# alexoz12v2/cuda-optix-pathtracing

Hardware: AMD Instinct MI355X
Metric: Msamples/s (paths x spp / s) (higher is better)
Workload: dtype f32

## Files before the change

### cuda-optix-pathtracing_amd/binding.py

```python
import ctypes as C
import subprocess
from pathlib import Path

import numpy as np

_HERE = Path(__file__).resolve().parent
_CSRC = _HERE / "csrc"
_LIB = None

DMT_ACCEL_BRUTE_FORCE = 0
DMT_ACCEL_BVH = 1
BVH_BUILD_HOST = 0
BVH_BUILD_DEVICE = 1
BVH_BUILT_BY_HOST = 0
BVH_BUILT_BY_DEVICE = 1
BVH_BUILT_BY_HOST_AFTER_DEVICE = 2
BVH_UPDATE_REBUILD = 0
BVH_UPDATE_REFIT = 1
BVH_UPDATE_AUTO = 2
BVH_UPDATED_NONE = 0
BVH_UPDATED_REFIT = 1
BVH_UPDATED_REBUILD = 2
BVH_UPDATED_REBUILD_AFTER_REFIT = 3


class DmtError(RuntimeError):
    pass


def library_path():
    import os
    alt = os.environ.get("DMT_HIP_LIB")
    return Path(alt) if alt else _CSRC / "libdmt_hip.so"


def build_library(force=False):
    args = ["make", "-C", str(_CSRC)]
    if force:
        args.append("-B")
    subprocess.check_call(args)
    return library_path()


def load_library():
    global _LIB
    if _LIB is None:
        so = library_path()
        if not so.exists():
            raise DmtError(f"{so} is missing: run `python -c 'import __graft_entry__ as g; g.build()'` "
                           "(the HIP path has no fallback)")
        lib = C.CDLL(str(so))
        lib.dmt_last_error.restype = C.c_char_p
        lib.dmt_last_error.argtypes = [C.c_void_p]
        _LIB = lib
    return _LIB


EXPORTED_SYMBOLS = [
    "dmt_ctx_create", "dmt_ctx_destroy", "dmt_last_error", "dmt_upload_triangles", "dmt_upload_bsdfs",
    "dmt_upload_lights", "dmt_set_camera", "dmt_set_limits", "dmt_set_accel", "dmt_set_light_sampling", "dmt_light_tree_pmfs", "dmt_light_tree_ref_select", "dmt_set_bvh_strategy", "dmt_set_partition", "dmt_set_chunk", "dmt_render_profile",
    "dmt_upload_area_lights", "dmt_upload_textures", "dmt_upload_envmap", "dmt_clear_envmap", "dmt_envmap_tables", "dmt_test_envmap",
    "dmt_set_stream", "dmt_film_clear", "dmt_film_bind", "dmt_film_device_ptrs", "dmt_download_film",
    "dmt_render", "dmt_render_adaptive", "dmt_render_stats", "dmt_sync", "dmt_sched_diag", "dmt_kernel_time", "dmt_kernel_info", "dmt_bvh_validate", "dmt_brute_cull_plan", "dmt_brute_cull_box_plan", "dmt_test_triangle_intersect",
    "dmt_test_sampler", "dmt_test_camera_rays", "dmt_test_bsdf", "dmt_test_bsdf_ng", "dmt_test_material", "dmt_test_light", "dmt_test_half",
    "dmt_test_trace_samples", "dmt_test_trace_log", "dmt_test_closest_hit",
    "dmt_set_texture_filter", "dmt_texture_mip_chain", "dmt_texture_footprint", "dmt_test_texture_filter",
    "dmt_render_aovs", "dmt_upload_aovs", "dmt_download_aovs", "dmt_denoise_defaults", "dmt_denoise",
    "dmt_set_accel_build", "dmt_accel_build_info", "dmt_accel_download", "dmt_lbvh_reference", "dmt_bvh_check",
    "dmt_update_vertices", "dmt_update_vertices_device", "dmt_set_accel_update", "dmt_accel_update_info", "dmt_bvh_refit_reference",
    "dmt_download_aov_surface", "dmt_upload_aov_surface", "dmt_camera_project", "dmt_test_camera_project", "dmt_temporal_defaults",
    "dmt_denoise_temporal", "dmt_temporal_reset", "dmt_temporal_info", "dmt_temporal_download",
    "dmt_set_sampler_table", "dmt_sampler_table_plan", "dmt_test_sampler_table",
    "dmt_set_lens", "dmt_lens_info", "dmt_lens_rays", "dmt_focus_distance_at", "dmt_test_lens_values",
    "dmt_set_motion", "dmt_clear_motion", "dmt_set_shutter", "dmt_motion_info", "dmt_shutter_times", "dmt_motion_positions",
    "dmt_motion_bvh_validate", "dmt_test_shutter_times", "dmt_test_closest_hit_at",
]

SAMPLER_TABLE_OFF = 0
SAMPLER_TABLE_AUTO = 1
SAMPLER_TABLE_FORCE = 2


class SamplerTablePlanRecord(C.Structure):
    _fields_ = [("use", C.c_uint32), ("period_width", C.c_uint32), ("period_height", C.c_uint32), ("entry_bytes", C.c_uint32),
                ("slices", C.c_uint32), ("reserved", C.c_uint32), ("slice_bytes", C.c_uint64)]


def sampler_table_plan(width, height, owned_pixels, spp, chunk_spp, budget_bytes=0, mode=SAMPLER_TABLE_AUTO):
    lib = load_library()
    rec = SamplerTablePlanRecord()
    args = [int(width), int(height), C.c_uint64(int(owned_pixels)), C.c_uint32(int(spp)), C.c_uint32(int(chunk_spp)),
            C.c_uint64(int(budget_bytes)), int(mode)]
    rc = lib.dmt_sampler_table_plan(*args, C.byref(rec), None, C.c_uint32(0))
    if rc != 0:
        raise DmtError(f"dmt_sampler_table_plan failed ({rc})")
    lens = (C.c_uint32 * max(int(rec.slices), 1))()
    rc = lib.dmt_sampler_table_plan(*args, C.byref(rec), lens, C.c_uint32(int(rec.slices)))
    if rc != 0:
        raise DmtError(f"dmt_sampler_table_plan failed ({rc})")
    out = {name: int(getattr(rec, name)) for name, _ in SamplerTablePlanRecord._fields_ if name != "reserved"}
    out["use"] = bool(rec.use)
    out["slice_spp"] = [int(x) for x in lens[:int(rec.slices)]]
    return out


class DenoiseParams(C.Structure):
    _fields_ = [("iterations", C.c_int32), ("sigma_normal", C.c_float), ("sigma_position", C.c_float),
                ("sigma_albedo", C.c_float), ("sigma_luminance", C.c_float)]


def denoise_defaults():
    lib = load_library()
    lib.dmt_denoise_defaults.restype = DenoiseParams
    p = lib.dmt_denoise_defaults()
    return {name: getattr(p, name) for name, _ in DenoiseParams._fields_}



class TemporalParams(C.Structure):
    _fields_ = [("alpha", C.c_float), ("normal_threshold", C.c_float), ("plane_threshold", C.c_float)]


class TemporalRecord(C.Structure):
    _fields_ = [("frames", C.c_uint32), ("reprojected", C.c_uint32), ("reset", C.c_uint32), ("temporal_ms", C.c_float),
                ("history_bytes", C.c_uint64)]


def temporal_defaults():
    lib = load_library()
    lib.dmt_temporal_defaults.restype = TemporalParams
    p = lib.dmt_temporal_defaults()
    return {name: getattr(p, name) for name, _ in TemporalParams._fields_}


def camera_project(camera44, points):
    lib = load_library()
    cam = np.ascontiguousarray(camera44, np.uint8).reshape(44)
    p = np.ascontiguousarray(points, np.float32).reshape(-1, 3)
    xy, depth = np.zeros((p.shape[0], 2), np.float32), np.zeros(p.shape[0], np.float32)
    rc = lib.dmt_camera_project(cam.ctypes.data_as(C.c_void_p), int(p.shape[0]), p.ctypes.data_as(C.c_void_p),
                                xy.ctypes.data_as(C.c_void_p), depth.ctypes.data_as(C.c_void_p))
    if rc != 0:
        raise DmtError(f"dmt_camera_project failed ({rc})")
    return xy, depth


def lens_rays(camera44, lens_radius, focus_distance, pxs, pys, ss):
    lib = load_library()
    cam = np.ascontiguousarray(camera44, np.uint8).reshape(44)
    pxs, pys, ss = (np.ascontiguousarray(a, np.int32).reshape(-1) for a in (pxs, pys, ss))
    n = pxs.shape[0]
    assert pys.shape[0] == n and ss.shape[0] == n
    o, d, u = np.zeros((n, 3), np.float32), np.zeros((n, 3), np.float32), np.zeros((n, 2), np.float32)
    as_p = lambda a: a.ctypes.data_as(C.c_void_p)
    rc = lib.dmt_lens_rays(as_p(cam), C.c_float(lens_radius), C.c_float(focus_distance), int(n), as_p(pxs), as_p(pys), as_p(ss),
                           as_p(o), as_p(d), as_p(u))
    if rc != 0:
        raise DmtError(f"dmt_lens_rays failed ({rc})")
# ... 340 lines not shown
        else:
            self.upload_textures(None, None, None, None)

    def upload_textures(self, tex_rgba, tex_desc, mat_tex, tri_uv):
        if tex_desc is None or len(tex_desc) == 0:
            self._check(self._lib.dmt_upload_textures(self._ctx, None, C.c_uint64(0), None, C.c_uint32(0), None, C.c_uint32(0), None,
                                                      C.c_uint64(0)), "dmt_upload_textures")
            return
        rgba = np.ascontiguousarray(tex_rgba, np.uint8).reshape(-1, 4)
        desc = np.ascontiguousarray(tex_desc, np.int32).reshape(-1, 3)
        mt = np.ascontiguousarray(mat_tex, np.uint32).reshape(-1, 4)
        uv = np.ascontiguousarray(tri_uv, np.float32).reshape(-1, 6)
        self._check(self._lib.dmt_upload_textures(self._ctx, _p(rgba), C.c_uint64(rgba.shape[0]), _p(desc), C.c_uint32(desc.shape[0]), _p(mt),
                                                  C.c_uint32(mt.shape[0]), _p(uv), C.c_uint64(uv.shape[0])), "dmt_upload_textures")

    def upload_area_lights(self, tri, le):
        tri = np.ascontiguousarray(tri, np.uint32).reshape(-1)
        le = np.ascontiguousarray(le, np.float32).reshape(-1, 3)
        assert tri.shape[0] == le.shape[0]
        self._check(self._lib.dmt_upload_area_lights(self._ctx, _p(tri), _p(le), C.c_uint32(tri.shape[0])),
                    "dmt_upload_area_lights")

    def upload_envmap(self, rgb, quat=(0, 0, 0, 1), scale=1.0):
        rgb = np.ascontiguousarray(rgb, np.float32)
        h, w = rgb.shape[:2]
        q = np.ascontiguousarray(quat, np.float32)
        self._check(self._lib.dmt_upload_envmap(self._ctx, _p(rgb), int(w), int(h), _p(q), C.c_float(scale)),
                    "dmt_upload_envmap")

    def clear_envmap(self):
        self._check(self._lib.dmt_clear_envmap(self._ctx), "dmt_clear_envmap")

    def test_envmap(self, u2, wi):
        u2, wi = _f32(u2).reshape(-1, 2), _f32(wi).reshape(-1, 3)
        n = u2.shape[0]
        assert wi.shape[0] == n
        out = dict(wi=np.zeros((n, 3), np.float32), pdf=np.zeros(n, np.float32), uv=np.zeros((n, 2), np.float32),
                   Le=np.zeros((n, 3), np.float32), ok=np.zeros(n, np.int32), Le_dir=np.zeros((n, 3), np.float32),
                   pdf_dir=np.zeros(n, np.float32))
        self._check(self._lib.dmt_test_envmap(self._ctx, n, _p(u2), _p(wi), _p(out["wi"]), _p(out["pdf"]), _p(out["uv"]),
                                              _p(out["Le"]), _p(out["ok"]), _p(out["Le_dir"]), _p(out["pdf_dir"])),
                    "dmt_test_envmap")
        return out

    def set_limits(self, max_depth):
        self._check(self._lib.dmt_set_limits(self._ctx, int(max_depth)), "dmt_set_limits")

    def set_accel(self, mode):
        self._check(self._lib.dmt_set_accel(self._ctx, int(mode)), "dmt_set_accel")

    def set_accel_build(self, mode):
        self._check(self._lib.dmt_set_accel_build(self._ctx, int(mode)), "dmt_set_accel_build")

    def accel_build_info(self):
        rec = AccelBuildRecord()
        self._check(self._lib.dmt_accel_build_info(self._ctx, C.byref(rec)), "dmt_accel_build_info")
        return {name: getattr(rec, name) for name, _ in AccelBuildRecord._fields_ if name != "reserved"}

    def download_accel(self):
        info = self.accel_build_info()
        nodes = np.zeros((max(info["nodes"], 1), 64), np.uint8)
        pairs = np.zeros((max(info["pairs"], 1), 2), np.uint32)
        self._check(self._lib.dmt_accel_download(self._ctx, _p(nodes), C.c_size_t(nodes.shape[0]), _p(pairs), C.c_size_t(pairs.shape[0])),
                    "dmt_accel_download")
        return nodes[:info["nodes"]].copy(), pairs[:info["pairs"]].copy()

    def set_light_sampling(self, mode):
        self._check(self._lib.dmt_set_light_sampling(self._ctx, int(mode)), "dmt_set_light_sampling")

    def set_texture_filter(self, mode):
        self._check(self._lib.dmt_set_texture_filter(self._ctx, int(mode)), "dmt_set_texture_filter")

    def set_bvh_strategy(self, strategy, paths_per_pass=0):
        self._check(self._lib.dmt_set_bvh_strategy(self._ctx, int(strategy), C.c_uint64(int(paths_per_pass))), "dmt_set_bvh_strategy")

    def set_partition(self, rank, world):
        self._check(self._lib.dmt_set_partition(self._ctx, int(rank), int(world)), "dmt_set_partition")

    def set_chunk(self, samples_per_item):
        self._check(self._lib.dmt_set_chunk(self._ctx, C.c_uint32(samples_per_item)), "dmt_set_chunk")

    def set_sampler_table(self, mode, budget_bytes=0):
        self._check(self._lib.dmt_set_sampler_table(self._ctx, int(mode), C.c_uint64(int(budget_bytes))), "dmt_set_sampler_table")

    def set_stream(self, stream_ptr):
        self._check(self._lib.dmt_set_stream(self._ctx, C.c_void_p(stream_ptr)), "dmt_set_stream")

    def film_clear(self):
        self._check(self._lib.dmt_film_clear(self._ctx), "dmt_film_clear")

    def film_bind(self, mean_ptr, m2_ptr):
        self._check(self._lib.dmt_film_bind(self._ctx, C.c_void_p(mean_ptr), C.c_void_p(m2_ptr)), "dmt_film_bind")

    def film_device_ptrs(self):
        a, b = C.c_void_p(), C.c_void_p()
        self._check(self._lib.dmt_film_device_ptrs(self._ctx, C.byref(a), C.byref(b)), "dmt_film_device_ptrs")
        return a.value, b.value

    def download_film(self):
        mean = np.zeros((self.height, self.width, 4), np.float32)
        m2 = np.zeros((self.height, self.width, 4), np.float32)
        self._check(self._lib.dmt_download_film(self._ctx, _p(mean), _p(m2)), "dmt_download_film")
        return mean, m2

    def render(self, spp, sample_offset=0, region=None):
        x0, y0, x1, y1 = region if region is not None else (0, 0, self.width, self.height)
        self._check(self._lib.dmt_render(self._ctx, C.c_uint32(sample_offset), C.c_uint32(spp), int(x0), int(y0),
                                         int(x1), int(y1)), "dmt_render")

    def render_adaptive(self, threshold, max_spp, step_spp, min_spp=0, region=None):
        x0, y0, x1, y1 = region if region is not None else (0, 0, self.width, self.height)
        rounds, samples = C.c_uint32(0), C.c_uint64(0)
        self._check(self._lib.dmt_render_adaptive(self._ctx, C.c_uint32(min_spp), C.c_uint32(max_spp), C.c_uint32(step_spp),
                                                  C.c_float(threshold), int(x0), int(y0), int(x1), int(y1), C.byref(rounds),
                                                  C.byref(samples)), "dmt_render_adaptive")
        return int(rounds.value), int(samples.value)

    def render_stats(self, spp, sample_offset=0, region=None):
        x0, y0, x1, y1 = region if region is not None else (0, 0, self.width, self.height)
        out = np.zeros(6, np.uint64)
        self._check(self._lib.dmt_render_stats(self._ctx, C.c_uint32(sample_offset), C.c_uint32(spp), int(x0), int(y0),
                                               int(x1), int(y1), _p(out)), "dmt_render_stats")
        keys = ["samples", "closest_rays", "shadow_rays", "node_visits", "tri_tests", "bounces"]
        return dict(zip(keys, (int(v) for v in out)))

    def render_profile(self, spp, sample_offset=0, region=None):
        x0, y0, x1, y1 = region if region is not None else (0, 0, self.width, self.height)
        out = np.zeros(16, np.uint64)
        self._check(self._lib.dmt_render_profile(self._ctx, C.c_uint32(sample_offset), C.c_uint32(spp), int(x0), int(y0),
                                                 int(x1), int(y1), _p(out)), "dmt_render_profile")
        keys = ["samples", "closest_rays", "shadow_rays", "node_visits", "tri_tests", "bounces", "it_node", "it_leaf",
                "it_shade", "it_outer", "it_prep", "lanes_leaf", "lanes_shade", "lanes_prep", "dead_nodes", "overflow_pushes"]
        return dict(zip(keys, (int(v) for v in out)))

    def render_aovs(self, aov_spp=4):
        self._check(self._lib.dmt_render_aovs(self._ctx, C.c_uint32(aov_spp)), "dmt_render_aovs")
        self._aov_shape = (self.height, self.width)

    def upload_aovs(self, albedo, normal, position):
        a, n, p = _f32(albedo), _f32(normal), _f32(position)
        assert a.ndim == 3 and a.shape[2] == 4 and a.shape == n.shape == p.shape
        h, w = a.shape[:2]
        self._check(self._lib.dmt_upload_aovs(self._ctx, _p(a), _p(n), _p(p), int(w), int(h)), "dmt_upload_aovs")
        self._aov_shape = (h, w)

    def download_aovs(self):
        h, w = self._aov_shape or (self.height, self.width)
        out = [np.zeros((h, w, 4), np.float32) for _ in range(3)]
        self._check(self._lib.dmt_download_aovs(self._ctx, *[_p(x) for x in out]), "dmt_download_aovs")
        return tuple(out)

    def denoise(self, params=None, film=None):
        p = denoise_defaults()
        unknown = set(params or {}) - set(p)
        if unknown:
            raise ValueError(f"unknown denoise parameters {sorted(unknown)}")
        p.update(params or {})
        cp = DenoiseParams(int(p["iterations"]), float(p["sigma_normal"]), float(p["sigma_position"]), float(p["sigma_albedo"]),
                           float(p["sigma_luminance"]))
        mean = m2 = None
        if film is not None:
            mean, m2 = _f32(film[0]), _f32(film[1])
            assert mean.shape == m2.shape == (self.height, self.width, 4)
        out = np.zeros((self.height, self.width, 4), np.float32)
        ms = C.c_float()
        self._check(self._lib.dmt_denoise(self._ctx, C.byref(cp), _p(mean), _p(m2), _p(out), C.byref(ms)), "dmt_denoise")
# ... 67 lines not shown

    def kernel_time(self, reset=True):
        ms, n = C.c_double(), C.c_uint64()
        self._check(self._lib.dmt_kernel_time(self._ctx, C.byref(ms), C.byref(n), int(bool(reset))), "dmt_kernel_time")
        return ms.value, n.value

    def kernel_info(self):
        v = [C.c_int() for _ in range(5)]
        self._check(self._lib.dmt_kernel_info(self._ctx, *[C.byref(x) for x in v]), "dmt_kernel_info")
        keys = ["vgprs", "sgprs", "lds_bytes", "blocks_per_cu", "cu_count"]
        return dict(zip(keys, (x.value for x in v)))

    def test_triangle_intersect(self, xs, ys, zs, o, d):
        xs, ys, zs = _f32(xs), _f32(ys), _f32(zs)
        n = xs.size // 4
        o, d = _f32(o), _f32(d)
        hit = np.zeros(n, np.int32)
        t = np.zeros(n, np.float32)
        pos, nrm, err = (np.zeros((n, 3), np.float32) for _ in range(3))
        self._check(self._lib.dmt_test_triangle_intersect(self._ctx, _p(xs), _p(ys), _p(zs), C.c_size_t(n), _p(o),
                                                          _p(d), _p(hit), _p(t), _p(pos), _p(nrm), _p(err)),
                    "dmt_test_triangle_intersect")
        return hit, t, pos, nrm, err

    def test_sampler(self, w, h, pxs, pys, ss, ndims):
        pxs, pys, ss = _i32(pxs), _i32(pys), _i32(ss)
        n = pxs.shape[0]
        hi = np.zeros(n, np.int32)
        p2 = np.zeros((n, 2), np.float32)
        d = np.zeros((n, ndims), np.float32)
        self._check(self._lib.dmt_test_sampler(self._ctx, int(w), int(h), n, _p(pxs), _p(pys), _p(ss), int(ndims),
                                               _p(hi), _p(p2), _p(d)), "dmt_test_sampler")
        return hi, p2, d

    def test_sampler_table(self, w, h, s0, n):
        pw, ph = min(int(w), 128), min(int(h), 128)
        vals = np.zeros((n, ph, pw, 8), np.float32)
        jit = np.zeros((n, ph, pw, 2), np.float32)
        self._check(self._lib.dmt_test_sampler_table(self._ctx, int(w), int(h), C.c_uint32(int(s0)), C.c_uint32(int(n)), _p(vals), _p(jit)),
                    "dmt_test_sampler_table")
        return vals, jit

    def test_camera_rays(self, pxs, pys, ss):
        pxs, pys, ss = _i32(pxs), _i32(pys), _i32(ss)
        n = pxs.shape[0]
        o = np.zeros((n, 3), np.float32)
        d = np.zeros((n, 3), np.float32)
        self._check(self._lib.dmt_test_camera_rays(self._ctx, n, _p(pxs), _p(pys), _p(ss), _p(o), _p(d)),
                    "dmt_test_camera_rays")
        return o, d

    def test_lens_values(self, pxs, pys, ss):
        pxs, pys, ss = _i32(pxs), _i32(pys), _i32(ss)
        n = pxs.shape[0]
        u = np.zeros((n, 2), np.float32)
        self._check(self._lib.dmt_test_lens_values(self._ctx, n, _p(pxs), _p(pys), _p(ss), _p(u)), "dmt_test_lens_values")
        return u

    def test_bsdf(self, bsdf32, ns, wo, u2, uc, wi_eval):
        b = np.ascontiguousarray(bsdf32, np.uint8).reshape(32)
        ns, wo, wi_eval = _f32(ns, (-1, 3)), _f32(wo, (-1, 3)), _f32(wi_eval, (-1, 3))
        u2, uc = _f32(u2, (-1, 2)), _f32(uc, (-1,))
        n = ns.shape[0]
        prep = np.zeros((n, 12), np.float32)
        samp = np.zeros((n, 10), np.float32)
        ev = np.zeros((n, 4), np.float32)
        self._check(self._lib.dmt_test_bsdf(self._ctx, _p(b), n, _p(ns), _p(wo), _p(u2), _p(uc), _p(wi_eval),
                                            _p(prep), _p(samp), _p(ev)), "dmt_test_bsdf")
        return prep, samp, ev

    def test_bsdf_ng(self, bsdf32, ns, ng, wo, u2, uc, wi_eval):
        b = np.ascontiguousarray(bsdf32, np.uint8).reshape(32)
        ns, ng, wo, wi_eval = _f32(ns, (-1, 3)), _f32(ng, (-1, 3)), _f32(wo, (-1, 3)), _f32(wi_eval, (-1, 3))
        u2, uc = _f32(u2, (-1, 2)), _f32(uc, (-1,))
        n = ns.shape[0]
        assert ng.shape[0] == n and wo.shape[0] == n and wi_eval.shape[0] == n and u2.shape[0] == n and uc.shape[0] == n
        prep = np.zeros((n, 12), np.float32)
        samp = np.zeros((n, 10), np.float32)
        ev = np.zeros((n, 4), np.float32)
        self._check(self._lib.dmt_test_bsdf_ng(self._ctx, _p(b), n, _p(ns), _p(ng), _p(wo), _p(u2), _p(uc), _p(wi_eval),
                                               _p(prep), _p(samp), _p(ev)), "dmt_test_bsdf_ng")
        return prep, samp, ev

    def test_material(self, tri, bu, bv, ng):
        tri, bu, bv, ng = _i32(tri), _f32(bu, (-1,)), _f32(bv, (-1,)), _f32(ng, (-1, 3))
        n = tri.shape[0]
        assert bu.shape[0] == n and bv.shape[0] == n and ng.shape[0] == n
        rec, rec2 = np.zeros((n, 32), np.uint8), np.zeros((n, 32), np.uint8)
        ns = np.zeros((n, 3), np.float32)
        mix = np.zeros(n, np.float32)
        self._check(self._lib.dmt_test_material(self._ctx, n, _p(tri), _p(bu), _p(bv), _p(ng), _p(rec), _p(ns), _p(rec2),
                                                _p(mix)), "dmt_test_material")
        return rec, ns, rec2, mix

    def test_light(self, light32, pos, nrm, u2, had_t):
        l = np.ascontiguousarray(light32, np.uint8).reshape(32)
        pos, nrm, u2 = _f32(pos, (-1, 3)), _f32(nrm, (-1, 3)), _f32(u2, (-1, 2))
        ht = _i32(had_t)
        n = pos.shape[0]
        out = np.zeros((n, 14), np.float32)
        self._check(self._lib.dmt_test_light(self._ctx, _p(l), n, _p(pos), _p(nrm), _p(u2), _p(ht), _p(out)),
                    "dmt_test_light")
        return out

    def test_half(self, floats=None, halves=None):
        h_out = f_out = None
        n = 0
        if floats is not None:
            floats = _f32(floats, (-1,))
            n = floats.shape[0]
            h_out = np.zeros(n, np.uint16)
        if halves is not None:
            halves = np.ascontiguousarray(halves, np.uint16).reshape(-1)
            n = halves.shape[0]
            f_out = np.zeros(n, np.float32)
        if floats is not None and halves is not None:
            assert floats.shape[0] == halves.shape[0]
        self._check(self._lib.dmt_test_half(self._ctx, n, _p(floats), _p(h_out), _p(halves), _p(f_out)),
                    "dmt_test_half")
        return h_out, f_out

    def test_trace_samples(self, pxs, pys, ss):
        pxs, pys, ss = _i32(pxs), _i32(pys), _i32(ss)
        n = pxs.shape[0]
        out = np.zeros((n, 3), np.float32)
        self._check(self._lib.dmt_test_trace_samples(self._ctx, n, _p(pxs), _p(pys), _p(ss), _p(out)),
                    "dmt_test_trace_samples")
        return out

    def test_texture_filter(self, tri, bu, bv, tex, depth=0):
        tri, tex = _i32(tri), _i32(tex)
        bu, bv = _f32(bu), _f32(bv)
        n = tri.shape[0]
        tex = np.ascontiguousarray(np.broadcast_to(tex, (n,)), np.int32)
        depth = np.ascontiguousarray(np.broadcast_to(_i32(depth), (n,)), np.int32)
        assert bu.shape[0] == n and bv.shape[0] == n
        rgb = np.zeros((n, 3), np.float32)
        branch = np.zeros(n, np.int32)
        lod = np.zeros(n, np.float32)
        self._check(self._lib.dmt_test_texture_filter(self._ctx, n, _p(tri), _p(bu), _p(bv), _p(tex), _p(depth), _p(rgb),
                                                      _p(branch), _p(lod)), "dmt_test_texture_filter")
        return rgb, branch, lod

    def test_trace_log(self, px, py, s, cap=64):
        rec = np.zeros((cap, 12), np.float32)
        n = C.c_int()
        L = np.zeros(3, np.float32)
        self._check(self._lib.dmt_test_trace_log(self._ctx, int(px), int(py), int(s), _p(rec), int(cap), C.byref(n),
                                                 _p(L)), "dmt_test_trace_log")
        return rec[:n.value], L

    def test_shutter_times(self, pxs, pys, ss):
        pxs, pys, ss = _i32(pxs), _i32(pys), _i32(ss)
        n = pxs.shape[0]
        t = np.zeros(n, np.float32)
        self._check(self._lib.dmt_test_shutter_times(self._ctx, n, _p(pxs), _p(pys), _p(ss), _p(t)), "dmt_test_shutter_times")
        return t

    def test_closest_hit_at(self, o, d, time):
        o, d = _f32(o, (-1, 3)), _f32(d, (-1, 3))
        n = o.shape[0]
        time = np.ascontiguousarray(np.broadcast_to(np.asarray(time, np.float32), (n,)))
        idx, t, uv = np.zeros(n, np.int32), np.zeros(n, np.float32), np.zeros((n, 2), np.float32)
        self._check(self._lib.dmt_test_closest_hit_at(self._ctx, n, _p(o), _p(d), _p(time), _p(idx), _p(t), _p(uv)),
                    "dmt_test_closest_hit_at")
        return idx, t, uv

    def test_closest_hit(self, o, d):
        o, d = _f32(o, (-1, 3)), _f32(d, (-1, 3))
        n = o.shape[0]
        idx = np.zeros(n, np.int32)
        t = np.zeros(n, np.float32)
        self._check(self._lib.dmt_test_closest_hit(self._ctx, n, _p(o), _p(d), _p(idx), _p(t)),
                    "dmt_test_closest_hit")
        return idx, t
```

### cuda-optix-pathtracing_amd/csrc/dmt_hip.hip

```cpp
#include <hip/hip_runtime.h>

#include <algorithm>
#include <chrono>
#include <cmath>
#include <cstddef>
#include <cstdio>
#include <cstdlib>
#include <cstring>
#include <limits>
#include <memory>
#include <new>
#include <string>
#include <vector>

#include "../../include/dmt_hip.h"
#include "pt_device.hpp"
#include "bvh_device.hpp"
#include "bvh_gpu_build.hpp"
#include "devbuf.hpp"
#include "envmap.hpp"
#include "light_tree.hpp"
#include "light_tree_ref.hpp"

using namespace dmt;

namespace {

constexpr uint32_t kCullMaxClusters = 12;
constexpr uint32_t kCullGroup = 4;
constexpr uint32_t kCullMaxTris = 44;
constexpr uint32_t kCullSlotBits = 6;
constexpr uint32_t kCullMaxIndex = 1u << (32 - kCullSlotBits);
struct CullCluster {
  float b[6];
  uint32_t box;
  uint32_t first, count;
  uint32_t slot, magic;
  uint32_t pad;
};
struct CullRec {
  uint32_t first, countSlot, magic;
};
struct CullView {
  TriIsect const* always;
  uint32_t const* alwaysIdx;
  CullCluster const* clusters;
  float const* tri9;
  uint32_t alwaysCount, clusterCount;
};

struct RenderParams {
  SceneView scene;
  CullView cull;
  BvhView bvh;
  CameraXf cam;
  SamplerParams sp;
  float4* __restrict__ mean;
  float4* __restrict__ m2;
  uint32_t* __restrict__ counter;
  int width, height;
  int x0, y0, x1, y1;
  int tx0, ty0, rtx;
  uint32_t numItems;
  uint32_t subShift;
  int rank, world;
  uint32_t sampleOffset, spp;
  uint32_t chunkSpp;
  uint32_t numChunks;
  float* stage;
  uint32_t* link;
  uint32_t* slabBusy;
  uint32_t const* tileList;
  unsigned long long const* tileMask;
  unsigned long long* schedDiag;
  float4 const* samTab;
  float2 const* samTabJit;
  float2 const* samTabLens;
  uint32_t samTabS0, samTabPw, samTabPh;
  float lensR, lensD;
  int maxDepth;
  int shadeThreshold;
  EnvView env;
  uint32_t const* areaOf;
  uint32_t const* areaTri;
  float const* areaLe;
  uint32_t areaCount;
  uint32_t const* texRgba;
  int32_t const* texDesc;
  uint32_t const* matTex;
  float const* triUv;
  LightTreeNode const* lightTree;
  LightTreeRefNode const* lightTreeRef;
  unsigned long long* stats;
  float texCfr[12];
  float texMinDx[3], texMinDy[3];
  float texSppScale;
  uint32_t const* texMip;
  int32_t const* texMipDesc;
  MotionView motion;
};

typedef RenderParams const DMT_CONST_AS* KArgs;
DMT_DEV KArgs kargs_base() { return (KArgs)__builtin_amdgcn_kernarg_segment_ptr(); }
DMT_DEV KArgs kargs(KArgs p) {
  asm volatile("" : "+s"(p));
  return p;
}
DMT_DEV SceneView load_scene(KArgs k) {
  k = kargs(k);
  SceneView s;
  s.tris = k->scene.tris, s.post = k->scene.post, s.bsdfs = k->scene.bsdfs, s.lights = k->scene.lights;
  s.infLights = k->scene.infLights, s.triCount = k->scene.triCount, s.bsdfCount = k->scene.bsdfCount;
  s.lightCount = k->scene.lightCount, s.infLightCount = k->scene.infLightCount;
  return s;
}
DMT_DEV BvhView load_bvh(KArgs k) {
  k = kargs(k);
  BvhView b;
  b.nodes = k->bvh.nodes, b.pairs = k->bvh.pairs, b.overflow = k->bvh.overflow, b.overflowStride = k->bvh.overflowStride;
  return b;
}

DMT_DEV EnvView load_env(KArgs k) {
  k = kargs(k);
  EnvView e;
  e.func = k->env.func, e.cdf = k->env.cdf, e.rowInt = k->env.rowInt, e.mFunc = k->env.mFunc, e.mCdf = k->env.mCdf;
  e.rgb = k->env.rgb, e.mInt = k->env.mInt, e.w = k->env.w, e.h = k->env.h;
  e.qx = k->env.qx, e.qy = k->env.qy, e.qz = k->env.qz, e.qw = k->env.qw;
  return e;
}

#ifndef DMT_SECTION_TIMING
#define DMT_SECTION_TIMING 0
#endif
#if DMT_SECTION_TIMING
__device__ unsigned long long g_sect[16];
__shared__ unsigned long long s_sectLast[kLdsThreads / 64];
__shared__ unsigned long long s_sectAcc[kLdsThreads / 64][16];
#endif
DMT_DEV void sect_mark(int i) {
#if DMT_SECTION_TIMING
  unsigned long long const now = __builtin_readcyclecounter();
  unsigned long long const m = __ballot(1);
  if (int(__ffsll((long long)m)) - 1 == int(threadIdx.x & 63u)) {
    uint32_t const w = threadIdx.x >> 6;
    s_sectAcc[w][i] += now - s_sectLast[w];
    s_sectLast[w] = now;
  }
#endif
}
struct PathState {
  RayPair rp;
  f3 beta, L;
  int depth;
  bool lastT;
  bool active;
  bool hasShadow;
  bool finPending;
  float smax;
  Sampler rng;
  uint32_t sidx;
  float lastPdf;
  bool lastSpecular;
};
__shared__ float s_cold[7 * kLdsThreads];
DMT_DEV void put_C(f3 v) {
  float* const c = s_cold + threadIdx.x;
  c[0 * kLdsThreads] = v.x, c[1 * kLdsThreads] = v.y, c[2 * kLdsThreads] = v.z;
}
DMT_DEV f3 get_C() {
  float const* const c = s_cold + threadIdx.x;
  return mk3(c[0 * kLdsThreads], c[1 * kLdsThreads], c[2 * kLdsThreads]);
}
DMT_DEV void put_Lfin(f3 v) {
  float* const c = s_cold + threadIdx.x;
  c[3 * kLdsThreads] = v.x, c[4 * kLdsThreads] = v.y, c[5 * kLdsThreads] = v.z;
}
DMT_DEV f3 get_Lfin() {
  float const* const c = s_cold + threadIdx.x;
  return mk3(c[3 * kLdsThreads], c[4 * kLdsThreads], c[5 * kLdsThreads]);
}
DMT_DEV void put_finIdx(uint32_t i) { s_cold[6 * kLdsThreads + threadIdx.x] = __uint_as_float(i); }
// ... 431 lines not shown
  gram_schmidt(ng, tx, ty);
  f3 const ns = tx * n.x + ty * n.y + ng * n.z;
  float const l2 = dot(ns, ns);
  return (l2 > 0.f && l2 < kInf) ? ns / sqrtf(l2) : ng;
}

template <bool CULL = true>
DMT_DEV void trace_pair_brute(KArgs k, PathState const& st, bool doC, bool doS, int& bestTri, float& bu, float& bv, bool& occluded);

#include "motion.hpp"

constexpr uint32_t kFeatBvh = 1u << 0;
constexpr uint32_t kFeatStats = 1u << 1;
constexpr uint32_t kFeatEnv = 1u << 2;
constexpr uint32_t kFeatArea = 1u << 3;
constexpr uint32_t kFeatTex = 1u << 4;
constexpr uint32_t kFeatBlend = 1u << 5;
constexpr uint32_t kFeatLightTree = 1u << 6;
constexpr uint32_t kFeatLightTreeRef = 1u << 7;
constexpr uint32_t kFeatTexFilter = 1u << 8;
constexpr uint32_t kFeatMotion = 1u << 9;

template <uint32_t F>
DMT_DEV Hit shade_hit(KArgs k, SceneView const& sc, int tri, float bu, float bv, f3 rd) {
  if constexpr (F & kFeatMotion) return hit_finish(motion_post(k, sc.post[tri], tri, motion_time()), bu, bv, rd);
  else return hit_finish(sc.post[tri], bu, bv, rd);
}

template <uint32_t F>
DMT_DEV bool path_shade(KArgs k, PathState& st, int bestTri, float bu, float bv) {
  static_assert(!((F & kFeatLightTree) && (F & kFeatLightTreeRef)), "one light tree at a time");
  static_assert(!((F & kFeatTex) && (F & kFeatBlend)), "kFeatBlend carries the texture code itself");
  static_assert(!(F & kFeatTexFilter) || (F & (kFeatTex | kFeatBlend)), "the texture filter needs the texture code");
  static_assert(!(F & kFeatMotion) || !(F & ~(kFeatMotion | kFeatBvh | kFeatEnv)), "motion: the plain and env-map rows only");
  SceneView const sc = load_scene(k);
  int const maxDepth = kargs(k)->maxDepth;
  if constexpr (F & kFeatEnv) {
    if (bestTri < 0) {
      EnvView const env = load_env(k);
      float pdfLight = 0.f;
      f3 const Le = env_eval_dir(env, ray_dir(st), pdfLight);
      if (st.depth == 0 || st.lastSpecular)
        st.L = st.L + st.beta * Le;
      else
        st.L = st.L + st.beta * (st.lastPdf / (st.lastPdf + pdfLight)) * Le;
      return true;
    }
  }
  if (bestTri < 0) {
    if (sc.infLightCount > 0) {
      uint32_t const li = pick_index(st.rng.get1D(), sc.infLightCount);
      Rec32 const light = sc.infLights[li];
      float const pmf = 1.f / float(sc.infLightCount);
      if (light_type(light) == LT_ENV) st.L = st.L + st.beta * light_intensity(light) / pmf;
    }
    sect_mark(4);
    return true;
  }
  f3 const rd = ray_dir(st);
  Hit const hit = shade_hit<F>(k, sc, bestTri, bu, bv, rd);
  uint32_t nAll = sc.lightCount;
  if constexpr (F & kFeatArea) {
    KArgs const ka = kargs(k);
    nAll += ka->areaCount;
    uint32_t const ai = ka->areaOf[bestTri];
    if (ai != 0xFFFFFFFFu) {
      f3 const o = mk3(st.rp.ox.x, st.rp.oy.x, st.rp.oz.x);
      float const pl = area_pdf(sc.post[bestTri], rd, dot(hit.pos - o, rd));
      if (pl > 0.f) {
        f3 const Le = mk3(ka->areaLe[3 * ai], ka->areaLe[3 * ai + 1], ka->areaLe[3 * ai + 2]);
        if (st.depth == 0 || st.lastSpecular) {
          st.L = st.L + st.beta * Le;
        } else {
          float const a = st.lastPdf, b = pl * ((F & kFeatEnv) ? 0.5f : 1.f) / float(nAll);
          st.L = st.L + st.beta * Le * ((a * a) / (a * a + b * b));
        }
      }
    }
  }
  sect_mark(4);
  if (st.depth >= maxDepth) return true;

  f3 const wo = -rd;
  Rec32 rec = sc.bsdfs[hit.matId];
  f3 ns = hit.normal;
  Rec32 rec2{};
  float mix = 0.f;
  bool blend = false;
  constexpr bool FILT = (F & kFeatTexFilter) != 0;
  TexDiff td{0.f, 0.f, 0.f, 0.f};
  if constexpr (FILT) {
    if (st.depth == 0) td = tex_footprint(k, bestTri, hit.pos, hit.normal);
  }
  if constexpr (F & kFeatBlend) {
    if (hi16(rec.w[1]) == BS_GGX_BLEND) {
      mix = blend_metallic<FILT>(k, rec, hit.matId, bestTri, bu, bv, td);
      rec.w[1] = (rec.w[1] & 0x0000FFFFu) | (uint32_t(BS_GGX_DIEL) << 16);
      rec2 = sc.bsdfs[hit.matId + 1u];
      if (mix >= 1.f) rec = rec2;
      else blend = mix > 0.f;
    }
  }
  if constexpr (F & (kFeatTex | kFeatBlend)) {
    if (!(F & kFeatBlend) || kargs(k)->matTex != nullptr) {
      ns = apply_material_textures<FILT>(k, rec, hit.matId, bestTri, bu, bv, hit.normal, td);
      if (blend) (void)apply_material_textures<FILT>(k, rec2, hit.matId + 1u, bestTri, bu, bv, hit.normal, td);
    }
  }
#if DMT_SECTION_TIMING
  {
    bool const ggx = hi16(rec.w[1]) != BS_OREN;
    unsigned long long const all = __ballot(1), mg = __ballot(ggx);
    if (int(__ffsll((long long)all)) - 1 == int(threadIdx.x & 63u)) {
      unsigned long long* const acc = s_sectAcc[threadIdx.x >> 6];
      acc[11] += mg ? 1u : 0u, acc[12] += uint32_t(__popcll(mg)), acc[13] += 1u, acc[14] += uint32_t(__popcll(all));
    }
  }
#endif
  Bsdf const b = bsdf_prepare(rec, ns, wo);
  Bsdf b2{};
  if constexpr (F & kFeatBlend) {
    if (blend) b2 = bsdf_prepare(rec2, ns, wo);
  }
  auto blend_pdf = [&](float pdfD, float pdfC) { return (1.f - pdfD) * pdfC + pdfD * mix; };
  auto eval_material = [&](f3 wi, float& pdf) {
    f3 f = eval_bsdf(b, wo, wi, ns, hit.normal, pdf) * b.weight;
    if constexpr (F & kFeatBlend) {
      if (blend) {
        float pdfC = 0.f;
        f3 const fC = eval_bsdf(b2, wo, wi, ns, hit.normal, pdfC) * b2.weight;
        f = f * (1.f - mix) + fC * mix;
        pdf = blend_pdf(pdf, pdfC);
      }
    }
    return f;
  };
  sect_mark(5);

  float uLight = st.rng.get1D();
  f2 const uLight2 = st.rng.get2D();
  bool envNee = false;
  if constexpr (F & kFeatEnv) {
    envNee = uLight < 0.5f;
    uLight = envNee ? uLight : (uLight - 0.5f) * 2.f;
    if (envNee) {
      EnvView const env = load_env(k);
      EnvSampleDev const es = env_sample(env, uLight2);
      if (es.ok) {
        float bsdfPdf = 0.f;
        f3 const f = eval_material(es.wi, bsdfPdf);
        f3 const Le = env_eval_uv(env, es.uv);
        if (!is_zero(f) && max3(Le) > 0.f) {
          put_C(st.beta * (Le * f / (es.pdf * 0.5f + bsdfPdf)));
          set_shadow_ray(st, offset_ray_origin(hit.pos, hit.error, hit.normal, es.wi), es.wi);
          st.smax = kInf;
          st.hasShadow = true;
        }
      }
    }
  }
  bool areaNee = false;
  if constexpr (F & kFeatArea) {
    uint32_t const li = pick_index(uLight, nAll);
    areaNee = !envNee && li >= sc.lightCount;
    if (areaNee) {
      KArgs const ka = kargs(k);
      uint32_t const ai = li - sc.lightCount;
      AreaSampleDev const as = area_sample(sc.post[ka->areaTri[ai]], hit.pos, uLight2);
      if (as.ok) {
        float bsdfPdf = 0.f;
        f3 const f = eval_material(as.wi, bsdfPdf);
        if (!is_zero(f)) {
          f3 const Le = mk3(ka->areaLe[3 * ai], ka->areaLe[3 * ai + 1], ka->areaLe[3 * ai + 2]);
          float const a = as.pdf * ((F & kFeatEnv) ? 0.5f : 1.f) / float(nAll), bb = bsdfPdf;
          put_C(st.beta * (Le * f * (((a * a) / (a * a + bb * bb)) / a)));
          set_shadow_ray(st, offset_ray_origin(hit.pos, hit.error, hit.normal, as.wi), as.wi);
          st.smax = as.dist * 0.999f;
          st.hasShadow = true;
        }
      }
    }
  }
  bool treeNee = false;
  if constexpr (F & kFeatLightTreeRef) {
    treeNee = !envNee && sc.lightCount > 1;
    if (treeNee) {
      LightTreeRefSelection const sel = ltr_select(kargs(k)->lightTreeRef, hit.pos.x, hit.pos.y, hit.pos.z, hit.normal.x, hit.normal.y,
                                                   hit.normal.z, uLight, (F & kFeatEnv) ? 0.5f : 1.f);
      bool pending = false;
      f3 pendC = mk3(0, 0, 0), pendO = mk3(0, 0, 0), pendD = mk3(0, 0, 0);
      float pendMax = 0.f;
      for (uint32_t i = 0; i < sel.count; ++i) {
        Rec32 const light = sc.lights[sel.indices[i]];
        float const pmf = sel.pmfs[i];
        LightSample const ls = sample_light(light, hit.pos, uLight2, st.lastT, hit.normal);
        if (!ls.valid()) continue;
        float bsdfPdf = 0.f;
        f3 const f = eval_material(ls.direction, bsdfPdf);
        if (is_zero(f)) continue;
        f3 const Le = eval_light(light, ls);
        f3 C;
        if (ls.delta) {
          C = st.beta * Le * f / pmf;
        } else {
          float const w = sqr(pmf * ls.pdf) / sqr(pmf * ls.pdf + bsdfPdf);
          C = Le * f * st.beta * w;
        }
        if (pending) {
          bool occ;
          if constexpr (F & kFeatBvh) {
            occ = bvh_any(load_bvh(k), true, pendO, pendD, pendMax, blockIdx.x * blockDim.x + threadIdx.x);
          } else {
            PathState tmp = st;
            set_shadow_ray(tmp, pendO, pendD);
            tmp.smax = pendMax;
            int bt;
            float tu, tvv;
            trace_pair_brute<false>(k, tmp, false, true, bt, tu, tvv, occ);
          }
          if (!occ) st.L = st.L + pendC;
        }
        pending = true, pendC = C, pendMax = ls.distance;
        pendO = offset_ray_origin(hit.pos, hit.error, hit.normal, ls.direction), pendD = ls.direction;
      }
      if (pending) {
        put_C(pendC);
        set_shadow_ray(st, pendO, pendD);
        st.smax = pendMax;
        st.hasShadow = true;
      }
    }
  }
  if (!envNee && !areaNee && !treeNee && sc.lightCount > 0) {
    uint32_t li = 0;
    float pmf = 0.f;
    bool picked = true;
    if constexpr (F & kFeatLightTree) {
      float treePmf = 0.f;
      int const sel = lt_select(kargs(k)->lightTree, hit.pos.x, hit.pos.y, hit.pos.z, hit.normal.x, hit.normal.y, hit.normal.z, uLight, treePmf);
      picked = sel >= 0;
      li = picked ? uint32_t(sel) : 0u;
      pmf = ((F & kFeatEnv) ? 0.5f : 1.f) * treePmf;
    } else {
      li = pick_index(uLight, (F & kFeatArea) ? nAll : sc.lightCount);
      pmf = ((F & kFeatEnv) ? 0.5f : 1.f) / float((F & kFeatArea) ? nAll : sc.lightCount);
    }
    Rec32 const light = sc.lights[li];
    LightSample const ls = sample_light(light, hit.pos, uLight2, st.lastT, hit.normal);
    sect_mark(6);
    if (picked && ls.valid()) {
      float bsdfPdf = 0.f;
      f3 const f = eval_material(ls.direction, bsdfPdf);
      if (!is_zero(f)) {
        f3 const Le = eval_light(light, ls);
        if (ls.delta) {
          put_C(st.beta * Le * f / pmf);
        } else {
          float const w = sqr(pmf * ls.pdf) / sqr(pmf * ls.pdf + bsdfPdf);
          put_C(Le * f * st.beta * w);
        }
        set_shadow_ray(st, offset_ray_origin(hit.pos, hit.error, hit.normal, ls.direction), ls.direction);
        st.smax = ls.distance;
        st.hasShadow = true;
      }
    }
  }

  sect_mark(7);
  f2 const u2 = st.rng.get2D();
  float const uc = st.rng.get1D();
  BsdfSample bs = sample_bsdf(b, wo, ns, hit.normal, u2, uc);
  if constexpr (F & kFeatBlend) {
    if (blend) {
      BsdfSample sC = sample_bsdf(b2, wo, ns, hit.normal, u2, uc);
      sC.f = bs.f * (1.f - mix) + sC.f * mix;
      sC.pdf = blend_pdf(bs.pdf, sC.pdf);
      sC.eta = 1.f;
      bs = sC;
    }
  }
  sect_mark(8);
  if (!bs.valid()) return true;
  st.lastT = bs.refract;
  if constexpr (F & (kFeatEnv | kFeatArea)) st.lastPdf = bs.pdf, st.lastSpecular = bs.delta;
  set_ray(st, offset_ray_origin(hit.pos, hit.error, hit.normal, bs.wi), bs.wi);
  st.beta = st.beta * (bs.f * fabsf(dot(bs.wi, hit.normal)) / bs.pdf);
  float const rrBeta = max3(st.beta * bs.eta);
  if (rrBeta < 1 && st.depth > 1) {
    float const q = fmaxf(0.f, 1.f - rrBeta);
    if (st.rng.get1D() < q) return true;
    st.beta = st.beta / (1 - q);
  }
  ++st.depth;
  sect_mark(9);
  return false;
}

DMT_DEV TriS load_tri(TriIsect const DMT_CONST_AS* tris, uint32_t i) {
  TriS T;
  T.p0x = tris[i].p0x, T.p0y = tris[i].p0y, T.p0z = tris[i].p0z;
  T.e0x = tris[i].e0x, T.e0y = tris[i].e0y, T.e0z = tris[i].e0z;
  T.e1x = tris[i].e1x, T.e1y = tris[i].e1y, T.e1z = tris[i].e1z;
  return T;
}

struct BruteHit {
  float bt, bu, bv;
  int tri;
  bool occluded;
};
#define DMT_TRI_DECL(P) float P##0, P##1, P##2, P##3, P##4, P##5, P##6, P##7, P##8
#define DMT_TRI_LOAD(P, idx)                                                                          \
  P##0 = tris[idx].p0x, P##1 = tris[idx].p0y, P##2 = tris[idx].p0z, P##3 = tris[idx].e0x, P##4 = tris[idx].e0y, \
  P##5 = tris[idx].e0z, P##6 = tris[idx].e1x, P##7 = tris[idx].e1y, P##8 = tris[idx].e1z
#define DMT_TRI_TEST(P, idx)                                                                                   \
  do {                                                                                                         \
    MTPair m;                                                                                                  \
    mt_core9<v2f>(P##0, P##1, P##2, P##3, P##4, P##5, P##6, P##7, P##8, st.rp.ox, st.rp.oy, st.rp.oz, st.rp.dx, \
                  st.rp.dy, st.rp.dz, m.det, m.t, m.u, m.v);                                                   \
    bool const v1 = mt_valid(m.det.x, m.t.x, m.u.x, m.v.x);                                                    \
    bool const v2 = mt_valid(m.det.y, m.t.y, m.u.y, m.v.y);                                                    \
    if (doC && v1 && m.t.x < h.bt) {                  \
      h.bt = m.t.x;                                                                                            \
      h.tri = int(idx);                                                                                        \
      h.bu = m.u.x;                                                                                            \
      h.bv = m.v.x;                                                                                            \
    }                                                                                                          \
    if (doS && v2 && m.t.y < st.smax) h.occluded = true;                                         \
  } while (0)

__shared__ float s_cullTri[9 * kCullMaxTris];
__shared__ CullRec s_cullRec[kCullMaxClusters];
__shared__ unsigned long long s_cullKey[kLdsThreads];
__shared__ unsigned long long s_cullOcc[kLdsThreads / 64];
__shared__ uint8_t s_cullOwner[kLdsThreads / 64][kCullGroup][128];
constexpr float kCullTSlack = 1.0f + 1.0f / 256;
constexpr float kCullRel = 1.0f / 16384;
constexpr float kCullTLo = 1e-4f * (1.0f - 1.0f / 256);

#ifndef DMT_CULL_COUNTS
#define DMT_CULL_COUNTS 0
#endif
#if DMT_CULL_COUNTS
__device__ unsigned long long g_cullCount[16];
#endif

DMT_DEV void cull_stage(KArgs k) {
  k = kargs(k);
  if (k->cull.clusterCount == 0) return;
  float const* const t9 = k->cull.tri9;
  for (uint32_t i = threadIdx.x; i < 9 * kCullMaxTris; i += blockDim.x) s_cullTri[i] = t9[i];
  CullCluster const* const cl = k->cull.clusters;
  for (uint32_t i = threadIdx.x; i < kCullMaxClusters; i += blockDim.x)
    s_cullRec[i] = CullRec{cl[i].first, cl[i].count | cl[i].slot << 16, cl[i].magic};
// ... 820 lines not shown
        }
        bool const onNode = traversing && !(tv.cur & kBvhLeafFlag);
        bool const onLeaf = traversing && (tv.cur & kBvhLeafFlag) != 0u;
        int const nNode = __popcll(__ballot(onNode)), nLeaf = __popcll(__ballot(onLeaf));
        if (nNode + nLeaf == 0) break;
        if (__popcll(__ballot(tv.phase == TR_DONE)) >= shadeThreshold) break;
#ifdef DMT_BVH_BOTH_STEPS
        if constexpr (STATS) ++ls.itNode, ++ls.itLeaf, ls.lanesLeaf += onLeaf ? 1u : 0u;
        if (onNode) trav_node<STATS>(bvh, tv, STATS ? &ls.tc : nullptr);
        if (onLeaf) trav_leaf<STATS>(bvh, tv, ray_org(st), ray_dir(st), STATS ? &ls.tc : nullptr, leafMotion());
#else
        if (nNode * DMT_BVH_NODE_WEIGHT >= nLeaf * DMT_BVH_LEAF_WEIGHT) {
          if constexpr (STATS) ++ls.itNode;
          if (onNode) {
            trav_node<STATS>(bvh, tv, nd, STATS ? &ls.tc : nullptr);
            if (!(tv.cur & kBvhLeafFlag)) nd = node_fetch(bvh, tv.cur);
          }
        } else {
          if constexpr (STATS) ++ls.itLeaf, ls.lanesLeaf += onLeaf ? 1u : 0u;
          if (onLeaf) {
            trav_leaf<STATS>(bvh, tv, ray_org(st), ray_dir(st), STATS ? &ls.tc : nullptr, leafMotion());
            if (!(tv.cur & kBvhLeafFlag)) nd = node_fetch(bvh, tv.cur);
          }
        }
#endif
      }
      if constexpr (STATS) ++ls.itShade, ls.lanesShade += tv.phase == TR_DONE ? 1u : 0u;
      if (tv.phase == TR_DONE) {
        if constexpr (STATS) ls.bounces += (st.active && tv.bestTri >= 0 && st.depth < kargs(Pk)->maxDepth) ? 1u : 0u;
        lane_finish<F & ~kFeatStats>(Pk, st, st.active, st.hasShadow, tv.bestTri, tv.bu, tv.bv, st.smax < 0.f, sink);
        tv.phase = TR_IDLE;
      }
    }
  }
  flush_stats<STATS>(Pk, ls);
}

#define DMT_MEGAKERNELS(X)                                                          \
  X(, 0, DMT_MIN_WAVES_PER_SIMD, megakernel_body)                                   \
  X(_bvh, kFeatBvh, DMT_MIN_WAVES_PER_SIMD_BVH, megakernel_body_bvh)                \
  X(_env, kFeatEnv, 4, megakernel_body)                                             \
  X(_bvh_env, kFeatBvh | kFeatEnv, 3, megakernel_body_bvh)                          \
  X(_area, kFeatArea, 4, megakernel_body)                                           \
  X(_bvh_area, kFeatBvh | kFeatArea, 3, megakernel_body_bvh)                        \
  X(_env_area, kFeatEnv | kFeatArea, 4, megakernel_body)                            \
  X(_bvh_env_area, kFeatBvh | kFeatEnv | kFeatArea, 3, megakernel_body_bvh)         \
  X(_tex, kFeatTex, 4, megakernel_body)                                             \
  X(_bvh_tex, kFeatBvh | kFeatTex, 3, megakernel_body_bvh)                          \
  X(_env_tex, kFeatEnv | kFeatTex, 4, megakernel_body)                              \
  X(_bvh_env_tex, kFeatBvh | kFeatEnv | kFeatTex, 3, megakernel_body_bvh)           \
  X(_blend, kFeatBlend, 3, megakernel_body)                                         \
  X(_bvh_blend, kFeatBvh | kFeatBlend, 2, megakernel_body_bvh)                      \
  X(_env_blend, kFeatEnv | kFeatBlend, 3, megakernel_body)                          \
  X(_bvh_env_blend, kFeatBvh | kFeatEnv | kFeatBlend, 2, megakernel_body_bvh)       \
  X(_ltree, kFeatLightTree, 4, megakernel_body)                                     \
  X(_bvh_ltree, kFeatBvh | kFeatLightTree, 3, megakernel_body_bvh)                  \
  X(_env_ltree, kFeatEnv | kFeatLightTree, 4, megakernel_body)                      \
  X(_bvh_env_ltree, kFeatBvh | kFeatEnv | kFeatLightTree, 3, megakernel_body_bvh)   \
  X(_ltree2, kFeatLightTreeRef, 3, megakernel_body)                                 \
  X(_bvh_ltree2, kFeatBvh | kFeatLightTreeRef, 2, megakernel_body_bvh)              \
  X(_env_ltree2, kFeatEnv | kFeatLightTreeRef, 3, megakernel_body)                  \
  X(_bvh_env_ltree2, kFeatBvh | kFeatEnv | kFeatLightTreeRef, 2, megakernel_body_bvh)   \
  X(_texf, kFeatTex | kFeatTexFilter, 2, megakernel_body)                           \
  X(_bvh_texf, kFeatBvh | kFeatTex | kFeatTexFilter, 2, megakernel_body_bvh)        \
  X(_env_texf, kFeatEnv | kFeatTex | kFeatTexFilter, 2, megakernel_body)            \
  X(_bvh_env_texf, kFeatBvh | kFeatEnv | kFeatTex | kFeatTexFilter, 2, megakernel_body_bvh) \
  X(_blendf, kFeatBlend | kFeatTexFilter, 2, megakernel_body)                       \
  X(_bvh_blendf, kFeatBvh | kFeatBlend | kFeatTexFilter, 2, megakernel_body_bvh)    \
  X(_env_blendf, kFeatEnv | kFeatBlend | kFeatTexFilter, 2, megakernel_body)        \
  X(_bvh_env_blendf, kFeatBvh | kFeatEnv | kFeatBlend | kFeatTexFilter, 2, megakernel_body_bvh) \
  X(_motion, kFeatMotion, 4, megakernel_body)                                       \
  X(_bvh_motion, kFeatBvh | kFeatMotion, 3, megakernel_body_bvh)                    \
  X(_env_motion, kFeatEnv | kFeatMotion, 4, megakernel_body)                        \
  X(_bvh_env_motion, kFeatBvh | kFeatEnv | kFeatMotion, 3, megakernel_body_bvh)
#define DMT_STATS_MEGAKERNELS(X)                                                    \
  X(_bvh_stats, kFeatBvh | kFeatStats, 2, megakernel_body_bvh)                      \
  X(_bvh_stats_env, kFeatBvh | kFeatStats | kFeatEnv, 2, megakernel_body_bvh)

#define DMT_DEFINE_MEGAKERNEL(suffix, mask, waves, body) \
  __global__ void __launch_bounds__(256, waves) k_megakernel##suffix(RenderParams P) { body<mask>(); }
DMT_MEGAKERNELS(DMT_DEFINE_MEGAKERNEL)
DMT_STATS_MEGAKERNELS(DMT_DEFINE_MEGAKERNEL)

__global__ void __launch_bounds__(256) k_sampler_table(SamplerParams sp, uint32_t s0, uint32_t n, uint32_t pw, uint32_t ph,
                                                       float4* vals, float2* jit, float2* lens) {
  uint32_t const e = blockIdx.x * 256u + threadIdx.x;
  if (e >= n * pw * ph) return;
  uint32_t const x = e % pw, row = e / pw, y = row % ph, k = row / ph;
  int32_t const hidx = halton_pixel_base(sp, int(x), int(y)) + int32_t(s0 + k) * (sp.scale0 * sp.scale1);
  float* const u = s_sampler_u + threadIdx.x;
  sampler_values(uint32_t(hidx), u);
  vals[2 * size_t(e)] = make_float4(u[0 * kLdsThreads], u[1 * kLdsThreads], u[2 * kLdsThreads], u[3 * kLdsThreads]);
  vals[2 * size_t(e) + 1] = make_float4(u[4 * kLdsThreads], u[5 * kLdsThreads], u[6 * kLdsThreads], u[7 * kLdsThreads]);
  f2 const p = pixel2d(sp, hidx);
  jit[e] = make_float2(p.x, p.y);
  if (lens) {
    LensU const u = lens_values(uint32_t(hidx));
    lens[e] = make_float2(u.x, u.y);
  }
}

DMT_DEV bool adaptive_active(float4 m, float4 v, uint32_t offset, uint32_t minSpp, uint32_t maxSpp, float threshold) {
  float const N = v.w;
  if (N != float(offset) || !(N < float(maxSpp))) return false;
  if (N < float(minSpp) || N < 2.f) return true;
  float const err = sqrtf((v.x + v.y + v.z) / (N * (N - 1.f))) / fmaxf(m.x + m.y + m.z, 1e-3f);
  return err > threshold;
}
struct AdaptiveArgs {
  float4 const* mean;
  float4 const* m2;
  unsigned long long* mask;
  uint32_t* list;
  uint32_t* counters;
  int width, x0, y0, x1, y1, tx0, ty0, rtx;
  uint32_t owned;
  int rank, world;
  uint32_t offset, minSpp, maxSpp;
  float threshold;
};
__global__ void __launch_bounds__(256) k_adaptive_mask(AdaptiveArgs A) {
  uint32_t const w = blockIdx.x * 4u + (threadIdx.x >> 6);
  if (w >= A.owned) return;
  int const lane = int(threadIdx.x) & 63;
  uint32_t const j = uint32_t(A.rank) + w * uint32_t(A.world);
  int const px = (A.tx0 + int(j % uint32_t(A.rtx))) * 8 + (lane & 7), py = (A.ty0 + int(j / uint32_t(A.rtx))) * 8 + (lane >> 3);
  bool active = false;
  if (px >= A.x0 && px < A.x1 && py >= A.y0 && py < A.y1) {
    size_t const pidx = size_t(px) + size_t(py) * size_t(A.width);
    active = adaptive_active(film_load(A.mean + pidx), film_load(A.m2 + pidx), A.offset, A.minSpp, A.maxSpp, A.threshold);
  }
  unsigned long long const word = __ballot(active);
  if (lane == 0) {
    A.mask[j] = word;
    if (word != 0ull) {
      A.list[atomicAdd(&A.counters[0], 1u)] = j;
      atomicAdd(&A.counters[1], uint32_t(__popcll(word)));
    }
  }
}

#include "wavefront.hpp"
#include "denoise.hpp"

}

constexpr uint32_t kSamTabEntryBytes = 40;
constexpr uint32_t kSamTabLensEntryBytes = 48;
constexpr uint64_t kSamTabDefaultBudget = 512ull << 20;
constexpr uint64_t kSamTabMinRatio = 4;
struct SamplerTablePlan {
  bool use = false;
  uint32_t pw = 0, ph = 0;
  uint32_t slices = 0;
  uint32_t sliceChunks = 0;
};
static SamplerTablePlan samplerTablePlan(int width, int height, uint64_t ownedPixels, uint32_t spp, uint32_t chunkSpp, uint64_t budget, int mode,
                                         uint32_t entryBytes = kSamTabEntryBytes) {
  SamplerTablePlan p;
  if (width <= 0 || height <= 0) return p;
  p.pw = uint32_t(width < 128 ? width : 128), p.ph = uint32_t(height < 128 ? height : 128);
  if (mode == DMT_SAMPLER_TABLE_OFF || spp == 0 || chunkSpp == 0) return p;
  if (chunkSpp > spp) chunkSpp = spp;
  uint64_t const period = uint64_t(p.pw) * p.ph;
  if (mode != DMT_SAMPLER_TABLE_FORCE && ownedPixels < kSamTabMinRatio * period) return p;
  uint64_t const chunkEntries = uint64_t(chunkSpp) * period;
  uint64_t maxChunks = budget / (chunkEntries * entryBytes);
  uint64_t const maxChunksByIndex = 0x7FFFFFFFull / chunkEntries;
  if (maxChunks > maxChunksByIndex) maxChunks = maxChunksByIndex;
  if (maxChunks == 0) return p;
  uint64_t const numChunks = (uint64_t(spp) + chunkSpp - 1) / chunkSpp;
  uint64_t const k = (numChunks + maxChunks - 1) / maxChunks;
  p.sliceChunks = uint32_t((numChunks + k - 1) / k);
  p.slices = uint32_t((numChunks + p.sliceChunks - 1) / p.sliceChunks);
  p.use = true;
  return p;
}

struct dmt_ctx {
  int device = 0;
  hipStream_t ownStream = nullptr;
  hipStream_t stream = nullptr;
  std::string err;
  DevBuf<TriIsect> d_tris;
  DevBuf<TriPost> d_post;
  DevBuf<Rec32> d_bsdfs, d_lights, d_inf;
  uint32_t triCount = 0, bsdfCount = 0, lightCount = 0, infCount = 0;
  uint32_t maxMatId = 0;
  int bruteCull = 2;
  DevBuf<TriIsect> d_cullAlways;
  DevBuf<uint32_t> d_cullIdx;
  DevBuf<CullCluster> d_cullClusters;
  DevBuf<float> d_cullTri9;
  uint32_t cullAlwaysCount = 0, cullClusterCount = 0;
  std::vector<float> h_xs, h_ys, h_zs;
  std::vector<uint32_t> h_mat;
  DevBuf<Bvh4Node> d_bvhNodes;
  int shadeThresholdEnv = 0;
  DevBuf<TriPair> d_trisBvh;
  DevBuf<uint32_t> d_overflow;
  bool haveBvh = false;
  int bvhDepth = 0;
  uint32_t bvhNodeCount = 0, bvhPairCount = 0;
  int blocksPerCUBvh = 0;
  int accelBuild = DMT_BVH_BUILD_HOST;
  dmt_accel_build_record buildRecord{};
  lbvh_gpu::Scratch lbvhScratch;
  std::vector<uint32_t> bvhLevels;
  int accelUpdate = DMT_BVH_UPDATE_REBUILD;
  double maxCostRatio = 0.0;
  dmt_accel_update_record updateRecord{};
  bool costAtBuildKnown = false;
  lbvh_gpu::RefitScratch refitScratch;
  int lightSampling = DMT_LIGHTS_UNIFORM;
  std::vector<uint8_t> h_lights;
  DevBuf<LightTreeNode> d_lightTree;
  DevBuf<LightTreeRefNode> d_lightTreeRef;
  uint32_t lightTreeNodes = 0;
  int lightTreeDepth = 0;
  bool lightTreeValid = false;
  bool lightTreeTooDeep = false;
  bool lightsTreeable = false;
  std::vector<std::pair<void const*, int>> occupancy;
  DevBuf<uint32_t> d_texRgba;
  DevBuf<int32_t> d_texDesc;
  DevBuf<uint32_t> d_matTex;
  DevBuf<float> d_triUv;
  uint32_t texCount = 0, matTexCount = 0;
  DevBuf<uint32_t> d_texMip;
  DevBuf<int32_t> d_texMipDesc;
  int texFilter = DMT_TEXFILTER_LEVEL0;
  float texFoot[19] = {};
  bool hasBlend = false;
  size_t triUvCount = 0;
  int bvhStrategy = 0;
  size_t wfTargetPaths = size_t(1) << 22;
  DevBuf<float> d_wfState;
  DevBuf<uint32_t> d_wfQueue;
  DevBuf<uint32_t> d_wfCounts;
  int wfBlocksTrace = 0, wfBlocksShade = 0;
  DevBuf<float> d_env;
  EnvView env{};
  DevBuf<uint32_t> d_areaOf;
  DevBuf<uint32_t> d_areaTri;
  DevBuf<float> d_areaLe;
  uint32_t areaCount = 0;
  std::vector<uint32_t> h_areaTri;
  std::vector<float> h_areaLe;
  bool haveTris = false, haveBsdfs = false, haveLights = false, haveCamera = false;
  dmt_camera cam{};
  CameraXf xf{};
  SamplerParams sp{};
  float lensR = 0.f, lensD = 1.f;
  bool haveMotion = false;
  float shutterOpen = 0.f, shutterClose = 1.f;
  std::vector<float> h_xs1, h_ys1, h_zs1;
  DevBuf<TriIsect> d_dtris;
  DevBuf<TriKey1> d_post1;
  DevBuf<Bvh4Node> d_mNodes;
  DevBuf<TriPair> d_mPairs;
  DevBuf<TriPairDelta> d_mDelta;
  bool haveMotionTree = false;
  uint32_t mNodeCount = 0, mPairCount = 0;
  int mDepth = 0;
  double mBuildMs = 0.0;
  DevBuf<float4> ownMean, ownM2;
  float4* d_mean = nullptr;
  float4* d_m2 = nullptr;
  int filmW = 0, filmH = 0;
// ... 302 lines not shown
  if (c->env.w > 0) F |= kFeatEnv;
  if (c->areaCount > 0) F |= kFeatArea;
  if (c->hasBlend) F |= kFeatBlend;
  else if (c->texCount > 0) F |= kFeatTex;
  if (treeable && c->lightSampling == DMT_LIGHTS_TREE) F |= kFeatLightTree;
  if (treeable && c->lightSampling == DMT_LIGHTS_TREE_REFERENCE) F |= kFeatLightTreeRef;
  if (c->texFilter == DMT_TEXFILTER_REFERENCE && (F & (kFeatTex | kFeatBlend))) F |= kFeatTexFilter;
  if (c->haveMotion) F |= kFeatMotion;
  return F;
}
int ensureLightTree(dmt_ctx* ctx);
int resolveFeatures(dmt_ctx* ctx, uint32_t* mask) {
  if ((featuresOf(ctx) & (kFeatLightTree | kFeatLightTreeRef)) && !ctx->lightTreeValid) {
    if (int const rc = ensureLightTree(ctx)) return rc;
  }
  *mask = featuresOf(ctx);
  return DMT_OK;
}
int checkFeatures(dmt_ctx* ctx, uint32_t F) {
  if (F & kFeatMotion) {
    if (F & kFeatStats) return fail(ctx, DMT_ERR_STATE, "dmt_render_stats / dmt_render_profile: motion blur (dmt_set_motion) has no counting kernels");
    if (F & kFeatTexFilter) return fail(ctx, DMT_ERR_STATE, "dmt_render: motion blur (dmt_set_motion) together with the first-hit texture filter is not supported");
    if (F & (kFeatTex | kFeatBlend)) return fail(ctx, DMT_ERR_STATE, "dmt_render: motion blur (dmt_set_motion) together with image textures or blend materials is not supported");
    if (F & kFeatArea) return fail(ctx, DMT_ERR_STATE, "dmt_render: motion blur (dmt_set_motion) together with emissive triangles is not supported");
    if (F & (kFeatLightTree | kFeatLightTreeRef)) return fail(ctx, DMT_ERR_STATE, "dmt_render: motion blur (dmt_set_motion) together with a light tree is not supported");
    if ((F & kFeatBvh) && ctx->bvhStrategy == 2) return fail(ctx, DMT_ERR_STATE, "dmt_render: motion blur (dmt_set_motion) together with the wavefront BVH strategy is not supported");
  }
  if ((F & kFeatStats) && (F & (kFeatTex | kFeatBlend | kFeatArea | kFeatLightTree | kFeatLightTreeRef)))
    return fail(ctx, DMT_ERR_STATE, "dmt_render_stats / dmt_render_profile: the counting kernels exist for the plain and env-map BVH kernels only; "
                                    "with textures, blended materials, emissive triangles or a light tree they would describe a different kernel");
  if ((F & kFeatBlend) && (F & kFeatArea)) return fail(ctx, DMT_ERR_STATE, "dmt_render: fractional-metallic materials together with emissive triangles are not supported");
  if ((F & kFeatTex) && (F & kFeatArea)) return fail(ctx, DMT_ERR_STATE, "dmt_render: image textures together with emissive triangles are not supported");
  if (ctx->texCount > 0 && (ctx->matTexCount != ctx->bsdfCount || ctx->triUvCount != ctx->triCount))
    return fail(ctx, DMT_ERR_STATE, "dmt_render: texture tables do not match the uploaded BSDFs / triangles (upload textures last)");
  return DMT_OK;
}

SceneView sceneView(dmt_ctx const* c) {
  SceneView s;
  s.tris = c->d_tris.get(), s.post = c->d_post.get(), s.bsdfs = c->d_bsdfs.get(), s.lights = c->d_lights.get();
  s.infLights = c->d_inf.get();
  s.triCount = c->triCount, s.bsdfCount = c->bsdfCount, s.lightCount = c->lightCount;
  s.infLightCount = c->infCount;
  return s;
}

BvhView bvhView(dmt_ctx const* c, size_t threads) {
  BvhView b;
  b.nodes = c->d_bvhNodes.get(), b.pairs = c->d_trisBvh.get(), b.overflow = c->d_overflow.get();
  b.overflowStride = uint32_t(threads);
  return b;
}

int bvhShadeThreshold(dmt_ctx const* c) {
  if (c->shadeThresholdEnv > 0) return c->shadeThresholdEnv;
  uint32_t const n = c->bvhNodeCount;
  return n <= 1024u ? 56 : n <= 16384u ? 52 : n <= 131072u ? 40 : DMT_BVH_SHADE_THRESHOLD;
}
RenderParams baseParams(dmt_ctx const* c, size_t threads) {
  RenderParams P{};
  P.scene = sceneView(c);
  if (c->cullClusterCount > 0) {
    P.cull.always = c->d_cullAlways.get(), P.cull.alwaysIdx = c->d_cullIdx.get(), P.cull.clusters = c->d_cullClusters.get();
    P.cull.tri9 = c->d_cullTri9.get(), P.cull.alwaysCount = c->cullAlwaysCount, P.cull.clusterCount = c->cullClusterCount;
  } else {
    P.cull.always = c->d_tris.get(), P.cull.alwaysCount = c->triCount;
  }
  P.bvh = bvhView(c, threads);
  P.cam = c->xf;
  P.sp = c->sp;
  P.lensR = c->lensR, P.lensD = c->lensD;
  P.maxDepth = c->maxDepth;
  P.shadeThreshold = bvhShadeThreshold(c);
  P.env = c->env;
  P.areaOf = c->d_areaOf.get(), P.areaTri = c->d_areaTri.get(), P.areaLe = c->d_areaLe.get(), P.areaCount = c->areaCount;
  if (c->texCount > 0) {
    P.texRgba = c->d_texRgba.get(), P.texDesc = c->d_texDesc.get(), P.matTex = c->d_matTex.get(), P.triUv = c->d_triUv.get();
    P.texMip = c->d_texMip.get(), P.texMipDesc = c->d_texMipDesc.get();
    memcpy(P.texCfr, c->texFoot, 12 * sizeof(float));
    memcpy(P.texMinDx, c->texFoot + 12, 3 * sizeof(float));
    memcpy(P.texMinDy, c->texFoot + 15, 3 * sizeof(float));
    P.texSppScale = c->texFoot[18];
  }
  uint32_t const F = featuresOf(c);
  if ((F & kFeatLightTree) && c->lightTreeValid) P.lightTree = c->d_lightTree.get();
  if ((F & kFeatLightTreeRef) && c->lightTreeValid) P.lightTreeRef = c->d_lightTreeRef.get();
  return P;
}

template <class Fn>
struct KernelRow { uint32_t mask; Fn fn; };
template <class Fn, size_t N>
Fn kernelOf(KernelRow<Fn> const (&rows)[N], uint32_t mask) {
  for (KernelRow<Fn> const& r : rows) if (r.mask == mask) return r.fn;
  return nullptr;
}
int noKernel(dmt_ctx* ctx, char const* what, uint32_t mask) {
  ctx->err = std::string(what) + ": no kernel is compiled for this combination of scene features (mask " + std::to_string(mask) + ")";
  return DMT_ERR_STATE;
}
typedef void (*MegakernelFn)(RenderParams);
typedef void (*WfKernelFn)(RenderParams, WfParams);
#define DMT_MEGAKERNEL_ROW(suffix, mask, waves, body) {mask, k_megakernel##suffix},
#define DMT_WF_SHADE_ROW(suffix, mask, waves) {mask, k_wf_shade##suffix},
KernelRow<MegakernelFn> const kMegakernels[] = {DMT_MEGAKERNELS(DMT_MEGAKERNEL_ROW) DMT_STATS_MEGAKERNELS(DMT_MEGAKERNEL_ROW)};
KernelRow<WfKernelFn> const kWfShadeKernels[] = {DMT_WF_SHADE_KERNELS(DMT_WF_SHADE_ROW)};

MegakernelFn megakernelOf(uint32_t mask) { return kernelOf(kMegakernels, mask); }
int blocksPerCuOf(dmt_ctx* c, MegakernelFn kernel) {
  void const* const fn = reinterpret_cast<void const*>(kernel);
  for (auto const& e : c->occupancy)
    if (e.first == fn) return e.second;
  int n = 0;
  if (hipOccupancyMaxActiveBlocksPerMultiprocessor(&n, fn, 256, 0) != hipSuccess || n <= 0) n = 1;
  c->occupancy.emplace_back(fn, n);
  return n;
}

hipError_t reserveOverflow(dmt_ctx* ctx, size_t threads) { return ctx->d_overflow.reserve(threads * size_t(kBvhOverflowStack)); }

void treeBuilt(dmt_ctx* ctx) {
  ctx->updateRecord.updates_since_build = 0;
  ctx->updateRecord.sah_cost = ctx->updateRecord.sah_cost_at_build = 0.0;
  ctx->costAtBuildKnown = false;
}

int buildBvhHost(dmt_ctx* ctx, int builder) {
  uint32_t const n = ctx->triCount;
  auto const t0 = std::chrono::steady_clock::now();
  bvh_build::Result r = bvh_build::build(ctx->h_xs.data(), ctx->h_ys.data(), ctx->h_zs.data(), n);
  size_t const npairs = r.pairTris.size() / 2;
  if (npairs > 0x7FFFFFFFull || r.nodes.size() > 0x7FFFFFFFull) return fail(ctx, DMT_ERR_INVALID, "BVH: too many nodes / triangle pairs");
  std::vector<TriPair> pairs(npairs ? npairs + 3 : 0);
  for (size_t p = 0; p < npairs; ++p)
    for (int half = 0; half < 2; ++half) {
      uint32_t const i = r.pairTris[2 * p + size_t(half)];
      float const* xs = &ctx->h_xs[4 * size_t(i)];
      float const* ys = &ctx->h_ys[4 * size_t(i)];
      float const* zs = &ctx->h_zs[4 * size_t(i)];
      TriPair& P = pairs[p];
      P.p0x[half] = xs[0], P.p0y[half] = ys[0], P.p0z[half] = zs[0];
      P.e0x[half] = xs[1] - xs[0], P.e0y[half] = ys[1] - ys[0], P.e0z[half] = zs[1] - zs[0];
      P.e1x[half] = xs[2] - xs[0], P.e1y[half] = ys[2] - ys[0], P.e1z[half] = zs[2] - zs[0];
      P.orig[half] = i;
    }
  for (size_t p = npairs; p < pairs.size(); ++p) pairs[p] = pairs[npairs - 1];
  DevBuf<Bvh4Node> nodes;
  DevBuf<TriPair> leaves;
  HIP_TRY(ctx, nodes.assign(r.nodes.data(), r.nodes.size()));
  HIP_TRY(ctx, leaves.assign(pairs.data(), pairs.size()));
  ctx->d_bvhNodes = std::move(nodes), ctx->d_trisBvh = std::move(leaves);
  ctx->bvhDepth = r.depth;
  ctx->bvhNodeCount = uint32_t(r.nodes.size());
  ctx->bvhPairCount = uint32_t(npairs);
  ctx->haveBvh = true;
  ctx->bvhLevels = refit::levelBounds(r.nodes.data(), r.nodes.size());
  treeBuilt(ctx);
  dmt_accel_build_record& R = ctx->buildRecord;
  R = dmt_accel_build_record{};
  R.builder = builder;
  R.triangles = n, R.nodes = ctx->bvhNodeCount, R.pairs = ctx->bvhPairCount, R.depth = r.depth;
  R.build_ms = std::chrono::duration<double, std::milli>(std::chrono::steady_clock::now() - t0).count();
  return DMT_OK;
}

int buildBvh(dmt_ctx* ctx) {
// ... 266 lines not shown
  HIP_TRY(ctx, hipMemcpy(&folds, ctx->d_schedDiag.get(), sizeof(folds), hipMemcpyDeviceToHost));
  if (folds != ctx->expectedFolds) {
    char msg[200];
    snprintf(msg, sizeof(msg), "in-launch ordering: %llu sample chunks were folded into the film, %llu were launched: the film is invalid",
             folds, ctx->expectedFolds);
    ctx->expectedFolds = folds;
    return fail(ctx, DMT_ERR_HIP, msg);
  }
  return DMT_OK;
}

int finishTest(dmt_ctx* ctx) {
  HIP_TRY(ctx, hipGetLastError());
  HIP_TRY(ctx, hipStreamSynchronize(ctx->stream));
  return DMT_OK;
}

}

#include "denoise_host.hpp"

static int rebuildAreaLights(dmt_ctx* ctx);

extern "C" {

int dmt_ctx_create(int device_ordinal, dmt_ctx** out) {
  if (!out) return DMT_ERR_INVALID;
  *out = nullptr;
  int count = 0;
  if (hipGetDeviceCount(&count) != hipSuccess || count <= 0) {
    g_createError = "no HIP device available (the HIP path has no CPU fallback)";
    return DMT_ERR_NO_DEVICE;
  }
  if (device_ordinal < 0 || device_ordinal >= count) {
    g_createError = "device ordinal out of range";
    return DMT_ERR_INVALID;
  }
  std::unique_ptr<dmt_ctx> ctx(new (std::nothrow) dmt_ctx());
  if (!ctx) return DMT_ERR_INVALID;
  ctx->device = device_ordinal;
  hipError_t e = hipSetDevice(device_ordinal);
  if (e == hipSuccess) e = hipStreamCreateWithFlags(&ctx->ownStream, hipStreamNonBlocking);
  hipDeviceProp_t prop{};
  if (e == hipSuccess) e = hipGetDeviceProperties(&prop, device_ordinal);
  if (e == hipSuccess) e = ctx->d_counter.reserve(2);
  if (e == hipSuccess) e = hipMemset(ctx->d_counter.get(), 0, 2 * sizeof(uint32_t));
  if (e == hipSuccess) e = ctx->d_schedDiag.reserve(kSchedDiagWords);
  if (e == hipSuccess) e = hipMemset(ctx->d_schedDiag.get(), 0, kSchedDiagWords * sizeof(unsigned long long));
  int bpc = 0;
  if (e == hipSuccess)
    e = hipOccupancyMaxActiveBlocksPerMultiprocessor(&bpc, reinterpret_cast<void const*>(k_megakernel), 256, 0);
  int bpcBvh = 0;
  if (e == hipSuccess)
    e = hipOccupancyMaxActiveBlocksPerMultiprocessor(&bpcBvh, reinterpret_cast<void const*>(k_megakernel_bvh), 256, 0);
  if (e != hipSuccess) {
    g_createError = std::string("dmt_ctx_create: ") + hipGetErrorString(e);
    if (ctx->ownStream) (void)hipStreamDestroy(ctx->ownStream);
    return DMT_ERR_HIP;
  }
  ctx->stream = ctx->ownStream;
  ctx->cuCount = prop.multiProcessorCount;
  ctx->blocksPerCU = bpc > 0 ? bpc : 1;
  ctx->blocksPerCUBvh = bpcBvh > 0 ? bpcBvh : 1;
  if (char const* e3 = std::getenv("DMT_BVH_STRATEGY")) {
    int const v = std::atoi(e3);
    ctx->bvhStrategy = v < 0 || v > 2 ? 0 : v;
  }
  if (char const* e5 = std::getenv("DMT_BVH_SHADE_THRESHOLD")) {
    int const v = std::atoi(e5);
    ctx->shadeThresholdEnv = v < 1 ? 0 : (v > 64 ? 64 : v);
  }
  if (char const* e4 = std::getenv("DMT_WF_PATHS")) {
    long long const v = std::atoll(e4);
    if (v >= 4096) ctx->wfTargetPaths = size_t(v);
  }
  if (char const* e6 = std::getenv("DMT_BRUTE_CULL")) {
    int const v = std::atoi(e6);
    ctx->bruteCull = v == 0 ? 0 : v == 1 ? 1 : 2;
  }
  if (char const* e7 = std::getenv("DMT_SAMPLER_TABLE")) {
    int const v = std::atoi(e7);
    ctx->samTabMode = v == 0 ? DMT_SAMPLER_TABLE_OFF : v == 2 ? DMT_SAMPLER_TABLE_FORCE : DMT_SAMPLER_TABLE_AUTO;
  }
  if (char const* e2 = std::getenv("DMT_SUB_SHIFT")) {
    int const v = std::atoi(e2);
    ctx->subShift = v < 0 ? -1 : (v > 2 ? 2 : v);
  }
  *out = ctx.release();
  return DMT_OK;
}

int dmt_ctx_destroy(dmt_ctx* ctx) {
  if (!ctx) return DMT_ERR_INVALID;
  (void)hipSetDevice(ctx->device);
  (void)hipStreamSynchronize(ctx->stream);
  for (auto& ev : ctx->events) {
    (void)hipEventDestroy(ev.first);
    (void)hipEventDestroy(ev.second);
  }
  if (ctx->ownStream) (void)hipStreamDestroy(ctx->ownStream);
  delete ctx;
  return DMT_OK;
}

const char* dmt_last_error(const dmt_ctx* ctx) { return ctx ? ctx->err.c_str() : g_createError.c_str(); }

int dmt_upload_triangles(dmt_ctx* ctx, const float* xs, const float* ys, const float* zs,
                         const uint32_t* mat_id, size_t count) {
  if (!ctx) return DMT_ERR_INVALID;
  if ((count && (!xs || !ys || !zs || !mat_id)) || count > 0x7FFFFFFFu)
    return fail(ctx, DMT_ERR_INVALID, "dmt_upload_triangles: null array or count out of range");
  HIP_TRY(ctx, hipSetDevice(ctx->device));
  std::vector<TriIsect> a;
  std::vector<TriPost> b;
  packSoup(xs, ys, zs, mat_id, count, a, b);
  uint32_t maxMat = 0;
  for (size_t i = 0; i < count; ++i)
    if (mat_id[i] > maxMat) maxMat = mat_id[i];
  DevBuf<TriIsect> tris;
  DevBuf<TriPost> post;
  HIP_TRY(ctx, tris.assign(a.data(), count));
  HIP_TRY(ctx, post.assign(b.data(), count));
  CullTables cull;
  if (int const rcC = uploadCullTables(ctx, planCullClusters(ctx, xs, ys, zs, mat_id, count), a.data(), count, cull)) return rcC;
  ctx->d_tris = std::move(tris), ctx->d_post = std::move(post);
  adoptCullTables(ctx, cull);
  ctx->triCount = uint32_t(count);
  ctx->maxMatId = maxMat;
  ctx->haveTris = true;
  ctx->h_xs.assign(xs, xs + 4 * count), ctx->h_ys.assign(ys, ys + 4 * count), ctx->h_zs.assign(zs, zs + 4 * count);
  ctx->h_mat.assign(mat_id, mat_id + count);
  ctx->haveBvh = false;
  dropMotion(ctx);
  ctx->dn.dropVertexMirror();
  ctx->h_areaTri.clear(), ctx->h_areaLe.clear();
  if (int const rcA = rebuildAreaLights(ctx)) return rcA;
  if (ctx->accel == DMT_ACCEL_BVH) return buildBvh(ctx);
  return DMT_OK;
}

namespace {
int beginUpdate(dmt_ctx* ctx, char const* name, bool nullArray, size_t count, EventPair& T, bool* done) {
  *done = false;
  if (!ctx) return DMT_ERR_INVALID;
  if (!ctx->haveTris) return fail(ctx, DMT_ERR_STATE, "update of vertices before any dmt_upload_triangles");
  if (count != ctx->triCount) return fail(ctx, DMT_ERR_INVALID, "update of vertices: count differs from the uploaded triangle count");
  if (count && nullArray) {
    ctx->err = std::string(name) + ": null array";
    return DMT_ERR_INVALID;
  }
  if (count == 0) {
    *done = true;
    return DMT_OK;
  }
  HIP_TRY(ctx, hipSetDevice(ctx->device));
  HIP_TRY(ctx, hipStreamSynchronize(ctx->stream));
  HIP_TRY(ctx, hipEventCreate(&T.a));
  HIP_TRY(ctx, hipEventCreate(&T.b));
  HIP_TRY(ctx, hipEventRecord(T.a, ctx->stream));
  return DMT_OK;
}
}

int dmt_update_vertices(dmt_ctx* ctx, const float* xs, const float* ys, const float* zs, size_t count) {
  EventPair T;
  bool done = false;
  if (int const rc = beginUpdate(ctx, "dmt_update_vertices", !xs || !ys || !zs, count, T, &done)) return rc;
  if (done) return DMT_OK;
  dropMotion(ctx);
  std::vector<TriIsect> a;
  std::vector<TriPost> b;
  packSoup(xs, ys, zs, ctx->h_mat.data(), count, a, b);
  CullTables cull;
  if (int const rcC = uploadCullTables(ctx, planCullClusters(ctx, xs, ys, zs, ctx->h_mat.data(), count), a.data(), count, cull)) return rcC;
  HIP_TRY(ctx, hipMemcpy(ctx->d_tris.get(), a.data(), count * sizeof(TriIsect), hipMemcpyHostToDevice));
  HIP_TRY(ctx, hipMemcpy(ctx->d_post.get(), b.data(), count * sizeof(TriPost), hipMemcpyHostToDevice));
  adoptCullTables(ctx, cull);
  ctx->h_xs.assign(xs, xs + 4 * count), ctx->h_ys.assign(ys, ys + 4 * count), ctx->h_zs.assign(zs, zs + 4 * count);
  if (int const rcT = mirrorHostUpdate(ctx)) return rcT;
  return finishUpdate(ctx, T);
}

int dmt_update_vertices_device(dmt_ctx* ctx, const void* d_verts9, size_t count) {
  EventPair T;
  bool done = false;
  if (int const rc = beginUpdate(ctx, "dmt_update_vertices_device", !d_verts9, count, T, &done)) return rc;
  if (done) return DMT_OK;
  dropMotion(ctx);
  HIP_TRY(ctx, lbvh_gpu::packRecords(static_cast<float const*>(d_verts9), uint32_t(count), ctx->d_tris.get(), ctx->d_post.get(), ctx->stream));
  if (int const rcT = mirrorDeviceUpdate(ctx, d_verts9, count)) return rcT;
  std::vector<TriPost> b(count);
  HIP_TRY(ctx, hipMemcpyAsync(b.data(), ctx->d_post.get(), count * sizeof(TriPost), hipMemcpyDeviceToHost, ctx->stream));
  HIP_TRY(ctx, hipStreamSynchronize(ctx->stream));
  for (size_t i = 0; i < count; ++i) {
    TriPost const& q = b[i];
    ctx->h_xs[4 * i] = q.p0x, ctx->h_xs[4 * i + 1] = q.p1x, ctx->h_xs[4 * i + 2] = q.p2x;
    ctx->h_ys[4 * i] = q.p0y, ctx->h_ys[4 * i + 1] = q.p1y, ctx->h_ys[4 * i + 2] = q.p2y;
    ctx->h_zs[4 * i] = q.p0z, ctx->h_zs[4 * i + 1] = q.p1z, ctx->h_zs[4 * i + 2] = q.p2z;
  }
  std::vector<CullCluster> const clusters = planCullClusters(ctx, ctx->h_xs.data(), ctx->h_ys.data(), ctx->h_zs.data(), ctx->h_mat.data(), count);
  std::vector<TriIsect> a;
  if (!clusters.empty()) {
    a.resize(count);
    HIP_TRY(ctx, hipMemcpy(a.data(), ctx->d_tris.get(), count * sizeof(TriIsect), hipMemcpyDeviceToHost));
  }
  CullTables cull;
  if (int const rcC = uploadCullTables(ctx, clusters, a.data(), count, cull)) return rcC;
  adoptCullTables(ctx, cull);
  return finishUpdate(ctx, T);
}

int dmt_set_accel_update(dmt_ctx* ctx, int mode, double max_cost_ratio) {
  if (!ctx) return DMT_ERR_INVALID;
  if (mode != DMT_BVH_UPDATE_REBUILD && mode != DMT_BVH_UPDATE_REFIT && mode != DMT_BVH_UPDATE_AUTO)
    return fail(ctx, DMT_ERR_INVALID, "dmt_set_accel_update: unknown mode");
  if (mode == DMT_BVH_UPDATE_AUTO && !(std::isfinite(max_cost_ratio) && max_cost_ratio > 1.0))
    return fail(ctx, DMT_ERR_INVALID, "dmt_set_accel_update: DMT_BVH_UPDATE_AUTO needs a finite max_cost_ratio > 1");
  ctx->accelUpdate = mode;
  if (mode == DMT_BVH_UPDATE_AUTO) ctx->maxCostRatio = max_cost_ratio;
  return DMT_OK;
}

int dmt_accel_update_info(dmt_ctx* ctx, dmt_accel_update_record* out) {
  if (!ctx || !out) return DMT_ERR_INVALID;
  *out = ctx->updateRecord;
  return DMT_OK;
}

int dmt_upload_bsdfs(dmt_ctx* ctx, const void* bsdf32, uint32_t count) {
  if (!ctx) return DMT_ERR_INVALID;
  if (count && !bsdf32) return fail(ctx, DMT_ERR_INVALID, "dmt_upload_bsdfs: null array");
  HIP_TRY(ctx, hipSetDevice(ctx->device));
  DevBuf<Rec32> bsdfs;
  HIP_TRY(ctx, bsdfs.assign(bsdf32, count));
  bool blend = false;
  for (uint32_t i = 0; i < count; ++i) {
    uint32_t w1;
    memcpy(&w1, static_cast<unsigned char const*>(bsdf32) + 32 * size_t(i) + 4, 4);
    if ((w1 >> 16) == BS_GGX_BLEND) {
      uint32_t w1next = 0;
      if (i + 1 < count) memcpy(&w1next, static_cast<unsigned char const*>(bsdf32) + 32 * size_t(i + 1) + 4, 4);
      if (i + 1 >= count || (w1next >> 16) != BS_GGX_COND)
        return fail(ctx, DMT_ERR_INVALID, "dmt_upload_bsdfs: a blend record (type 4) must be followed by its GGX conductor record");
      blend = true;
    }
  }
  ctx->d_bsdfs = std::move(bsdfs);
  ctx->hasBlend = blend;
  ctx->bsdfCount = count;
  ctx->haveBsdfs = true;
  return DMT_OK;
}

int dmt_upload_lights(dmt_ctx* ctx, const void* lights32, uint32_t count, const void* infinite32,
                      uint32_t infinite_count) {
  if (!ctx) return DMT_ERR_INVALID;
  if ((count && !lights32) || (infinite_count && !infinite32))
    return fail(ctx, DMT_ERR_INVALID, "dmt_upload_lights: null array");
  HIP_TRY(ctx, hipSetDevice(ctx->device));
  DevBuf<Rec32> lights, inf;
  HIP_TRY(ctx, lights.assign(lights32, count));
  HIP_TRY(ctx, inf.assign(infinite32, infinite_count));
  ctx->d_lights = std::move(lights), ctx->d_inf = std::move(inf);
  ctx->lightCount = count;
  ctx->infCount = infinite_count;
  ctx->haveLights = true;
  ctx->h_lights.assign(static_cast<uint8_t const*>(lights32), static_cast<uint8_t const*>(lights32) + size_t(count) * 32);
  ctx->lightTreeValid = false;
  ctx->lightTreeTooDeep = false;
  ctx->lightsTreeable = count > 0;
  for (uint32_t i = 0; i < count; ++i) {
    uint16_t type;
    memcpy(&type, ctx->h_lights.data() + 32 * size_t(i) + 6, 2);
    if (type != 0 && type != 1) ctx->lightsTreeable = false;
  }
  return DMT_OK;
}

int dmt_set_camera(dmt_ctx* ctx, const dmt_camera* cam) {
  if (!ctx) return DMT_ERR_INVALID;
  if (!cam || cam->width <= 0 || cam->height <= 0 || cam->width > 65536 || cam->height > 65536)
    return fail(ctx, DMT_ERR_INVALID, "dmt_set_camera: bad camera / resolution");
  HIP_TRY(ctx, hipSetDevice(ctx->device));
  if (cam->width != ctx->filmW || cam->height != ctx->filmH) {
    size_t const pixels = size_t(cam->width) * size_t(cam->height);
    DevBuf<float4> mean, m2;
    HIP_TRY(ctx, mean.reserve(pixels));
    HIP_TRY(ctx, m2.reserve(pixels));
    HIP_TRY(ctx, hipMemsetAsync(mean.get(), 0, pixels * sizeof(float4), ctx->stream));
    HIP_TRY(ctx, hipMemsetAsync(m2.get(), 0, pixels * sizeof(float4), ctx->stream));
    ctx->ownMean = std::move(mean), ctx->ownM2 = std::move(m2);
    ctx->d_mean = ctx->ownMean.get(), ctx->d_m2 = ctx->ownM2.get();
    ctx->filmW = cam->width, ctx->filmH = cam->height;
    ctx->dn.dropHistory();
  }
  ctx->cam = *cam;
  float m[16];
  cameraFromRaster(cam->focal_length, cam->sensor_size, uint32_t(cam->width), uint32_t(cam->height), m);
  memcpy(ctx->xf.cfr, m, sizeof(m));
  worldFromCamera(cam->dir, cam->pos, m);
  memcpy(ctx->xf.rfc, m, sizeof(m));
  ctx->sp = computeSamplerParams(cam->width, cam->height);
  textureFootprint(*cam, ctx->texFoot);
  ctx->haveCamera = true;
  return DMT_OK;
}

int dmt_set_limits(dmt_ctx* ctx, int max_depth) {
  if (!ctx) return DMT_ERR_INVALID;
  if (max_depth < 0) return fail(ctx, DMT_ERR_INVALID, "dmt_set_limits: max_depth < 0");
  ctx->maxDepth = max_depth;
  return DMT_OK;
}

int dmt_set_accel(dmt_ctx* ctx, int mode) {
  if (!ctx) return DMT_ERR_INVALID;
  if (mode != DMT_ACCEL_BRUTE_FORCE && mode != DMT_ACCEL_BVH) return fail(ctx, DMT_ERR_INVALID, "dmt_set_accel: unknown mode");
  ctx->accel = mode;
  if (mode == DMT_ACCEL_BVH && ctx->haveTris && !ctx->haveBvh) {
    HIP_TRY(ctx, hipSetDevice(ctx->device));
    if (int const rc = buildBvh(ctx)) return rc;
  }
  if (mode == DMT_ACCEL_BVH && ctx->haveMotion) {
    HIP_TRY(ctx, hipSetDevice(ctx->device));
    return ensureMotionTree(ctx);
  }
  return DMT_OK;
}

int dmt_set_accel_build(dmt_ctx* ctx, int mode) {
  if (!ctx) return DMT_ERR_INVALID;
  if (mode != DMT_BVH_BUILD_HOST && mode != DMT_BVH_BUILD_DEVICE) return fail(ctx, DMT_ERR_INVALID, "dmt_set_accel_build: unknown mode");
  if (mode == ctx->accelBuild) return DMT_OK;
  ctx->accelBuild = mode;
  ctx->haveBvh = false;
  if (ctx->accel == DMT_ACCEL_BVH && ctx->haveTris) {
    HIP_TRY(ctx, hipSetDevice(ctx->device));
    HIP_TRY(ctx, hipStreamSynchronize(ctx->stream));
    return buildBvh(ctx);
  }
  return DMT_OK;
}

int dmt_accel_build_info(dmt_ctx* ctx, dmt_accel_build_record* out) {
  if (!ctx || !out) return DMT_ERR_INVALID;
  if (!ctx->haveBvh) {
// ... 930 lines not shown
```

### cuda-optix-pathtracing_amd/csrc/probes.hpp

```cpp
#pragma once

#include "probe_stage.hpp"

namespace {

template <uint32_t F>
__global__ void k_test_trace(RenderParams P, int n, int32_t const* pxs, int32_t const* pys, int32_t const* ss, float* L3) {
  KArgs const k = kargs_base();
  if constexpr (!(F & (kFeatBvh | kFeatMotion))) cull_stage(k);
  int const i = int(blockIdx.x * blockDim.x + threadIdx.x);
  PathState st{};
  if (i < n) {
    ColdArgs const c = load_cold_args(k);
    path_begin(st, c.cam, c.sp, pxs[i], pys[i], halton_pixel_base(c.sp, pxs[i], pys[i]), uint32_t(ss[i]), kargs(k)->lensR, kargs(k)->lensD);
    if constexpr (F & kFeatMotion) motion_set_time(motion_sample_time(k, halton_pixel_base(c.sp, pxs[i], pys[i]), uint32_t(ss[i])));
  }
  auto store = [&](f3 L, uint32_t) { L3[3 * i] = L.x, L3[3 * i + 1] = L.y, L3[3 * i + 2] = L.z; };
  uint32_t const gtid = blockIdx.x * blockDim.x + threadIdx.x;
  while (__any(st.active || st.hasShadow)) lane_step<F>(k, gtid, st, store);
}

__global__ void k_test_texfilter(RenderParams P, int n, int32_t const* tri, float const* bu, float const* bv, int32_t const* tex,
                                 int32_t const* depth, float* rgb3, int32_t* branch, float* lod) {
#pragma clang fp contract(off)
// ... 60 lines not shown
        float* r = rec12 + 12 * n++;
        f3 pos = mk3(0, 0, 0);
        if (bestTri >= 0) pos = shade_hit<MOTION ? kFeatMotion : 0u>(k, sc, bestTri, bu, bv, ray_dir(st)).pos;
        r[0] = float(bestTri), r[1] = pos.x, r[2] = pos.y, r[3] = pos.z;
        r[4] = st.beta.x, r[5] = st.beta.y, r[6] = st.beta.z, r[7] = st.L.x, r[8] = st.L.y, r[9] = st.L.z;
        r[10] = float(st.depth), r[11] = float(st.rng.dim);
      }
      ended = path_shade<MOTION ? kFeatMotion : 0u>(k, st, bestTri, bu, bv);
      if (ended) st.active = false;
    }
    if (ended && !st.hasShadow) break;
  }
  *nOut = n;
  L3[0] = st.L.x, L3[1] = st.L.y, L3[2] = st.L.z;
}
__global__ void k_test_trace_log(RenderParams P, int px, int py, int smp, float* rec12, int cap, int* nOut,
                                 float* L3) {
  test_trace_log_body<false>(px, py, smp, rec12, cap, nOut, L3);
}
__global__ void k_test_trace_log_motion(RenderParams P, int px, int py, int smp, float* rec12, int cap, int* nOut, float* L3) {
  test_trace_log_body<true>(px, py, smp, rec12, cap, nOut, L3);
}

__global__ void k_test_tri(float const* xs, float const* ys, float const* zs, uint32_t n, f3 o, f3 d,
                           int32_t* hit, float* t, float* pos3, float* nrm3, float* err3) {
  uint32_t const i = blockIdx.x * blockDim.x + threadIdx.x;
  if (i >= n) return;
  f3 const p0 = mk3(xs[4 * i], ys[4 * i], zs[4 * i]);
  f3 const p1 = mk3(xs[4 * i + 1], ys[4 * i + 1], zs[4 * i + 1]);
  f3 const p2 = mk3(xs[4 * i + 2], ys[4 * i + 2], zs[4 * i + 2]);
  f3 const e0 = mk3(p1.x - p0.x, p1.y - p0.y, p1.z - p0.z);
  f3 const e1 = mk3(p2.x - p0.x, p2.y - p0.y, p2.z - p0.z);
  Ray const ray{o, d};
  MTResult const r = mt_test(p0, e0, e1, ray);
  hit[i] = r.valid ? 1 : 0;
  float const inf = kInf;
  t[i] = r.valid ? r.t : inf;
  f3 pos = mk3(0, 0, 0), nrm = mk3(0, 0, 0), err = mk3(0, 0, 0);
  if (r.valid) {
    TriPost P;
    P.p0x = p0.x, P.p0y = p0.y, P.p0z = p0.z, P.p1x = p1.x, P.p1y = p1.y, P.p1z = p1.z;
    P.p2x = p2.x, P.p2y = p2.y, P.p2z = p2.z;
    f3 const nn = normalize(cross(e1, e0));
    P.nx = nn.x, P.ny = nn.y, P.nz = nn.z;
    P.matId = 0;
    Hit const h = hit_finish(P, r.u, r.v, mk3(0, 0, 0));
    pos = h.pos, nrm = h.normal, err = h.error;
  }
  pos3[3 * i] = pos.x, pos3[3 * i + 1] = pos.y, pos3[3 * i + 2] = pos.z;
  nrm3[3 * i] = nrm.x, nrm3[3 * i + 1] = nrm.y, nrm3[3 * i + 2] = nrm.z;
  err3[3 * i] = err.x, err3[3 * i + 1] = err.y, err3[3 * i + 2] = err.z;
}

__global__ void k_test_sampler(SamplerParams sp, int n, int32_t const* pxs, int32_t const* pys,
                               int32_t const* ss, int ndims, int32_t* hidx, float* pix2, float* dims) {
  int const i = int(blockIdx.x * blockDim.x + threadIdx.x);
  if (i >= n) return;
  int32_t const h = halton_pixel_base(sp, pxs[i], pys[i]) + ss[i] * (sp.scale0 * sp.scale1);
  hidx[i] = h;
  f2 const p = pixel2d(sp, h);
  pix2[2 * i] = p.x, pix2[2 * i + 1] = p.y;
  Sampler r;
  r.start(uint32_t(h));
  for (int d = 0; d < ndims; ++d) dims[size_t(i) * ndims + d] = r.get1D();
}

__global__ void k_test_camera(CameraXf cam, SamplerParams sp, float lensR, float lensD, int n, int32_t const* pxs,
                              int32_t const* pys, int32_t const* ss, float* o3, float* d3, float* lens2) {
  int const i = int(blockIdx.x * blockDim.x + threadIdx.x);
  if (i >= n) return;
  int32_t const h = halton_pixel_base(sp, pxs[i], pys[i]) + ss[i] * (sp.scale0 * sp.scale1);
  if (lens2) {
    LensU const u = lens_values(uint32_t(h));
    lens2[2 * i] = u.x, lens2[2 * i + 1] = u.y;
    return;
  }
  Ray const r = camera_ray_any(cam, sp, pxs[i], pys[i], h, lensR, lensD);
  o3[3 * i] = r.o.x, o3[3 * i + 1] = r.o.y, o3[3 * i + 2] = r.o.z;
  d3[3 * i] = r.d.x, d3[3 * i + 1] = r.d.y, d3[3 * i + 2] = r.d.z;
}

template <bool kOwnNg>
DMT_DEV void test_bsdf_body(Rec32 rec, int n, float const* ns3, float const* ng3, float const* wo3, float const* u2,
                            float const* uc, float const* wi3, float* prep12, float* samp10, float* eval4) {
  int const i = int(blockIdx.x * blockDim.x + threadIdx.x);
  if (i >= n) return;
  f3 const ns = mk3(ns3[3 * i], ns3[3 * i + 1], ns3[3 * i + 2]);
  f3 const ng = kOwnNg ? mk3(ng3[3 * i], ng3[3 * i + 1], ng3[3 * i + 2]) : ns;
  f3 const wo = mk3(wo3[3 * i], wo3[3 * i + 1], wo3[3 * i + 2]);
  Bsdf const b = bsdf_prepare(rec, ns, wo);
  float* p = prep12 + 12 * size_t(i);
  p[0] = b.weight.x, p[1] = b.weight.y, p[2] = b.weight.z;
  bool const oren = b.type == BS_OREN, ggx = b.type == BS_GGX_DIEL || b.type == BS_GGX_COND;
  p[3] = oren ? b.ms.x : 0.f, p[4] = oren ? b.ms.y : 0.f, p[5] = oren ? b.ms.z : 0.f;
  p[6] = ggx ? b.escale : 0.f, p[7] = float(b.type), p[8] = ggx ? b.ax : 0.f, p[9] = ggx ? b.ay : 0.f, p[10] = ggx ? b.phi0 : 0.f;
  p[11] = b.type == BS_GGX_DIEL ? b.eta : 0.f;
  BsdfSample const s = sample_bsdf(b, wo, ns, ng, mk2(u2[2 * i], u2[2 * i + 1]), uc[i]);
  float* o = samp10 + 10 * size_t(i);
  o[0] = s.wi.x, o[1] = s.wi.y, o[2] = s.wi.z, o[3] = s.f.x, o[4] = s.f.y, o[5] = s.f.z;
  o[6] = s.pdf, o[7] = s.eta, o[8] = s.delta ? 1.f : 0.f, o[9] = s.refract ? 1.f : 0.f;
  float pdf = 0.f;
  f3 const f = eval_bsdf(b, wo, mk3(wi3[3 * i], wi3[3 * i + 1], wi3[3 * i + 2]), ns, ng, pdf) * b.weight;
  float* e = eval4 + 4 * size_t(i);
  e[0] = f.x, e[1] = f.y, e[2] = f.z, e[3] = pdf;
}

__global__ void k_test_bsdf(Rec32 rec, int n, float const* ns3, float const* wo3, float const* u2, float const* uc, float const* wi3,
                            float* prep12, float* samp10, float* eval4) {
  test_bsdf_body<false>(rec, n, ns3, nullptr, wo3, u2, uc, wi3, prep12, samp10, eval4);
}

__global__ void k_test_bsdf_ng(Rec32 rec, int n, float const* ns3, float const* ng3, float const* wo3, float const* u2,
                               float const* uc, float const* wi3, float* prep12, float* samp10, float* eval4) {
  test_bsdf_body<true>(rec, n, ns3, ng3, wo3, u2, uc, wi3, prep12, samp10, eval4);
}

__global__ void k_test_material(RenderParams P, int n, int32_t const* tri, float const* bu, float const* bv, float const* ng3,
                                uint32_t* rec8, float* ns3, uint32_t* rec2_8, float* mixOut) {
  KArgs const k = kargs_base();
  int const i = int(blockIdx.x * blockDim.x + threadIdx.x);
  if (i >= n) return;
  SceneView const sc = load_scene(k);
  uint32_t const matId = sc.post[tri[i]].matId;
  f3 const ng = mk3(ng3[3 * i], ng3[3 * i + 1], ng3[3 * i + 2]);
  Rec32 rec = sc.bsdfs[matId], rec2{};
  float mix = 0.f;
  bool const blend = hi16(rec.w[1]) == BS_GGX_BLEND && matId + 1u < sc.bsdfCount;
  if (blend) {
    mix = blend_metallic<false>(k, rec, matId, tri[i], bu[i], bv[i]);
    rec.w[1] = (rec.w[1] & 0x0000FFFFu) | (uint32_t(BS_GGX_DIEL) << 16);
    rec2 = sc.bsdfs[matId + 1u];
  }
  f3 ns = ng;
  if (kargs(k)->matTex != nullptr) {
    ns = apply_material_textures<false>(k, rec, matId, tri[i], bu[i], bv[i], ng);
    if (blend) (void)apply_material_textures<false>(k, rec2, matId + 1u, tri[i], bu[i], bv[i], ng);
  }
  if (blend) rec.w[1] = (rec.w[1] & 0x0000FFFFu) | (uint32_t(BS_GGX_BLEND) << 16);
  for (int w = 0; w < 8; ++w) rec8[8 * size_t(i) + w] = rec.w[w], rec2_8[8 * size_t(i) + w] = rec2.w[w];
  ns3[3 * i] = ns.x, ns3[3 * i + 1] = ns.y, ns3[3 * i + 2] = ns.z;
  mixOut[i] = mix;
}

__global__ void k_test_light(Rec32 rec, int n, float const* pos3, float const* nrm3, float const* u2,
                             int32_t const* hadT, float* out14) {
  int const i = int(blockIdx.x * blockDim.x + threadIdx.x);
  if (i >= n) return;
  LightSample const s = sample_light(rec, mk3(pos3[3 * i], pos3[3 * i + 1], pos3[3 * i + 2]),
                                     mk2(u2[2 * i], u2[2 * i + 1]), hadT[i] != 0,
                                     mk3(nrm3[3 * i], nrm3[3 * i + 1], nrm3[3 * i + 2]));
  f3 const Le = eval_light(rec, s);
  float* o = out14 + 14 * size_t(i);
  o[0] = s.pLight.x, o[1] = s.pLight.y, o[2] = s.pLight.z;
  o[3] = s.direction.x, o[4] = s.direction.y, o[5] = s.direction.z;
  o[6] = s.pdf, o[7] = float(s.delta), o[8] = s.distance, o[9] = s.factor;
  o[10] = Le.x, o[11] = Le.y, o[12] = Le.z, o[13] = s.valid() ? 1.f : 0.f;
}

__global__ void k_test_half(int n, float const* fin, uint16_t* hout, uint16_t const* hin, float* fout) {
  int const i = int(blockIdx.x * blockDim.x + threadIdx.x);
  if (i >= n) return;
  if (fin && hout) hout[i] = uint16_t(f2h(fin[i]));
  if (hin && fout) fout[i] = h2f(hin[i]);
}

__global__ void k_test_closest(RenderParams P, bool useBvh, int n, float const* o3, float const* d3, int32_t* tri,
                               float* tOut) {
  KArgs const k = kargs_base();
  if (!useBvh) cull_stage(k);
  int const i = int(blockIdx.x * blockDim.x + threadIdx.x);
  bool const alive = i < n;
  PathState st{};
  if (alive)
    set_ray(st, mk3(o3[3 * i], o3[3 * i + 1], o3[3 * i + 2]), mk3(d3[3 * i], d3[3 * i + 1], d3[3 * i + 2]));
  st.active = alive;
  int best;
  float bu, bv, bt = kInf;
  bool occluded;
  if (useBvh)
    trace_pair_bvh(k, st, alive, false, blockIdx.x * blockDim.x + threadIdx.x, best, bu, bv, occluded);
  else
    trace_pair_brute(k, st, alive, false, best, bu, bv, occluded);
  if (alive && best >= 0) {
    TriS const T = load_tri(to_const_as(load_scene(k).tris), uint32_t(best));
    bt = mt_pair(T, st.rp).t.x;
  }
  if (alive) tri[i] = best, tOut[i] = bt;
}

__global__ void k_test_closest_at(RenderParams P, bool useBvh, int n, float const* o3, float const* d3, float const* time, int32_t* tri,
                                  float* tOut, float* uv2) {
  KArgs const k = kargs_base();
  int const i = int(blockIdx.x * blockDim.x + threadIdx.x);
  bool const alive = i < n;
  PathState st{};
  if (alive)
    set_ray(st, mk3(o3[3 * i], o3[3 * i + 1], o3[3 * i + 2]), mk3(d3[3 * i], d3[3 * i + 1], d3[3 * i + 2]));
  st.active = alive;
  float const tm = alive ? time[i] : 0.f;
  int best;
  float bu, bv, bt = kInf;
  bool occluded;
  if (useBvh)
    trace_pair_bvh_motion(k, st, alive, false, v2f{tm, tm}, blockIdx.x * blockDim.x + threadIdx.x, best, bu, bv, occluded, &bt);
  else
    trace_pair_brute_motion(k, st, alive, false, v2f{tm, tm}, best, bu, bv, occluded, &bt);
  if (alive) {
    tri[i] = best, tOut[i] = best >= 0 ? bt : kInf;
    if (uv2) uv2[2 * i] = best >= 0 ? bu : 0.f, uv2[2 * i + 1] = best >= 0 ? bv : 0.f;
  }
}

__global__ void k_test_shutter(SamplerParams sp, float open, float close, int n, int32_t const* pxs, int32_t const* pys, int32_t const* ss,
                               float* t) {
  int const i = int(blockIdx.x * blockDim.x + threadIdx.x);
  if (i >= n) return;
  int32_t const h = halton_pixel_base(sp, pxs[i], pys[i]) + ss[i] * (sp.scale0 * sp.scale1);
  t[i] = shutter_time(uint32_t(h), open, close);
}

__global__ void k_test_project(ProjXf c, int n, float const* p3, float* xy2, float* depth) {
  int const i = int(blockIdx.x * blockDim.x + threadIdx.x);
  if (i >= n) return;
  Proj const o = project_point(c, p3[3 * i], p3[3 * i + 1], p3[3 * i + 2]);
  xy2[2 * i] = o.fx, xy2[2 * i + 1] = o.fy, depth[i] = o.depth;
}

typedef void (*TestTraceFn)(RenderParams, int, int32_t const*, int32_t const*, int32_t const*, float*);
#define DMT_TEST_TRACE_ROW(suffix, mask, waves, body) {mask, k_test_trace<mask>},
KernelRow<TestTraceFn> const kTestTraceKernels[] = {DMT_MEGAKERNELS(DMT_TEST_TRACE_ROW)};

int probeError(dmt_ctx* ctx, Probe const& p) {
  ctx->err = std::string(p.call) + ": " + hipGetErrorName(p.err) + " - " + hipGetErrorString(p.err);
  return DMT_ERR_HIP;
}

int finishProbe(dmt_ctx* ctx, Probe& p) {
  if (int const rc = finishTest(ctx)) return rc;
  return p.fetch() == hipSuccess ? DMT_OK : probeError(ctx, p);
}

int sceneReady(dmt_ctx* ctx, char const* who, bool wholeScene) {
  if (wholeScene && !(ctx->haveTris && ctx->haveBsdfs && ctx->haveLights && ctx->haveCamera))
    return fail(ctx, DMT_ERR_STATE, (std::string(who) + ": scene/camera not set").c_str());
  if (ctx->triCount > 0 && ctx->maxMatId >= ctx->bsdfCount)
    return fail(ctx, DMT_ERR_INVALID, (std::string(who) + ": material index outside the BSDF array").c_str());
  return DMT_OK;
}

int probeBsdf(dmt_ctx* ctx, void const* bsdf32, int n, float const* ns3, float const* ng3, float const* wo3, float const* u2,
              float const* uc, float const* wi_eval3, float* prepared12, float* sample10, float* eval4) {
  if (n == 0) return DMT_OK;
  Probe p(ctx->device, size_t(n));
  ProbeIn<float> dns(p, ns3, 3), dng(p, ng3, 3), dwo(p, wo3, 3), du2(p, u2, 2), duc(p, uc, 1), dwi(p, wi_eval3, 3);
  ProbeOut<float> dp(p, prepared12, 12), ds(p, sample10, 10), de(p, eval4, 4);
  if (p.err != hipSuccess) return probeError(ctx, p);
  Rec32 rec;
  memcpy(&rec, bsdf32, 32);
  if (ng3)
    hipLaunchKernelGGL(k_test_bsdf_ng, dim3(p.blocks(64)), dim3(64), 0, ctx->stream, rec, n, dns.get(), dng.get(), dwo.get(), du2.get(),
                       duc.get(), dwi.get(), dp.get(), ds.get(), de.get());
  else
    hipLaunchKernelGGL(k_test_bsdf, dim3(p.blocks(64)), dim3(64), 0, ctx->stream, rec, n, dns.get(), dwo.get(), du2.get(), duc.get(),
                       dwi.get(), dp.get(), ds.get(), de.get());
  return finishProbe(ctx, p);
}

}

extern "C" {

int dmt_test_envmap(dmt_ctx* ctx, int n, const float* u2, const float* wi_in3, float* wi3, float* pdf, float* uv2, float* Le3,
                    int32_t* ok, float* Le_dir3, float* pdf_dir) {
  if (!ctx || n <= 0 || !u2 || !wi_in3 || !wi3 || !pdf || !uv2 || !Le3 || !ok || !Le_dir3 || !pdf_dir) return DMT_ERR_INVALID;
  if (ctx->env.w <= 0) return fail(ctx, DMT_ERR_STATE, "dmt_test_envmap: no env map uploaded");
  Probe p(ctx->device, size_t(n));
  ProbeIn<float> du(p, u2, 2), dwin(p, wi_in3, 3);
  ProbeOut<float> dwi(p, wi3, 3), dpdf(p, pdf, 1), duv(p, uv2, 2), dLe(p, Le3, 3), dLd(p, Le_dir3, 3), dpd(p, pdf_dir, 1);
  ProbeOut<int32_t> dok(p, ok, 1);
  if (p.err != hipSuccess) return probeError(ctx, p);
  hipLaunchKernelGGL(k_test_envmap, dim3(p.blocks(64)), dim3(64), 0, ctx->stream, ctx->env, n, du.get(), dwin.get(), dwi.get(),
                     dpdf.get(), duv.get(), dLe.get(), dok.get(), dLd.get(), dpd.get());
  return finishProbe(ctx, p);
}

int dmt_test_sampler_table(dmt_ctx* ctx, int width, int height, uint32_t s0, uint32_t n, float* out_vals, float* out_jitter) {
  if (!ctx || width <= 0 || height <= 0 || !out_vals || !out_jitter) return DMT_ERR_INVALID;
  uint32_t const pw = uint32_t(width < 128 ? width : 128), ph = uint32_t(height < 128 ? height : 128);
  SamplerParams const sp = computeSamplerParams(width, height);
  if (uint64_t(n) * pw * ph > 0x7FFFFFFFull || (uint64_t(s0) + n + 1) * uint64_t(sp.scale0) * uint64_t(sp.scale1) > 0x7FFFFFFFull)
    return fail(ctx, DMT_ERR_INVALID, "dmt_test_sampler_table: too many entries, or the sample index overflows the 32-bit Halton index");
  if (n == 0) return DMT_OK;
  Probe p(ctx->device, size_t(n) * pw * ph);
  ProbeOut<float4> dv(p, out_vals, 2);
  ProbeOut<float2> dj(p, out_jitter, 1);
  if (p.err != hipSuccess) return probeError(ctx, p);
  hipLaunchKernelGGL(k_sampler_table, dim3(p.blocks(256)), dim3(256), 0, ctx->stream, sp, s0, n, pw, ph, dv.get(), dj.get(),
                     static_cast<float2*>(nullptr));
  return finishProbe(ctx, p);
}

int dmt_test_triangle_intersect(dmt_ctx* ctx, const float* xs, const float* ys, const float* zs, size_t count, const float* o3,
                                const float* d3, int32_t* hit, float* t, float* pos3, float* nrm3, float* err3) {
  if (!ctx || !xs || !ys || !zs || !o3 || !d3 || !hit) return DMT_ERR_INVALID;
  if (count == 0) return DMT_OK;
  Probe p(ctx->device, count);
  ProbeIn<float> dx(p, xs, 4), dy(p, ys, 4), dz(p, zs, 4);
  ProbeOut<int32_t> dh(p, hit, 1);
  ProbeOut<float> dt(p, t, 1), dp(p, pos3, 3), dn(p, nrm3, 3), de(p, err3, 3);
  if (p.err != hipSuccess) return probeError(ctx, p);
  uint32_t const n = uint32_t(count);
  hipLaunchKernelGGL(k_test_tri, dim3(p.blocks(256)), dim3(256), 0, ctx->stream, dx.get(), dy.get(), dz.get(), n,
                     f3{o3[0], o3[1], o3[2]}, f3{d3[0], d3[1], d3[2]}, dh.get(), dt.get(), dp.get(), dn.get(), de.get());
  return finishProbe(ctx, p);
}

int dmt_test_sampler(dmt_ctx* ctx, int width, int height, int n, const int32_t* pxs, const int32_t* pys, const int32_t* ss,
                     int ndims, int32_t* halton_index, float* pixel2d_out, float* dims) {
  if (!ctx || n < 0 || ndims < 0 || !pxs || !pys || !ss || !halton_index || !pixel2d_out || !dims || width <= 0 || height <= 0)
    return DMT_ERR_INVALID;
  if (n == 0) return DMT_OK;
  Probe p(ctx->device, size_t(n));
  ProbeIn<int32_t> dpx(p, pxs, 1), dpy(p, pys, 1), dss(p, ss, 1);
  ProbeOut<int32_t> dh(p, halton_index, 1);
  ProbeOut<float> dp2(p, pixel2d_out, 2), dd(p, dims, size_t(ndims));
  if (p.err != hipSuccess) return probeError(ctx, p);
  hipLaunchKernelGGL(k_test_sampler, dim3(p.blocks(64)), dim3(64), 0, ctx->stream, computeSamplerParams(width, height), n, dpx.get(),
                     dpy.get(), dss.get(), ndims, dh.get(), dp2.get(), dd.get());
  return finishProbe(ctx, p);
}

int dmt_test_camera_rays(dmt_ctx* ctx, int n, const int32_t* pxs, const int32_t* pys, const int32_t* ss, float* o3, float* d3) {
  if (!ctx || n < 0 || !pxs || !pys || !ss || !o3 || !d3) return DMT_ERR_INVALID;
  if (!ctx->haveCamera) return fail(ctx, DMT_ERR_STATE, "dmt_test_camera_rays: set the camera first");
  if (n == 0) return DMT_OK;
  Probe p(ctx->device, size_t(n));
  ProbeIn<int32_t> dpx(p, pxs, 1), dpy(p, pys, 1), dss(p, ss, 1);
  ProbeOut<float> dO(p, o3, 3), dD(p, d3, 3);
  if (p.err != hipSuccess) return probeError(ctx, p);
  hipLaunchKernelGGL(k_test_camera, dim3(p.blocks(64)), dim3(64), 0, ctx->stream, ctx->xf, ctx->sp, ctx->lensR, ctx->lensD, n, dpx.get(),
                     dpy.get(), dss.get(), dO.get(), dD.get(), static_cast<float*>(nullptr));
  return finishProbe(ctx, p);
}

int dmt_test_lens_values(dmt_ctx* ctx, int n, const int32_t* pxs, const int32_t* pys, const int32_t* ss, float* lens2) {
  if (!ctx || n < 0 || !pxs || !pys || !ss || !lens2) return DMT_ERR_INVALID;
  if (!ctx->haveCamera) return fail(ctx, DMT_ERR_STATE, "dmt_test_lens_values: set the camera first");
  if (n == 0) return DMT_OK;
  Probe p(ctx->device, size_t(n));
  ProbeIn<int32_t> dpx(p, pxs, 1), dpy(p, pys, 1), dss(p, ss, 1);
  ProbeOut<float> dL(p, lens2, 2);
  if (p.err != hipSuccess) return probeError(ctx, p);
  hipLaunchKernelGGL(k_test_camera, dim3(p.blocks(64)), dim3(64), 0, ctx->stream, ctx->xf, ctx->sp, ctx->lensR, ctx->lensD, n, dpx.get(),
                     dpy.get(), dss.get(), static_cast<float*>(nullptr), static_cast<float*>(nullptr), dL.get());
  return finishProbe(ctx, p);
}

int dmt_test_camera_project(dmt_ctx* ctx, int n, const float* p3, float* xy2, float* depth) {
  if (!ctx || n < 0 || !p3 || !xy2 || !depth) return DMT_ERR_INVALID;
  if (!ctx->haveCamera) return fail(ctx, DMT_ERR_STATE, "dmt_test_camera_project: set the camera first");
  if (n == 0) return DMT_OK;
  Probe p(ctx->device, size_t(n));
  ProbeIn<float> dP(p, p3, 3);
  ProbeOut<float> dXy(p, xy2, 2), dD(p, depth, 1);
  if (p.err != hipSuccess) return probeError(ctx, p);
  hipLaunchKernelGGL(k_test_project, dim3(p.blocks(64)), dim3(64), 0, ctx->stream, makeProjXf(ctx->cam), n, dP.get(), dXy.get(), dD.get());
  return finishProbe(ctx, p);
}

int dmt_test_bsdf(dmt_ctx* ctx, const void* bsdf32, int n, const float* ns3, const float* wo3, const float* u2, const float* uc,
                  const float* wi_eval3, float* prepared12, float* sample10, float* eval4) {
  if (!ctx || n < 0 || !bsdf32 || !ns3 || !wo3 || !u2 || !uc || !wi_eval3 || !prepared12 || !sample10 || !eval4) return DMT_ERR_INVALID;
  return probeBsdf(ctx, bsdf32, n, ns3, nullptr, wo3, u2, uc, wi_eval3, prepared12, sample10, eval4);
}

int dmt_test_bsdf_ng(dmt_ctx* ctx, const void* bsdf32, int n, const float* ns3, const float* ng3, const float* wo3, const float* u2,
                     const float* uc, const float* wi_eval3, float* prepared12, float* sample10, float* eval4) {
  if (!ctx || n < 0 || !bsdf32 || !ns3 || !ng3 || !wo3 || !u2 || !uc || !wi_eval3 || !prepared12 || !sample10 || !eval4)
    return DMT_ERR_INVALID;
  return probeBsdf(ctx, bsdf32, n, ns3, ng3, wo3, u2, uc, wi_eval3, prepared12, sample10, eval4);
}

int dmt_test_material(dmt_ctx* ctx, int n, const int32_t* tri, const float* bu, const float* bv, const float* ng3, void* rec32,
                      float* ns3, void* rec2_32, float* mix) {
  if (!ctx || n < 0 || !tri || !bu || !bv || !ng3 || !rec32 || !ns3 || !rec2_32 || !mix) return DMT_ERR_INVALID;
  if (!(ctx->haveTris && ctx->haveBsdfs)) return fail(ctx, DMT_ERR_STATE, "dmt_test_material: triangles and BSDFs first");
  if (int const rc = sceneReady(ctx, "dmt_test_material", false)) return rc;
  if (ctx->texCount > 0 && (ctx->matTexCount != ctx->bsdfCount || ctx->triUvCount != ctx->triCount))
    return fail(ctx, DMT_ERR_STATE, "dmt_test_material: texture tables do not match the uploaded BSDFs / triangles (upload textures last)");
  for (int i = 0; i < n; ++i)
    if (tri[i] < 0 || size_t(tri[i]) >= ctx->triCount) return fail(ctx, DMT_ERR_INVALID, "dmt_test_material: triangle index out of range");
  if (n == 0) return DMT_OK;
  Probe p(ctx->device, size_t(n));
  ProbeIn<int32_t> dTri(p, tri, 1);
  ProbeIn<float> dBu(p, bu, 1), dBv(p, bv, 1), dNg(p, ng3, 3);
  ProbeOut<uint32_t> dRec(p, rec32, 8), dRec2(p, rec2_32, 8);
  ProbeOut<float> dNs(p, ns3, 3), dMix(p, mix, 1);
  if (p.err != hipSuccess) return probeError(ctx, p);
  hipLaunchKernelGGL(k_test_material, dim3(p.blocks(64)), dim3(64), 0, ctx->stream, baseParams(ctx, p.threads(64)), n, dTri.get(),
                     dBu.get(), dBv.get(), dNg.get(), dRec.get(), dNs.get(), dRec2.get(), dMix.get());
  return finishProbe(ctx, p);
}

int dmt_test_light(dmt_ctx* ctx, const void* light32, int n, const float* pos3, const float* nrm3, const float* u2,
                   const int32_t* had_transmission, float* out14) {
  if (!ctx || n < 0 || !light32 || !pos3 || !nrm3 || !u2 || !had_transmission || !out14) return DMT_ERR_INVALID;
  if (n == 0) return DMT_OK;
  Probe p(ctx->device, size_t(n));
  ProbeIn<float> dp(p, pos3, 3), dn(p, nrm3, 3), du(p, u2, 2);
  ProbeIn<int32_t> dh(p, had_transmission, 1);
  ProbeOut<float> dout(p, out14, 14);
  if (p.err != hipSuccess) return probeError(ctx, p);
  Rec32 rec;
  memcpy(&rec, light32, 32);
  hipLaunchKernelGGL(k_test_light, dim3(p.blocks(64)), dim3(64), 0, ctx->stream, rec, n, dp.get(), dn.get(), du.get(), dh.get(),
                     dout.get());
  return finishProbe(ctx, p);
}

int dmt_test_half(dmt_ctx* ctx, int n, const float* f_in, uint16_t* h_out, const uint16_t* h_in, float* f_out) {
  if (!ctx || n < 0) return DMT_ERR_INVALID;
  if (n == 0) return DMT_OK;
  Probe p(ctx->device, size_t(n));
  ProbeIn<float> dfi(p, f_in, 1);
  ProbeOut<uint16_t> dho(p, h_out, f_in && h_out ? 1 : 0);
  ProbeIn<uint16_t> dhi(p, h_in, 1);
  ProbeOut<float> dfo(p, f_out, h_in && f_out ? 1 : 0);
  if (p.err != hipSuccess) return probeError(ctx, p);
  hipLaunchKernelGGL(k_test_half, dim3(p.blocks(256)), dim3(256), 0, ctx->stream, n, dfi.get(), dho.get(), dhi.get(), dfo.get());
  return finishProbe(ctx, p);
}

int dmt_test_trace_samples(dmt_ctx* ctx, int n, const int32_t* pxs, const int32_t* pys, const int32_t* ss, float* L3) {
  if (!ctx || n < 0 || !pxs || !pys || !ss || !L3) return DMT_ERR_INVALID;
  if (int const rc = sceneReady(ctx, "dmt_test_trace_samples", true)) return rc;
  if (n == 0) return DMT_OK;
  Probe p(ctx->device, size_t(n));
  ProbeIn<int32_t> dpx(p, pxs, 1), dpy(p, pys, 1), dss(p, ss, 1);
  ProbeOut<float> dL(p, L3, 3);
  if (p.err != hipSuccess) return probeError(ctx, p);
  uint32_t F = 0;
  if (int const rc = resolveFeatures(ctx, &F)) return rc;
  TestTraceFn const kernel = kernelOf(kTestTraceKernels, F);
  if (!kernel) return noKernel(ctx, "dmt_test_trace_samples", F);
  if (F & kFeatBvh) {
    if (!ctx->haveBvh) return fail(ctx, DMT_ERR_STATE, "dmt_test_trace_samples: BVH not built");
    HIP_TRY(ctx, reserveOverflow(ctx, p.threads(64)));
  }
  RenderParams P = baseParams(ctx, p.threads(64));
  if (int const rc = motionParams(ctx, F, P)) return rc;
  hipLaunchKernelGGL(kernel, dim3(p.blocks(64)), dim3(64), 0, ctx->stream, P, n, dpx.get(), dpy.get(),
                     dss.get(), dL.get());
  return finishProbe(ctx, p);
}

int dmt_test_texture_filter(dmt_ctx* ctx, int n, const int32_t* tri, const float* bu, const float* bv, const int32_t* tex,
                            const int32_t* depth, float* rgb3, int32_t* branch, float* lod) {
  if (!ctx || n < 0 || !tri || !bu || !bv || !tex || !depth || !rgb3 || !branch || !lod) return DMT_ERR_INVALID;
  if (!(ctx->haveTris && ctx->haveCamera) || ctx->texCount == 0 || ctx->triUvCount != ctx->triCount)
    return fail(ctx, DMT_ERR_STATE, "dmt_test_texture_filter: triangles, camera and textures (with one UV triple per triangle) first");
  for (int i = 0; i < n; ++i)
    if (tri[i] < 0 || size_t(tri[i]) >= ctx->triCount || tex[i] < 0 || uint32_t(tex[i]) >= ctx->texCount)
      return fail(ctx, DMT_ERR_INVALID, "dmt_test_texture_filter: triangle or texture index out of range");
  if (n == 0) return DMT_OK;
  Probe p(ctx->device, size_t(n));
  ProbeIn<int32_t> dTri(p, tri, 1), dTex(p, tex, 1), dDepth(p, depth, 1);
  ProbeIn<float> dBu(p, bu, 1), dBv(p, bv, 1);
  ProbeOut<float> dRgb(p, rgb3, 3), dLod(p, lod, 1);
  ProbeOut<int32_t> dBranch(p, branch, 1);
  if (p.err != hipSuccess) return probeError(ctx, p);
  hipLaunchKernelGGL(k_test_texfilter, dim3(p.blocks(64)), dim3(64), 0, ctx->stream, baseParams(ctx, p.threads(64)), n, dTri.get(),
                     dBu.get(), dBv.get(), dTex.get(), dDepth.get(), dRgb.get(), dBranch.get(), dLod.get());
  return finishProbe(ctx, p);
}

int dmt_test_trace_log(dmt_ctx* ctx, int px, int py, int s, float* rec12, int cap, int* n_out, float* L3) {
  if (!ctx || !rec12 || cap <= 0 || !n_out || !L3) return DMT_ERR_INVALID;
  if (int const rc = sceneReady(ctx, "dmt_test_trace_log", true)) return rc;
  Probe p(ctx->device, 1);
  ProbeOut<float> dr(p, rec12, 12 * size_t(cap)), dL(p, L3, 3);
  ProbeOut<int> dn(p, n_out, 1);
  if (p.err != hipSuccess) return probeError(ctx, p);
  RenderParams P = baseParams(ctx, p.threads(64));
  if (int const rc = motionParams(ctx, ctx->haveMotion ? kFeatMotion : 0u, P)) return rc;
  hipLaunchKernelGGL(ctx->haveMotion ? k_test_trace_log_motion : k_test_trace_log, dim3(p.blocks(64)), dim3(64), 0, ctx->stream, P, px, py, s,
                     dr.get(), cap, dn.get(), dL.get());
  return finishProbe(ctx, p);
}

int dmt_test_closest_hit(dmt_ctx* ctx, int nrays, const float* o3, const float* d3, int32_t* tri_index, float* t) {
  if (!ctx || nrays < 0 || !o3 || !d3 || !tri_index || !t) return DMT_ERR_INVALID;
  if (!ctx->haveTris) return fail(ctx, DMT_ERR_STATE, "dmt_test_closest_hit: upload triangles first");
  if (nrays == 0) return DMT_OK;
  Probe p(ctx->device, size_t(nrays));
  ProbeIn<float> dO(p, o3, 3), dD(p, d3, 3);
  ProbeOut<int32_t> di(p, tri_index, 1);
  ProbeOut<float> dt(p, t, 1);
  if (p.err != hipSuccess) return probeError(ctx, p);
  bool const useBvh = ctx->accel == DMT_ACCEL_BVH;
// ... 46 lines not shown
```

### cuda-optix-pathtracing_amd/csrc/pt_device.hpp

```cpp
#pragma once

#include <hip/hip_runtime.h>
#include <stdint.h>

#include "../../include/dmt_ggx_tables.inc"
#include "tri_records.hpp"

#define DMT_DEV __device__ __forceinline__
#define DMT_HD __host__ __device__ __forceinline__

namespace dmt {

struct f2 {
  float x, y;
};
struct f3 {
  float x, y, z;
};
DMT_DEV f3 mk3(float x, float y, float z) { return f3{x, y, z}; }
DMT_DEV f2 mk2(float x, float y) { return f2{x, y}; }
DMT_DEV f3 operator+(f3 a, f3 b) { return mk3(a.x + b.x, a.y + b.y, a.z + b.z); }
DMT_DEV f3 operator-(f3 a, f3 b) { return mk3(a.x - b.x, a.y - b.y, a.z - b.z); }
DMT_DEV f3 operator-(f3 a) { return mk3(-a.x, -a.y, -a.z); }
DMT_DEV f3 operator*(f3 a, f3 b) { return mk3(a.x * b.x, a.y * b.y, a.z * b.z); }
// ... 601 lines not shown
  float const a = 2.f * u.x - 1.f;
  float const b = 2.f * u.y - 1.f;
  if (a == 0.f && b == 0.f) return mk2(0.f, 0.f);
  float rho, phi;
  if (fabsf(a) > fabsf(b)) {
    rho = a;
    phi = (kPi / 4) * (b / a);
  } else {
    rho = b;
    phi = (3 * kPi / 4) * (a / b);
  }
  float sn, cs;
  sincos_bounded(phi, sn, cs);
  return mk2(rho * cs, rho * sn);
}
DMT_DEV f3 sample_cos_hemisphere(f3 n, f2 u, float& pdf) {
  f2 const r = sample_uniform_disk(u);
  float const cosTheta = safe_sqrt(1.f - dot(r, r));
  f3 T, B;
  gram_schmidt(n, T, B);
  pdf = cosTheta * kInvPi;
  return r.x * T + r.y * B + cosTheta * n;
}
DMT_DEV f3 sample_uniform_sphere(f2 rnd) {
  float const z = 1.0f - 2.0f * rnd.x;
  float const r = safe_sqrt(1.f - z * z);
  float const phi = 2 * kPi * rnd.y;
  float sn, cs;
  sincos_bounded(phi, sn, cs);
  return mk3(r * cs, r * sn, z);
}
DMT_DEV f3 sample_uniform_cone(f3 N, float omc, f2 rnd, float& cosTheta, float& pdf, int& delta) {
  if (omc > 0) {
    f2 const xy = sample_uniform_disk(rnd);
    float const r2 = dot(xy, xy);
    cosTheta = 1.0f - r2 * omc;
    float const s = safe_sqrt(r2 * omc * (2.0f - r2 * omc));
    pdf = 0.5f / (kPi * fmaxf(omc, 1e-8f));
    f3 T, B;
    gram_schmidt(N, T, B);
    return s * T + s * B + cosTheta * N;
  }
  delta = 1;
  cosTheta = 1.0f;
  pdf = 1.0f;
  return N;
}
DMT_DEV bool ray_sphere(f3 o, f3 d, float tMin, float tMax, f3 C, float radius, f3& ip, float& it) {
  f3 const dv = C - o;
  float const r_sq = radius * radius;
  float const d_sq = dot(dv, dv);
  float const dcos = dot(dv, d);
  if (d_sq > r_sq && dcos < 0.0f) return false;
  f3 const perp = dv - dcos * d;
  float const dsin_sq = dot(perp, perp);
  if (dsin_sq > r_sq) return false;
  float const t = dcos - copysignf(sqrtf(r_sq - dsin_sq), d_sq - r_sq);
  if (t > tMin && t < tMax) {
    it = t;
    ip = o + d * t;
    return true;
  }
  return false;
}

enum : uint32_t { LT_POINT = 0, LT_SPOT = 1, LT_ENV = 2, LT_DIR = 3 };
struct LightSample {
  f3 pLight, direction;
  float pdf;
  int delta;
  float distance;
  float factor;
  DMT_DEV bool valid() const {
    return direction.x != 0 && direction.y != 0 && direction.z != 0 && pdf != 0;
  }
};
DMT_DEV uint32_t light_type(Rec32 const& L) { return hi16(L.w[1]); }
DMT_DEV f3 light_intensity(Rec32 const& L) {
  return mk3(h2f(lo16(L.w[0])), h2f(hi16(L.w[0])), h2f(lo16(L.w[1])));
}
DMT_DEV f3 light_pos(Rec32 const& L) {
  return mk3(__uint_as_float(L.w[2]), __uint_as_float(L.w[3]), __uint_as_float(L.w[4]));
}
DMT_DEV LightSample sample_point_light(Rec32 const& L, f3 position, f2 u, bool hadT, f3 normal) {
  LightSample s{};
  s.factor = 1.0f;
  float const radius = h2f(lo16(L.w[5]));
  float const radiusSqr = sqr(radius);
  f3 lightN = position - light_pos(L);
  float const distSqr = dot(lightN, lightN);
  float const dist = sqrtf(distSqr);
  lightN = lightN / dist;
  bool const effDelta = (radius / dist) < 1e-3f;
  float cosTheta = 0.f;
  if (distSqr > radiusSqr) {
    float const omc = sin_sqr_to_one_minus_cos(radiusSqr / distSqr);
    s.direction = sample_uniform_cone(-lightN, omc, u, cosTheta, s.pdf, s.delta);
    if (effDelta || s.delta) {
      s.pdf = 1;
      s.delta = 1;
    }
  } else {
    if (hadT) {
      s.direction = sample_uniform_sphere(u);
      s.pdf = 0.25f * kInvPi;
    } else {
      s.direction = sample_cos_hemisphere(normal, u, s.pdf);
    }
    cosTheta = -dot(s.direction, lightN);
  }
  s.distance = dist * cosTheta -
               copysignf(safe_sqrt(radiusSqr - distSqr + distSqr * cosTheta * cosTheta),
                         distSqr - radiusSqr);
  s.pLight = position + s.direction * s.distance;
  return s;
}
DMT_DEV LightSample sample_spot_light(Rec32 const& L, f3 position, f2 u, bool hadT, f3 normal) {
  LightSample s{};
  float const fltMax = 3.402823466e+38f;
  s.distance = fltMax;
  float const radius = h2f(lo16(L.w[7]));
  float const cosThetaE = h2f(hi16(L.w[6]));
  f3 const lpos = light_pos(L);
  float const radiusSqr = radius * radius;
  f3 lightN = position - lpos;
  float const distSqr = dot(lightN, lightN);
  float const dist = sqrtf(distSqr);
  lightN = lightN / dist;
  bool const effDelta = (radius / dist) < 1e-3f;
  bool outside = false;
  float cosTheta = 0.f;
  if (distSqr > radiusSqr) {
    float const omcSpread = 1.f - cosThetaE;
    float const omcHalf = sin_sqr_to_one_minus_cos(radiusSqr / distSqr);
    if (omcHalf < omcSpread) {
      s.direction = sample_uniform_cone(-lightN, omcHalf, u, cosTheta, s.pdf, s.delta);
    } else {
      f3 const spotDir = normalize(dir_from_octa(L.w[5]));
      s.direction = sample_uniform_cone(-spotDir, omcSpread, u, cosTheta, s.pdf, s.delta);
      if (!ray_sphere(position, s.direction, 0.f, fltMax, lpos, radius, s.pLight, s.distance)) {
        outside = true;
        s.pdf = 0;
      }
    }
  } else {
    if (hadT) {
      s.direction = sample_uniform_sphere(u);
      s.pdf = 0.25f * kInvPi;
    } else {
      s.direction = sample_cos_hemisphere(normal, u, s.pdf);
    }
    cosTheta = -dot(s.direction, lightN);
  }
  if (!outside) {
    s.factor = 1.f;
    if (s.distance == fltMax) {
      s.distance = dist * cosTheta *
                   copysignf(safe_sqrt(radiusSqr - distSqr + distSqr * cosTheta * cosTheta),
                             distSqr - radiusSqr);
    }
    if (effDelta) {
      s.pdf = 1.f;
      s.delta = 1;
    }
    s.pLight = position + s.direction * s.distance;
    f3 const ng = normalize(s.pLight - lpos);
    s.pLight = ng * radius + lpos;
    f3 const newDir = s.pLight - position;
    float const distance = sqrtf(newDir.x * newDir.x + newDir.y * newDir.y + newDir.z * newDir.z);
    s.direction = newDir / distance;
    s.distance = distance;
  }
  return s;
}
DMT_DEV LightSample sample_light(Rec32 const& L, f3 position, f2 u, bool hadT, f3 normal) {
  LightSample s{};
  uint32_t const type = light_type(L);
  if (type == LT_SPOT) {
    s = sample_spot_light(L, position, u, hadT, normal);
  } else if (type == LT_POINT) {
    s = sample_point_light(L, position, u, hadT, normal);
  } else if (type == LT_ENV) {
    s.direction = sample_uniform_sphere(u);
    s.pdf = 0.25f * kInvPi;
    s.factor = 1.f;
    s.pLight = s.direction;
    s.distance = 3.402823466e+38f;
  } else if (type == LT_DIR) {
    float unused = 0.f;
    s.pLight = sample_uniform_cone(dir_from_octa(L.w[2]), h2f(lo16(L.w[3])), u, unused, s.pdf,
                                   s.delta);
    s.direction = -s.pLight;
    s.factor = 1.f;
    s.delta = 1;
    s.distance = 3.402823466e+38f;
  }
  return s;
}
DMT_DEV f3 eval_light(Rec32 const& L, LightSample const& ls) {
  f3 Le = light_intensity(L) * ls.factor;
  uint32_t const t = light_type(L);
  if (t == LT_POINT || t == LT_SPOT) Le = Le / (ls.distance * ls.distance);
  return Le;
}

enum : uint32_t { BS_OREN = 0, BS_GGX_DIEL = 1, BS_GGX_COND = 2, BS_LAMBERT = 3,
                  BS_GGX_BLEND = 4 };

__constant__ float c_ggxE[DMT_GGX_E_ROWS * DMT_GGX_E_COLS] = {DMT_GGX_E_TABLE_VALUES};
__constant__ float c_ggxEavg[DMT_GGX_EAVG_COUNT] = {DMT_GGX_EAVG_TABLE_VALUES};

DMT_DEV float table_read(float const* table, float x, int size) {
  x = fminf(fmaxf(x, 0.f), 1.f) * float(size - 1);
  int const index = int(fminf(float(int(x)), float(size - 1)));
  int const nIndex = int(fminf(float(index + 1), float(size - 1)));
  float const t = x - float(index);
  float const d0 = table[index];
  if (t == 0.f) return d0;
  float const d1 = table[nIndex];
  return (1.f - t) * d0 + t * d1;
}
DMT_DEV float table_read_2d(float const* table, float x, float y, int sx, int sy) {
  y = fminf(fmaxf(y, 0.f), 1.f) * float(sy - 1);
  int const index = int(fminf(float(int(y)), float(sy - 1)));
  int const nIndex = int(fminf(float(index + 1), float(sy - 1)));
  float const t = y - float(index);
  float const d0 = table_read(table + sx * index, x, sx);
  if (t == 0.f) return d0;
  float const d1 = table_read(table + sx * nIndex, x, sx);
  return (1.f - t) * d0 + t * d1;
}

struct Bsdf {
  uint32_t type;
  f3 weight;
  union {
    struct {
      float a, b;
      f3 ms;
    };
    struct {
      float escale, ax, ay, phi0, eta;
    };
  };
  bool iso;
  f3 c0, c1;
};

DMT_DEV float fresnel_dielectric(float cosI, float eta, float& cosT_out) {
  cosI = fmaxf(-1.f, fminf(1.f, cosI));
  if (!(cosI > 0.f)) {
    eta = 1.f / eta;
    cosI = fabsf(cosI);
  }
  float const sinI = safe_sqrt(fmaxf(0.f, 1.f - cosI * cosI));
  float const sinT = sinI / eta;
  if (sinT >= 1.f) return 1.f;
  float const cosT = safe_sqrt(fmaxf(0.f, 1.f - sinT * sinT));
  cosT_out = cosT;
  float const rParl = ((eta * cosI) - (cosT)) / ((eta * cosI) + (cosT));
  float const rPerp = ((cosI) - (eta * cosT)) / ((cosI) + (eta * cosT));
  return (rParl * rParl + rPerp * rPerp) * 0.5f;
}
DMT_DEV f3 fresnel_conductor(float cosI, f3 eta, f3 k) {
  cosI = fmaxf(-1.f, fminf(1.f, cosI));
  float const c2 = cosI * cosI;
  float const s2 = 1.f - c2;
  f3 const eta2 = eta * eta;
  f3 const k2 = k * k;
  f3 const t0 = eta2 - k2 - s2;
  f3 const a2b2 = sqrt3(t0 * t0 + 4.f * eta2 * k2);
  f3 const t1 = a2b2 + c2;
  f3 const a = sqrt3(0.5f * (a2b2 + t0));
  f3 const t2 = 2.f * cosI * a;
  f3 const Rs = (t1 - t2) / (t1 + t2);
  f3 const t3 = c2 * a2b2 + s2 * s2;
  f3 const t4 = t2 * s2;
  f3 const Rp = Rs * (t3 - t4) / (t3 + t4);
  return 0.5f * (Rp + Rs);
}
DMT_DEV void microfacet_fresnel(Bsdf const& b, float cos_HO, float& cos_HI, f3& R, f3& T) {
  if (b.type == BS_GGX_DIEL) {
    float const F = fresnel_dielectric(cos_HO, b.eta, cos_HI);
    R = F * b.c0;
    T = (1.f - F) * b.c1;
  } else {
    R = fresnel_conductor(cos_HO, b.c0, b.c1);
    T = mk3(0, 0, 0);
  }
}
DMT_DEV float oren_nayar_G(float cosTheta) {
  float const piOver2 = kPi / 2;
  float const twoThirds = 2.f / 3.f;
  float const piOver2m = piOver2 - twoThirds;
  if (cosTheta < 1e-6f) return piOver2m - cosTheta;
  float const sinTheta = sin_from_cos(cosTheta);
  float const theta = safe_acos(cosTheta);
  return sinTheta * (theta - twoThirds - sinTheta * cosTheta) +
         twoThirds * (sinTheta / cosTheta) * (1.f - sqr(sinTheta) * sinTheta);
}

DMT_DEV Bsdf bsdf_prepare(Rec32 const& r, f3 ns, f3 wo) {
  Bsdf b{};
  b.type = hi16(r.w[1]);
  b.weight = mk3(h2f(lo16(r.w[0])), h2f(hi16(r.w[0])), h2f(lo16(r.w[1])));
  if (b.type == BS_OREN) {
    b.a = h2f(hi16(r.w[5]));
    b.b = h2f(lo16(r.w[6]));
    float const nl = fmaxf(0.f, dot(ns, wo));
    float const Ev = b.a * kPi + b.b * oren_nayar_G(nl);
    f3 ms = b.weight * (1.f - Ev);
    ms = mk3(fmaxf(ms.x, 0.f), fmaxf(ms.y, 0.f), fmaxf(ms.z, 0.f));
    b.ms = q16(ms);
  } else if (b.type == BS_GGX_DIEL || b.type == BS_GGX_COND) {
    b.phi0 = float(lo16(r.w[3])) / 65535 * 2.f * kPi;
    uint32_t const axq = hi16(r.w[3]), ayq = lo16(r.w[4]);
    b.iso = axq == ayq;
    b.ax = float(axq) / 65535;
    b.ay = float(ayq) / 65535;
    f3 Fss;
    if (b.type == BS_GGX_DIEL) {
      b.eta = h2f(hi16(r.w[4]));
      b.c0 = mk3(h2f(lo16(r.w[5])), h2f(hi16(r.w[5])), h2f(lo16(r.w[6])));
      b.c1 = mk3(h2f(hi16(r.w[6])), h2f(lo16(r.w[7])), h2f(hi16(r.w[7])));
      Fss = b.c1;
    } else {
      b.c0 = mk3(h2f(hi16(r.w[4])), h2f(lo16(r.w[5])), h2f(hi16(r.w[5])));
      b.c1 = mk3(h2f(lo16(r.w[6])), h2f(hi16(r.w[6])), h2f(lo16(r.w[7])));
    }
    {
      float const cos_HO = fabsf(dot(wo, ns));
      float unused = 0.f;
      f3 R, T;
      microfacet_fresnel(b, cos_HO, unused, R, T);
      b.weight = q16(R + T);
    }
    if (b.type == BS_GGX_COND) {
      f3 const F0 = fresnel_conductor(1.f, b.c0, b.c1);
      f3 const F82 = fresnel_conductor(1.f / 7.f, b.c0, b.c1);
      f3 const B = (lerp3(F0, mk3(1, 1, 1), 0.46266436f) - F82) * 17.651384f;
      Fss = lerp3(F0, mk3(1, 1, 1), 1.f / 21.f) - B * (1.f / 126.f);
    }
    float const alpha2 = b.ax * b.ay;
    float const cos_NO = fmaxf(0.f, dot(ns, wo));
    float const E = table_read_2d(c_ggxE, alpha2, cos_NO, DMT_GGX_E_COLS, DMT_GGX_E_ROWS);
    float const Eavg = table_read(c_ggxEavg, alpha2, DMT_GGX_EAVG_COUNT);
    float const missing = (1.f - E) / E;
    b.escale = 1.f + missing;
    f3 const Fms = Fss * Eavg / (mk3(1, 1, 1) - Fss * (1.f - Eavg));
    b.weight = q16(b.weight * (1.f + Fms * missing) / b.escale);
  }
  return b;
}

struct BsdfSample {
  f3 wi, f;
  float pdf, eta;
  bool delta, refract;
  DMT_DEV bool valid() const { return wi.x != 0 && wi.y != 0 && wi.z != 0 && pdf != 0.f; }
};

DMT_DEV f3 oren_nayar_intensity(Bsdf const& b, f3 n, f3 v, f3 l) {
  float const nl = fmaxf(dot(n, l), 0.f);
  if (b.b <= 0) {
    float const r = nl * kInvPi;
    return mk3(r, r, r);
  }
  float const nv = fmaxf(dot(n, v), 0.f);
  float t = dot(l, v) - nl * nv;
  if (t > 0.f) t /= fmaxf(nl, nv) + 1.175494351e-38f;
  float const single = b.a + b.b * t;
  float const El = b.a * kPi + b.b * oren_nayar_G(nl);
  f3 const multi = b.ms * (1.f - El);
  return nl * (single + multi);
}
DMT_DEV f3 tangent_from_phi(f3 ns, float phi0) {
  f3 const ref = fabsf(ns.x) < 0.999f ? mk3(1.0f, 0.0f, 0.0f) : mk3(0.0f, 1.0f, 0.0f);
  f3 const t = normalize(cross(ref, ns));
  f3 const bt = cross(ns, t);
  float s, c;
  sincos_bounded(phi0, s, c);
  return c * t + s * bt;
}
DMT_DEV f3 sample_ggx_vndf(f3 wo, f2 u, float ax, float ay) {
  f3 const V = normalize(mk3(ax * wo.x, ay * wo.y, wo.z));
  f3 T1, T2;
  float const lensq = V.x * V.x + V.y * V.y;
  if (lensq > 1e-7f) {
    float const invLen = rsqrt_ieee(lensq);
    T1 = mk3(-V.y * invLen, V.x * invLen, 0.f);
    T2 = cross(V, T1);
  } else {
    T1 = mk3(1, 0, 0);
    T2 = mk3(0, 1, 0);
  }
  f2 t = sample_uniform_disk(u);
  t.y = lerp1(safe_sqrt(1.f - t.x * t.x), t.y, 0.5f * (1.f + V.z));
  f3 Nh = t.x * T1 + t.y * T2 + safe_sqrt(1.f - dot(t, t)) * V;
  Nh = normalize(mk3(ax * Nh.x, ay * Nh.y, fmaxf(0.f, Nh.z)));
  return Nh;
}
DMT_DEV float ggx_lambda_from(float x) { return 0.5f * (sqrtf(1.f + x) - 1.f); }
DMT_DEV float ggx_D(float alpha2, float cos_NH) {
  float const c2 = fminf(cos_NH * cos_NH, 1.f);
  float const omc2 = 1.f - c2;
  return alpha2 / (kPi * sqr(omc2 + alpha2 * c2));
}
DMT_DEV float ggx_lambda(float alpha2, float cos_N) {
  return ggx_lambda_from(alpha2 * fmaxf(0.f, 1.f / sqr(cos_N)));
}
DMT_DEV float ggx_aniso_D(float ax, float ay, f3 lH) {
  lH = lH / mk3(ax, ay, 1.f);
  return kInvPi / ((ax * ay) * sqr(dot(lH, lH)));
}
DMT_DEV float ggx_aniso_lambda(float ax, float ay, f3 V) {
  return ggx_lambda_from((sqr(ax * V.x) + sqr(ay * V.y)) / sqr(V.z));
}
constexpr float kThroughputEps = 1e-6f;

DMT_DEV BsdfSample sample_ggx(Bsdf const& b, f3 wo, f3 ns, f3 ng, f2 u, float uc) {
  BsdfSample s{};
  float const cos_NO = dot(ns, wo);
  s.eta = 1.f;
  float invEta = 1.f;
  s.delta = fmaxf(b.ax, b.ay) < 1e-3f;
  f3 H = ns, lH = mk3(0, 0, 0), lO = mk3(0, 0, 0);
  if (!s.delta) {
    f3 X, Y;
    if (b.iso)
      gram_schmidt(ns, X, Y);
    else
      orthonormal_tangent(ns, tangent_from_phi(ns, b.phi0), X, Y);
    lO = mk3(dot(X, wo), dot(Y, wo), cos_NO);
    lH = sample_ggx_vndf(lO, u, b.ax, b.ay);
    H = lH.x * X + lH.y * Y + lH.z * ns;
  }
  float const cos_HO = dot(H, wo);
  float cos_HI = 0.f;
  f3 R, T;
  microfacet_fresnel(b, cos_HO, cos_HI, R, T);
  if (near_zero_pos(R, kThroughputEps) && near_zero_pos(T, kThroughputEps)) return s;
  float const pdfReflect = fminf(fmaxf(average(R) / average(R + T), 0.f), 1.f);
  s.refract = uc > pdfReflect;
  if (s.refract) invEta = 1.f / b.eta;
  s.wi = s.refract ? (invEta * dot(H, wo) + cos_HI) * H - invEta * wo : 2.f * cos_HO * H - wo;
  if (dot(ng, s.wi) <= 0 && !s.refract) {
    s.pdf = 0;
    return s;
  }
  if (s.refract) {
    s.f = T;
    s.pdf = 1.f - pdfReflect;
    s.delta = s.delta || (fabsf(s.eta - 1.f) < 1e-4f);
  } else {
    s.pdf = pdfReflect;
  }
  if (s.delta) {
    s.pdf *= 1e6f;
    s.f = s.f * 1e6f;
  } else {
    float D, lamI, lamO;
    if (b.iso || s.refract) {
      float const alpha2 = b.ax * b.ay;
      D = ggx_D(alpha2, lH.z);
      lamI = ggx_lambda(alpha2, dot(ns, s.wi));
      lamO = ggx_lambda(alpha2, cos_NO);
    } else {
      f3 const lI = 2.f * cos_HO * lH - lO;
      D = ggx_aniso_D(b.ax, b.ay, lH);
      lamI = ggx_aniso_lambda(b.ax, b.ay, lI);
      lamO = ggx_aniso_lambda(b.ax, b.ay, lO);
    }
    float const common =
        D / cos_NO * (s.refract ? fabsf(cos_HO * cos_HI) / sqr(cos_HI + cos_HO * invEta) : 0.25f);
    s.pdf *= common / (1.f + lamO);
    s.f = s.f * (common / (1.f + lamO + lamI));
  }
  return s;
}
DMT_DEV f3 eval_ggx(Bsdf const& b, f3 wo, f3 wi, f3 ns, f3 ng, float& pdf) {
  bool const conductor = b.type == BS_GGX_COND;
  bool const hasReflection = conductor ? true : luminance(b.c0) > kThroughputEps;
  bool const hasTransmission = conductor ? false : luminance(b.c1) > kThroughputEps;
  bool const isotropic = b.ax == b.ay;
  float const cos_NO = dot(ns, wo);
  float const cos_NI = dot(ns, wi);
  float const cos_NgI = dot(ng, wi);
  bool const isT = cos_NI < 0.f;
  float const ior = isT ? b.eta : 1.f;
  bool const effSpecular = fmaxf(b.ax, b.ay) < 1e-3f;
  if (cos_NO <= 0.f || (cos_NgI < 0) != isT || effSpecular || (!hasReflection && cos_NgI > 0.f) ||
      (!hasTransmission && cos_NgI < 0.f)) {
    pdf = 0.f;
    return mk3(0, 0, 0);
  }
  f3 H = isT ? (ior * wi + wo) : (wi + wo);
  float const invLen_H = rsqrt_ieee(dot(H, H));
  H = H * invLen_H;
  float const cos_HO = dot(H, wo);
  float unused = 0.f;
  f3 R, T;
  microfacet_fresnel(b, cos_HO, unused, R, T);
  if (near_zero_pos(R, kThroughputEps) && near_zero_pos(T, kThroughputEps)) {
    pdf = 0.f;
    return mk3(0, 0, 0);
  }
  float const cos_NH = dot(ns, H);
  float D, lamI, lamO;
  if (isotropic || isT) {
    float const alpha2 = b.ax * b.ay;
    D = ggx_D(alpha2, cos_NH);
    lamI = ggx_lambda(alpha2, cos_NI);
    lamO = ggx_lambda(alpha2, cos_NO);
  } else {
    f3 X, Y;
    orthonormal_tangent(ns, tangent_from_phi(ns, b.phi0), X, Y);
    f3 const lH = mk3(dot(X, H), dot(Y, H), dot(ns, H));
    f3 const lO = mk3(dot(X, wo), dot(Y, wo), cos_NO);
    f3 const lI = mk3(dot(X, wi), dot(Y, wi), cos_NI);
    D = ggx_aniso_D(b.ax, b.ay, lH);
    lamI = ggx_aniso_lambda(b.ax, b.ay, lI);
    lamO = ggx_aniso_lambda(b.ax, b.ay, lO);
  }
  float const common = D / cos_NO * (isT ? sqr(ior * invLen_H) * fabsf(cos_HO * dot(H, wi)) : 0.25f);
  float const pdfReflect = average(R) / average(R + T);
  float const lobePdf = isT ? 1.f - pdfReflect : pdfReflect;
  pdf = lobePdf * common / (1.f + lamO);
  return b.escale * (isT ? T : R) * common / (1.f + lamO + lamI);
}

DMT_DEV BsdfSample sample_bsdf(Bsdf const& b, f3 wo, f3 ns, f3 ng, f2 u, float uc) {
  BsdfSample s{};
  if (dot(wo, ng) > 0.0f) {
    if (dot(ns, ng) < 0.0f) ns = -ns;
    if (b.type == BS_OREN || b.type == BS_LAMBERT) {
      s.eta = 1.f;
      s.wi = sample_cos_hemisphere(ns, u, s.pdf);
      if (dot(ng, s.wi) > 0.f) {
        s.f = b.type == BS_OREN ? oren_nayar_intensity(b, ns, wo, s.wi) : mk3(s.pdf, s.pdf, s.pdf);
      } else {
        s.pdf = 0;
      }
    } else {
      s = sample_ggx(b, wo, ns, ng, u, uc);
    }
  }
  return s;
}
DMT_DEV f3 eval_bsdf(Bsdf const& b, f3 wo, f3 wi, f3 ns, f3 ng, float& pdf) {
  pdf = 0;
  if (b.type == BS_OREN) {
    float const cos_NI = dot(ns, wi);
    if (cos_NI > 0.f) {
      pdf = cos_NI * kInvPi;
      return oren_nayar_intensity(b, ns, wo, wi);
    }
    return mk3(0, 0, 0);
  }
  if (b.type == BS_LAMBERT) {
    float const cos_NI = fmaxf(dot(ns, wi), 0.f);
    pdf = cos_NI * kInvPi;
    return mk3(pdf, pdf, pdf);
  }
  return eval_ggx(b, wo, wi, ns, ng, pdf);
}

DMT_DEV uint32_t pick_index(float u, uint32_t count) {
  uint32_t const a = uint32_t(int(u * float(count)));
  uint32_t const b = count - 1u;
  return a < b ? a : b;
}

}
```

### include/dmt_hip.h

```cpp
#ifndef DMT_HIP_H
#define DMT_HIP_H

#include <stddef.h>
#include <stdint.h>

#ifdef __cplusplus
extern "C" {
#endif

typedef struct dmt_ctx dmt_ctx;

typedef struct dmt_camera {
  float dir[3];
  float pos[3];
  int32_t width;
  int32_t height;
  int32_t spp;
  float focal_length;
  float sensor_size;
} dmt_camera;

enum {
  DMT_OK = 0,
  DMT_ERR_INVALID = 1,
  DMT_ERR_HIP = 2,
  DMT_ERR_STATE = 3,
  DMT_ERR_NO_DEVICE = 4,
};

enum {
  DMT_ACCEL_BRUTE_FORCE = 0,
  DMT_ACCEL_BVH = 1,
};

int dmt_ctx_create(int device_ordinal, dmt_ctx** out);
int dmt_ctx_destroy(dmt_ctx* ctx);
const char* dmt_last_error(const dmt_ctx* ctx);

int dmt_upload_triangles(dmt_ctx* ctx, const float* xs, const float* ys, const float* zs,
                         const uint32_t* mat_id, size_t count);
int dmt_upload_bsdfs(dmt_ctx* ctx, const void* bsdf32, uint32_t count);
int dmt_upload_lights(dmt_ctx* ctx, const void* lights32, uint32_t count, const void* infinite32,
                      uint32_t infinite_count);
int dmt_set_camera(dmt_ctx* ctx, const dmt_camera* cam);

int dmt_set_lens(dmt_ctx* ctx, float lens_radius, float focus_distance);
int dmt_lens_info(dmt_ctx* ctx, float* lens_radius, float* focus_distance);
int dmt_lens_rays(const dmt_camera* cam, float lens_radius, float focus_distance, int n, const int32_t* pxs, const int32_t* pys,
                  const int32_t* ss, float* o3, float* d3, float* lens2);
int dmt_focus_distance_at(dmt_ctx* ctx, float fx, float fy, float* distance);

int dmt_set_motion(dmt_ctx* ctx, const float* xs1, const float* ys1, const float* zs1, size_t count);
int dmt_clear_motion(dmt_ctx* ctx);
int dmt_set_shutter(dmt_ctx* ctx, float open, float close);
int dmt_motion_info(dmt_ctx* ctx, int* keys, float* open, float* close, uint32_t* tree_nodes, uint32_t* tree_pairs, double* tree_build_ms);
int dmt_shutter_times(int width, int height, float open, float close, int n, const int32_t* pxs, const int32_t* pys, const int32_t* ss,
                      float* t);
int dmt_motion_positions(const float* xs0, const float* ys0, const float* zs0, const float* xs1, const float* ys1, const float* zs1,
                         size_t count, float t, float* xs, float* ys, float* zs);
int dmt_motion_bvh_validate(const float* xs0, const float* ys0, const float* zs0, const float* xs1, const float* ys1, const float* zs1,
                            size_t count, int* node_count, int* pair_count, int* depth);
int dmt_set_limits(dmt_ctx* ctx, int max_depth);
int dmt_set_accel(dmt_ctx* ctx, int mode);
#define DMT_LIGHTS_UNIFORM 0
#define DMT_LIGHTS_TREE 1
#define DMT_LIGHTS_TREE_REFERENCE 2
int dmt_set_light_sampling(dmt_ctx* ctx, int mode);
int dmt_light_tree_ref_select(const void* lights32, uint32_t count, int n, const float* p3, const float* n3, const float* u, float start_pmf,
                              int32_t* indices4, float* pmfs4, int32_t* counts, int* node_count, int* depth);
int dmt_light_tree_pmfs(const void* lights32, uint32_t count, const float* p3, const float* n3, float* pmf_out, int* node_count,
                        int* depth);
int dmt_set_bvh_strategy(dmt_ctx* ctx, int strategy, uint64_t paths_per_pass);
int dmt_set_partition(dmt_ctx* ctx, int rank, int world);
int dmt_upload_area_lights(dmt_ctx* ctx, const uint32_t* triangle_index, const float* radiance_rgb, uint32_t count);
int dmt_upload_envmap(dmt_ctx* ctx, const float* rgb, int width, int height, const float* quat_xyzw, float scale);
int dmt_clear_envmap(dmt_ctx* ctx);
int dmt_upload_textures(dmt_ctx* ctx, const uint8_t* rgba8, uint64_t texel_count, const int32_t* desc3, uint32_t texture_count,
                        const uint32_t* mat_tex4, uint32_t bsdf_count, const float* tri_uv6, uint64_t triangle_count);
enum {
  DMT_TEXFILTER_LEVEL0 = 0,
  DMT_TEXFILTER_REFERENCE = 1,
};
int dmt_set_texture_filter(dmt_ctx* ctx, int mode);
int dmt_texture_mip_chain(const uint8_t* rgba8, int width, int height, uint8_t* out, uint64_t out_texels, int* levels);
int dmt_texture_footprint(const dmt_camera* cam, float* out);
int dmt_test_texture_filter(dmt_ctx* ctx, int n, const int32_t* tri, const float* bu, const float* bv, const int32_t* tex,
                            const int32_t* depth, float* rgb3, int32_t* branch, float* lod);
int dmt_envmap_tables(const float* rgb, int width, int height, float* func, float* cdf, float* row_integral,
                      float* marginal_func, float* marginal_cdf, float* marginal_integral);
int dmt_test_envmap(dmt_ctx* ctx, int n, const float* u2, const float* wi_in3, float* wi3, float* pdf, float* uv2,
                    float* Le3, int32_t* ok, float* Le_dir3, float* pdf_dir);
int dmt_set_chunk(dmt_ctx* ctx, uint32_t samples_per_item);
#define DMT_SAMPLER_TABLE_OFF 0
#define DMT_SAMPLER_TABLE_AUTO 1
#define DMT_SAMPLER_TABLE_FORCE 2
int dmt_set_sampler_table(dmt_ctx* ctx, int mode, uint64_t budget_bytes);
typedef struct dmt_sampler_table_plan_record {
  uint32_t use;
  uint32_t period_width, period_height;
  uint32_t entry_bytes;
  uint32_t slices;
  uint32_t reserved;
  uint64_t slice_bytes;
} dmt_sampler_table_plan_record;
int dmt_sampler_table_plan(int width, int height, uint64_t owned_pixels, uint32_t spp, uint32_t chunk_spp, uint64_t budget_bytes,
                           int mode, dmt_sampler_table_plan_record* out, uint32_t* slice_spp, uint32_t slice_cap);
int dmt_set_stream(dmt_ctx* ctx, void* hip_stream);

int dmt_film_clear(dmt_ctx* ctx);
int dmt_film_bind(dmt_ctx* ctx, void* d_mean, void* d_m2);
int dmt_film_device_ptrs(dmt_ctx* ctx, void** d_mean, void** d_m2);
int dmt_download_film(dmt_ctx* ctx, float* mean4, float* m24);

int dmt_render(dmt_ctx* ctx, uint32_t sample_offset, uint32_t spp, int x0, int y0, int x1, int y1);
int dmt_render_adaptive(dmt_ctx* ctx, uint32_t min_spp, uint32_t max_spp, uint32_t step_spp, float threshold,
                        int x0, int y0, int x1, int y1, uint32_t* rounds, uint64_t* samples);
int dmt_render_stats(dmt_ctx* ctx, uint32_t sample_offset, uint32_t spp, int x0, int y0, int x1, int y1,
                     uint64_t* stats6);
int dmt_render_profile(dmt_ctx* ctx, uint32_t sample_offset, uint32_t spp, int x0, int y0, int x1, int y1,
                       uint64_t* stats16);
int dmt_sync(dmt_ctx* ctx);
int dmt_sched_diag(dmt_ctx* ctx, uint64_t* out8, int reset);
int dmt_kernel_time(dmt_ctx* ctx, double* total_ms, uint64_t* launches, int reset);
int dmt_kernel_info(dmt_ctx* ctx, int* vgprs, int* sgprs, int* lds_bytes, int* blocks_per_cu,
                    int* cu_count);

int dmt_bvh_validate(const float* xs, const float* ys, const float* zs, size_t count, int* node_count,
                     int* depth, int* max_leaf);

enum {
  DMT_BVH_BUILD_HOST = 0,
  DMT_BVH_BUILD_DEVICE = 1,
};
enum {
  DMT_BVH_BUILT_BY_HOST = 0,
  DMT_BVH_BUILT_BY_DEVICE = 1,
  DMT_BVH_BUILT_BY_HOST_AFTER_DEVICE = 2,
};
int dmt_set_accel_build(dmt_ctx* ctx, int mode);
typedef struct dmt_accel_build_record {
  int32_t builder;
  int32_t depth;
  uint32_t triangles;
  uint32_t nodes;
  uint32_t pairs;
  uint32_t reserved;
  double build_ms;
  uint64_t temp_bytes;
} dmt_accel_build_record;
int dmt_accel_build_info(dmt_ctx* ctx, dmt_accel_build_record* out);
int dmt_accel_download(dmt_ctx* ctx, void* nodes64, size_t node_cap, uint32_t* pair_orig2, size_t pair_cap);
int dmt_lbvh_reference(const float* xs, const float* ys, const float* zs, size_t count, int max_depth, void* nodes64,
                       size_t node_cap, uint32_t* pair_orig2, size_t pair_cap, uint32_t* node_count, uint32_t* pair_count,
                       int* depth, int* abandoned);
int dmt_bvh_check(const void* nodes64, size_t node_count, const uint32_t* pair_orig2, size_t pair_count, const float* xs,
                  const float* ys, const float* zs, size_t count, int* depth, int* max_leaf, double* sah_cost);

int dmt_update_vertices(dmt_ctx* ctx, const float* xs, const float* ys, const float* zs, size_t count);
int dmt_update_vertices_device(dmt_ctx* ctx, const void* d_verts9, size_t count);
enum {
  DMT_BVH_UPDATE_REBUILD = 0,
  DMT_BVH_UPDATE_REFIT = 1,
  DMT_BVH_UPDATE_AUTO = 2,
};
int dmt_set_accel_update(dmt_ctx* ctx, int mode, double max_cost_ratio);
enum {
  DMT_BVH_UPDATED_NONE = 0,
  DMT_BVH_UPDATED_REFIT = 1,
  DMT_BVH_UPDATED_REBUILD = 2,
  DMT_BVH_UPDATED_REBUILD_AFTER_REFIT = 3,
};
typedef struct dmt_accel_update_record {
  int32_t action;
  uint32_t updates_since_build;
  double update_ms;
  double sah_cost;
  double sah_cost_at_build;
  uint64_t temp_bytes;
} dmt_accel_update_record;
int dmt_accel_update_info(dmt_ctx* ctx, dmt_accel_update_record* out);
int dmt_bvh_refit_reference(const void* nodes64, size_t node_count, const uint32_t* pair_orig2, size_t pair_count,
                            const float* xs, const float* ys, const float* zs, size_t count, void* nodes64_out);

int dmt_brute_cull_plan(const float* xs, const float* ys, const float* zs, const uint32_t* mat_id, size_t count,
                        int enable, uint32_t* cluster_count, uint32_t* cluster_first_count, float* cluster_sphere);

int dmt_brute_cull_box_plan(const float* xs, const float* ys, const float* zs, const uint32_t* mat_id, size_t count,
                            int enable, uint32_t* cluster_count, uint32_t* cluster_first_count, float* cluster_box);

int dmt_render_aovs(dmt_ctx* ctx, uint32_t aov_spp);
int dmt_upload_aovs(dmt_ctx* ctx, const float* albedo4, const float* normal4, const float* position4, int width, int height);
int dmt_download_aovs(dmt_ctx* ctx, float* albedo4, float* normal4, float* position4);
typedef struct dmt_denoise_params {
  int32_t iterations;
  float sigma_normal;
  float sigma_position;
  float sigma_albedo;
  float sigma_luminance;
} dmt_denoise_params;
dmt_denoise_params dmt_denoise_defaults(void);
int dmt_denoise(dmt_ctx* ctx, const dmt_denoise_params* params, const float* mean4, const float* m24, float* out4, float* kernel_ms);

int dmt_download_aov_surface(dmt_ctx* ctx, float* surface4);
int dmt_upload_aov_surface(dmt_ctx* ctx, const float* surface4, int width, int height);
int dmt_camera_project(const dmt_camera* cam, int n, const float* p3, float* xy2, float* depth);
typedef struct dmt_temporal_params {
  float alpha;
  float normal_threshold;
  float plane_threshold;
} dmt_temporal_params;
dmt_temporal_params dmt_temporal_defaults(void);
int dmt_denoise_temporal(dmt_ctx* ctx, const dmt_denoise_params* params, const dmt_temporal_params* tparams, const float* mean4,
                         const float* m24, float* out4, float* kernel_ms);
int dmt_temporal_reset(dmt_ctx* ctx);
typedef struct dmt_temporal_record {
  uint32_t frames;
  uint32_t reprojected;
  uint32_t reset;
  float temporal_ms;
  uint64_t history_bytes;
} dmt_temporal_record;
int dmt_temporal_info(dmt_ctx* ctx, dmt_temporal_record* out);
int dmt_temporal_download(dmt_ctx* ctx, float* color_var4, float* length1);

int dmt_test_triangle_intersect(dmt_ctx* ctx, const float* xs, const float* ys, const float* zs,
                                size_t count, const float* o3, const float* d3, int32_t* hit,
                                float* t, float* pos3, float* nrm3, float* err3);
int dmt_test_sampler(dmt_ctx* ctx, int width, int height, int n, const int32_t* pxs,
                     const int32_t* pys, const int32_t* ss, int ndims, int32_t* halton_index,
                     float* pixel2d, float* dims);
int dmt_test_sampler_table(dmt_ctx* ctx, int width, int height, uint32_t s0, uint32_t n, float* out_vals, float* out_jitter);
int dmt_test_camera_rays(dmt_ctx* ctx, int n, const int32_t* pxs, const int32_t* pys,
                         const int32_t* ss, float* o3, float* d3);
int dmt_test_lens_values(dmt_ctx* ctx, int n, const int32_t* pxs, const int32_t* pys, const int32_t* ss, float* lens2);
int dmt_test_shutter_times(dmt_ctx* ctx, int n, const int32_t* pxs, const int32_t* pys, const int32_t* ss, float* t);
int dmt_test_closest_hit_at(dmt_ctx* ctx, int nrays, const float* o3, const float* d3, const float* time, int32_t* tri_index, float* t,
                            float* uv2);
int dmt_test_camera_project(dmt_ctx* ctx, int n, const float* p3, float* xy2, float* depth);
int dmt_test_bsdf(dmt_ctx* ctx, const void* bsdf32, int n, const float* ns3, const float* wo3,
                  const float* u2, const float* uc, const float* wi_eval3, float* prepared12,
                  float* sample10, float* eval4);
int dmt_test_bsdf_ng(dmt_ctx* ctx, const void* bsdf32, int n, const float* ns3, const float* ng3, const float* wo3,
                     const float* u2, const float* uc, const float* wi_eval3, float* prepared12, float* sample10,
                     float* eval4);
int dmt_test_material(dmt_ctx* ctx, int n, const int32_t* tri, const float* bu, const float* bv, const float* ng3, void* rec32,
                      float* ns3, void* rec2_32, float* mix);
int dmt_test_light(dmt_ctx* ctx, const void* light32, int n, const float* pos3, const float* nrm3,
                   const float* u2, const int32_t* had_transmission, float* out14);
int dmt_test_half(dmt_ctx* ctx, int n, const float* f_in, uint16_t* h_out, const uint16_t* h_in,
                  float* f_out);
int dmt_test_trace_samples(dmt_ctx* ctx, int n, const int32_t* pxs, const int32_t* pys,
                           const int32_t* ss, float* L3);
int dmt_test_trace_log(dmt_ctx* ctx, int px, int py, int s, float* rec12, int cap, int* n_out,
                       float* L3);
int dmt_test_closest_hit(dmt_ctx* ctx, int nrays, const float* o3, const float* d3,
                         int32_t* tri_index, float* t);

#ifdef __cplusplus
}
#endif
#endif
```

Measured before the change: 5779.

## Pre-decode BSDF and light records into float constant structs at upload

Adds a decode kernel that runs at upload time and expands packed half-precision BSDF and light records into full-float structs. These structs also carry precomputed Fss, Eavg, table column indices, sin/cos of phi and reflection/transmission flags. The megakernel reads these structs instead of decoding the packed records per hit, for feature sets without textures, blending or the reference light tree. This removes per-hit half-to-float conversion, conductor Fresnel and table lookups, but records get larger, so each hit makes wider global loads and some late reloads, and register pressure may change.

Result: no change. 5790 (median of 6 runs) (+0.2%).

```diff
diff --git a/cuda-optix-pathtracing_amd/binding.py b/cuda-optix-pathtracing_amd/binding.py
--- a/cuda-optix-pathtracing_amd/binding.py
+++ b/cuda-optix-pathtracing_amd/binding.py
@@ -74,6 +74,7 @@
     "dmt_set_lens", "dmt_lens_info", "dmt_lens_rays", "dmt_focus_distance_at", "dmt_test_lens_values",
     "dmt_set_motion", "dmt_clear_motion", "dmt_set_shutter", "dmt_motion_info", "dmt_shutter_times", "dmt_motion_positions",
     "dmt_motion_bvh_validate", "dmt_test_shutter_times", "dmt_test_closest_hit_at",
+    "dmt_set_shade_constants", "dmt_test_bsdf_decoded", "dmt_test_light_decoded",
 ]
 
 SAMPLER_TABLE_OFF = 0
@@ -580,6 +581,9 @@
 
     def set_sampler_table(self, mode, budget_bytes=0):
         self._check(self._lib.dmt_set_sampler_table(self._ctx, int(mode), C.c_uint64(int(budget_bytes))), "dmt_set_sampler_table")
+
+    def set_shade_constants(self, on):
+        self._check(self._lib.dmt_set_shade_constants(self._ctx, 1 if on else 0), "dmt_set_shade_constants")
 
     def set_stream(self, stream_ptr):
         self._check(self._lib.dmt_set_stream(self._ctx, C.c_void_p(stream_ptr)), "dmt_set_stream")
@@ -813,6 +817,19 @@
                                                _p(prep), _p(samp), _p(ev)), "dmt_test_bsdf_ng")
         return prep, samp, ev
 
+    def test_bsdf_decoded(self, bsdf32, ns, ng, wo, u2, uc, wi_eval):
+        b = np.ascontiguousarray(bsdf32, np.uint8).reshape(32)
+        ns, ng, wo, wi_eval = _f32(ns, (-1, 3)), _f32(ng, (-1, 3)), _f32(wo, (-1, 3)), _f32(wi_eval, (-1, 3))
+        u2, uc = _f32(u2, (-1, 2)), _f32(uc, (-1,))
+        n = ns.shape[0]
+        assert ng.shape[0] == n and wo.shape[0] == n and wi_eval.shape[0] == n and u2.shape[0] == n and uc.shape[0] == n
+        prep = np.zeros((n, 12), np.float32)
+        samp = np.zeros((n, 10), np.float32)
+        ev = np.zeros((n, 4), np.float32)
+        self._check(self._lib.dmt_test_bsdf_decoded(self._ctx, _p(b), n, _p(ns), _p(ng), _p(wo), _p(u2), _p(uc), _p(wi_eval),
+                                                    _p(prep), _p(samp), _p(ev)), "dmt_test_bsdf_decoded")
+        return prep, samp, ev
+
     def test_material(self, tri, bu, bv, ng):
         tri, bu, bv, ng = _i32(tri), _f32(bu, (-1,)), _f32(bv, (-1,)), _f32(ng, (-1, 3))
         n = tri.shape[0]
@@ -832,6 +849,16 @@
         out = np.zeros((n, 14), np.float32)
         self._check(self._lib.dmt_test_light(self._ctx, _p(l), n, _p(pos), _p(nrm), _p(u2), _p(ht), _p(out)),
                     "dmt_test_light")
+        return out
+
+    def test_light_decoded(self, light32, pos, nrm, u2, had_t):
+        l = np.ascontiguousarray(light32, np.uint8).reshape(32)
+        pos, nrm, u2 = _f32(pos, (-1, 3)), _f32(nrm, (-1, 3)), _f32(u2, (-1, 2))
+        ht = _i32(had_t)
+        n = pos.shape[0]
+        out = np.zeros((n, 14), np.float32)
+        self._check(self._lib.dmt_test_light_decoded(self._ctx, _p(l), n, _p(pos), _p(nrm), _p(u2), _p(ht), _p(out)),
+                    "dmt_test_light_decoded")
         return out
 
     def test_half(self, floats=None, halves=None):
diff --git a/cuda-optix-pathtracing_amd/csrc/dmt_hip.hip b/cuda-optix-pathtracing_amd/csrc/dmt_hip.hip
--- a/cuda-optix-pathtracing_amd/csrc/dmt_hip.hip
+++ b/cuda-optix-pathtracing_amd/csrc/dmt_hip.hip
@@ -98,6 +98,8 @@
   uint32_t const* texMip;
   int32_t const* texMipDesc;
   MotionView motion;
+  BsdfConst const* bsdfConst;
+  LightConst const* lightConst;
 };
 
 typedef RenderParams const DMT_CONST_AS* KArgs;
@@ -695,7 +697,9 @@
   if (st.depth >= maxDepth) return true;
 
   f3 const wo = -rd;
-  Rec32 rec = sc.bsdfs[hit.matId];
+  constexpr bool kDecoded = (F & (kFeatTex | kFeatBlend | kFeatLightTreeRef)) == 0;
+  Rec32 rec{};
+  if constexpr (!kDecoded) rec = sc.bsdfs[hit.matId];
   f3 ns = hit.normal;
   Rec32 rec2{};
   float mix = 0.f;
@@ -722,7 +726,7 @@
   }
 #if DMT_SECTION_TIMING
   {
-    bool const ggx = hi16(rec.w[1]) != BS_OREN;
+    bool const ggx = hi16(sc.bsdfs[hit.matId].w[1]) != BS_OREN;
     unsigned long long const all = __ballot(1), mg = __ballot(ggx);
     if (int(__ffsll((long long)all)) - 1 == int(threadIdx.x & 63u)) {
       unsigned long long* const acc = s_sectAcc[threadIdx.x >> 6];
@@ -730,14 +734,24 @@
     }
   }
 #endif
-  Bsdf const b = bsdf_prepare(rec, ns, wo);
+  Bsdf b;
+  if constexpr (kDecoded) {
+    if (BsdfConst const* const bc = kargs(k)->bsdfConst) b = bsdf_prepare(bc[hit.matId], ns, wo);
+    else b = bsdf_prepare(sc.bsdfs[hit.matId], ns, wo);
+  } else {
+    b = bsdf_prepare(rec, ns, wo);
+  }
+  auto late = [&]() {
+    if constexpr (kDecoded) return BsdfLate{kargs(k)->bsdfConst, hit.matId};
+    else return BsdfLate{nullptr, 0u};
+  };
   Bsdf b2{};
   if constexpr (F & kFeatBlend) {
     if (blend) b2 = bsdf_prepare(rec2, ns, wo);
   }
   auto blend_pdf = [&](float pdfD, float pdfC) { return (1.f - pdfD) * pdfC + pdfD * mix; };
   auto eval_material = [&](f3 wi, float& pdf) {
-    f3 f = eval_bsdf(b, wo, wi, ns, hit.normal, pdf) * b.weight;
+    f3 f = eval_bsdf(b, wo, wi, ns, hit.normal, pdf, late()) * b.weight;
     if constexpr (F & kFeatBlend) {
       if (blend) {
         float pdfC = 0.f;
@@ -858,14 +872,17 @@
       li = pick_index(uLight, (F & kFeatArea) ? nAll : sc.lightCount);
       pmf = ((F & kFeatEnv) ? 0.5f : 1.f) / float((F & kFeatArea) ? nAll : sc.lightCount);
     }
-    Rec32 const light = sc.lights[li];
-    LightSample const ls = sample_light(light, hit.pos, uLight2, st.lastT, hit.normal);
+    LightConst const* lc = nullptr;
+    if constexpr (kDecoded) lc = kargs(k)->lightConst;
+    LightSample const ls = lc ? sample_light(lc[li], hit.pos, uLight2, st.lastT, hit.normal)
+                              : sample_light(sc.lights[li], hit.pos, uLight2, st.lastT, hit.normal);
     sect_mark(6);
     if (picked && ls.valid()) {
       float bsdfPdf = 0.f;
       f3 const f = eval_material(ls.direction, bsdfPdf);
       if (!is_zero(f)) {
-        f3 const Le = eval_light(light, ls);
+        if constexpr (kDecoded) lc = kargs(k)->lightConst;
+        f3 const Le = lc ? eval_light(lc[li], ls) : eval_light(sc.lights[li], ls);
         if (ls.delta) {
           put_C(st.beta * Le * f / pmf);
         } else {
@@ -882,7 +899,7 @@
   sect_mark(7);
   f2 const u2 = st.rng.get2D();
   float const uc = st.rng.get1D();
-  BsdfSample bs = sample_bsdf(b, wo, ns, hit.normal, u2, uc);
+  BsdfSample bs = sample_bsdf(b, wo, ns, hit.normal, u2, uc, late());
   if constexpr (F & kFeatBlend) {
     if (blend) {
       BsdfSample sC = sample_bsdf(b2, wo, ns, hit.normal, u2, uc);
@@ -1869,6 +1886,13 @@
 DMT_MEGAKERNELS(DMT_DEFINE_MEGAKERNEL)
 DMT_STATS_MEGAKERNELS(DMT_DEFINE_MEGAKERNEL)
 
+__global__ void __launch_bounds__(64) k_decode_records(Rec32 const* bsdfs, uint32_t nBsdfs, BsdfConst* bsdfOut, Rec32 const* lights,
+                                                       uint32_t nLights, LightConst* lightOut) {
+  uint32_t const i = blockIdx.x * 64u + threadIdx.x;
+  if (i < nBsdfs) bsdfOut[i] = bsdf_decode(bsdfs[i]);
+  if (i < nLights) lightOut[i] = light_decode(lights[i]);
+}
+
 __global__ void __launch_bounds__(256) k_sampler_table(SamplerParams sp, uint32_t s0, uint32_t n, uint32_t pw, uint32_t ph,
                                                        float4* vals, float2* jit, float2* lens) {
   uint32_t const e = blockIdx.x * 256u + threadIdx.x;
@@ -1972,6 +1996,9 @@
   DevBuf<TriIsect> d_tris;
   DevBuf<TriPost> d_post;
   DevBuf<Rec32> d_bsdfs, d_lights, d_inf;
+  DevBuf<BsdfConst> d_bsdfConst;
+  DevBuf<LightConst> d_lightConst;
+  bool shadeConstants = true;
   uint32_t triCount = 0, bsdfCount = 0, lightCount = 0, infCount = 0;
   uint32_t maxMatId = 0;
   int bruteCull = 2;
@@ -2440,6 +2467,7 @@
     memcpy(P.texMinDy, c->texFoot + 15, 3 * sizeof(float));
     P.texSppScale = c->texFoot[18];
   }
+  if (c->shadeConstants) P.bsdfConst = c->d_bsdfConst.get(), P.lightConst = c->d_lightConst.get();
   uint32_t const F = featuresOf(c);
   if ((F & kFeatLightTree) && c->lightTreeValid) P.lightTree = c->d_lightTree.get();
   if ((F & kFeatLightTreeRef) && c->lightTreeValid) P.lightTreeRef = c->d_lightTreeRef.get();
@@ -2872,6 +2900,7 @@
     int const v = std::atoi(e7);
     ctx->samTabMode = v == 0 ? DMT_SAMPLER_TABLE_OFF : v == 2 ? DMT_SAMPLER_TABLE_FORCE : DMT_SAMPLER_TABLE_AUTO;
   }
+  if (char const* e8 = std::getenv("DMT_SHADE_CONSTANTS")) ctx->shadeConstants = std::atoi(e8) != 0;
   if (char const* e2 = std::getenv("DMT_SUB_SHIFT")) {
     int const v = std::atoi(e2);
     ctx->subShift = v < 0 ? -1 : (v > 2 ? 2 : v);
@@ -3017,12 +3046,31 @@
   return DMT_OK;
 }
 
+namespace {
+int decodeRecords(dmt_ctx* ctx, uint32_t nBsdfs, uint32_t nLights) {
+  uint32_t const n = nBsdfs > nLights ? nBsdfs : nLights;
+  if (n == 0) return DMT_OK;
+  hipLaunchKernelGGL(k_decode_records, dim3((n + 63u) / 64u), dim3(64), 0, ctx->stream, ctx->d_bsdfs.get(), nBsdfs, ctx->d_bsdfConst.get(),
+                     ctx->d_lights.get(), nLights, ctx->d_lightConst.get());
+  HIP_TRY(ctx, hipGetLastError());
+  return DMT_OK;
+}
+}
+
+int dmt_set_shade_constants(dmt_ctx* ctx, int on) {
+  if (!ctx) return DMT_ERR_INVALID;
+  ctx->shadeConstants = on != 0;
+  return DMT_OK;
+}
+
 int dmt_upload_bsdfs(dmt_ctx* ctx, const void* bsdf32, uint32_t count) {
   if (!ctx) return DMT_ERR_INVALID;
   if (count && !bsdf32) return fail(ctx, DMT_ERR_INVALID, "dmt_upload_bsdfs: null array");
   HIP_TRY(ctx, hipSetDevice(ctx->device));
   DevBuf<Rec32> bsdfs;
+  DevBuf<BsdfConst> decoded;
   HIP_TRY(ctx, bsdfs.assign(bsdf32, count));
+  HIP_TRY(ctx, decoded.reserve(count ? count : 1));
   bool blend = false;
   for (uint32_t i = 0; i < count; ++i) {
     uint32_t w1;
@@ -3035,11 +3083,11 @@
       blend = true;
     }
   }
-  ctx->d_bsdfs = std::move(bsdfs);
+  ctx->d_bsdfs = std::move(bsdfs), ctx->d_bsdfConst = std::move(decoded);
   ctx->hasBlend = blend;
   ctx->bsdfCount = count;
   ctx->haveBsdfs = true;
-  return DMT_OK;
+  return decodeRecords(ctx, count, 0);
 }
 
 int dmt_upload_lights(dmt_ctx* ctx, const void* lights32, uint32_t count, const void* infinite32,
@@ -3049,9 +3097,12 @@
     return fail(ctx, DMT_ERR_INVALID, "dmt_upload_lights: null array");
   HIP_TRY(ctx, hipSetDevice(ctx->device));
   DevBuf<Rec32> lights, inf;
+  DevBuf<LightConst> decoded;
   HIP_TRY(ctx, lights.assign(lights32, count));
   HIP_TRY(ctx, inf.assign(infinite32, infinite_count));
-  ctx->d_lights = std::move(lights), ctx->d_inf = std::move(inf);
+  HIP_TRY(ctx, decoded.reserve(count ? count : 1));
+  ctx->d_lights = std::move(lights), ctx->d_inf = std::move(inf), ctx->d_lightConst = std::move(decoded);
+  if (int const rcD = decodeRecords(ctx, 0, count)) return rcD;
   ctx->lightCount = count;
   ctx->infCount = infinite_count;
   ctx->haveLights = true;
diff --git a/cuda-optix-pathtracing_amd/csrc/probes.hpp b/cuda-optix-pathtracing_amd/csrc/probes.hpp
--- a/cuda-optix-pathtracing_amd/csrc/probes.hpp
+++ b/cuda-optix-pathtracing_amd/csrc/probes.hpp
@@ -166,25 +166,27 @@
 
 template <bool kOwnNg>
 DMT_DEV void test_bsdf_body(Rec32 rec, int n, float const* ns3, float const* ng3, float const* wo3, float const* u2,
-                            float const* uc, float const* wi3, float* prep12, float* samp10, float* eval4) {
+                            float const* uc, float const* wi3, float* prep12, float* samp10, float* eval4,
+                            BsdfConst const* bc = nullptr) {
   int const i = int(blockIdx.x * blockDim.x + threadIdx.x);
   if (i >= n) return;
   f3 const ns = mk3(ns3[3 * i], ns3[3 * i + 1], ns3[3 * i + 2]);
   f3 const ng = kOwnNg ? mk3(ng3[3 * i], ng3[3 * i + 1], ng3[3 * i + 2]) : ns;
   f3 const wo = mk3(wo3[3 * i], wo3[3 * i + 1], wo3[3 * i + 2]);
-  Bsdf const b = bsdf_prepare(rec, ns, wo);
+  Bsdf const b = bc ? bsdf_prepare(bc[0], ns, wo) : bsdf_prepare(rec, ns, wo);
+  BsdfLate const late{bc, 0u};
   float* p = prep12 + 12 * size_t(i);
   p[0] = b.weight.x, p[1] = b.weight.y, p[2] = b.weight.z;
   bool const oren = b.type == BS_OREN, ggx = b.type == BS_GGX_DIEL || b.type == BS_GGX_COND;
   p[3] = oren ? b.ms.x : 0.f, p[4] = oren ? b.ms.y : 0.f, p[5] = oren ? b.ms.z : 0.f;
   p[6] = ggx ? b.escale : 0.f, p[7] = float(b.type), p[8] = ggx ? b.ax : 0.f, p[9] = ggx ? b.ay : 0.f, p[10] = ggx ? b.phi0 : 0.f;
   p[11] = b.type == BS_GGX_DIEL ? b.eta : 0.f;
-  BsdfSample const s = sample_bsdf(b, wo, ns, ng, mk2(u2[2 * i], u2[2 * i + 1]), uc[i]);
+  BsdfSample const s = sample_bsdf(b, wo, ns, ng, mk2(u2[2 * i], u2[2 * i + 1]), uc[i], late);
   float* o = samp10 + 10 * size_t(i);
   o[0] = s.wi.x, o[1] = s.wi.y, o[2] = s.wi.z, o[3] = s.f.x, o[4] = s.f.y, o[5] = s.f.z;
   o[6] = s.pdf, o[7] = s.eta, o[8] = s.delta ? 1.f : 0.f, o[9] = s.refract ? 1.f : 0.f;
   float pdf = 0.f;
-  f3 const f = eval_bsdf(b, wo, mk3(wi3[3 * i], wi3[3 * i + 1], wi3[3 * i + 2]), ns, ng, pdf) * b.weight;
+  f3 const f = eval_bsdf(b, wo, mk3(wi3[3 * i], wi3[3 * i + 1], wi3[3 * i + 2]), ns, ng, pdf, late) * b.weight;
   float* e = eval4 + 4 * size_t(i);
   e[0] = f.x, e[1] = f.y, e[2] = f.z, e[3] = pdf;
 }
@@ -197,6 +199,11 @@
 __global__ void k_test_bsdf_ng(Rec32 rec, int n, float const* ns3, float const* ng3, float const* wo3, float const* u2,
                                float const* uc, float const* wi3, float* prep12, float* samp10, float* eval4) {
   test_bsdf_body<true>(rec, n, ns3, ng3, wo3, u2, uc, wi3, prep12, samp10, eval4);
+}
+
+__global__ void k_test_bsdf_decoded(BsdfConst const* bc, int n, float const* ns3, float const* ng3, float const* wo3, float const* u2,
+                                    float const* uc, float const* wi3, float* prep12, float* samp10, float* eval4) {
+  test_bsdf_body<true>(Rec32{}, n, ns3, ng3, wo3, u2, uc, wi3, prep12, samp10, eval4, bc);
 }
 
 __global__ void k_test_material(RenderParams P, int n, int32_t const* tri, float const* bu, float const* bv, float const* ng3,
@@ -226,8 +233,9 @@
   mixOut[i] = mix;
 }
 
-__global__ void k_test_light(Rec32 rec, int n, float const* pos3, float const* nrm3, float const* u2,
-                             int32_t const* hadT, float* out14) {
+template <class Light>
+DMT_DEV void test_light_body(Light const& rec, int n, float const* pos3, float const* nrm3, float const* u2, int32_t const* hadT,
+                             float* out14) {
   int const i = int(blockIdx.x * blockDim.x + threadIdx.x);
   if (i >= n) return;
   LightSample const s = sample_light(rec, mk3(pos3[3 * i], pos3[3 * i + 1], pos3[3 * i + 2]),
@@ -239,6 +247,14 @@
   o[3] = s.direction.x, o[4] = s.direction.y, o[5] = s.direction.z;
   o[6] = s.pdf, o[7] = float(s.delta), o[8] = s.distance, o[9] = s.factor;
   o[10] = Le.x, o[11] = Le.y, o[12] = Le.z, o[13] = s.valid() ? 1.f : 0.f;
+}
+__global__ void k_test_light(Rec32 rec, int n, float const* pos3, float const* nrm3, float const* u2,
+                             int32_t const* hadT, float* out14) {
+  test_light_body(rec, n, pos3, nrm3, u2, hadT, out14);
+}
+__global__ void k_test_light_decoded(LightConst const* lc, int n, float const* pos3, float const* nrm3, float const* u2,
+                                     int32_t const* hadT, float* out14) {
+  test_light_body(lc[0], n, pos3, nrm3, u2, hadT, out14);
 }
 
 __global__ void k_test_half(int n, float const* fin, uint16_t* hout, uint16_t const* hin, float* fout) {
@@ -333,7 +349,7 @@
 }
 
 int probeBsdf(dmt_ctx* ctx, void const* bsdf32, int n, float const* ns3, float const* ng3, float const* wo3, float const* u2,
-              float const* uc, float const* wi_eval3, float* prepared12, float* sample10, float* eval4) {
+              float const* uc, float const* wi_eval3, float* prepared12, float* sample10, float* eval4, bool decoded = false) {
   if (n == 0) return DMT_OK;
   Probe p(ctx->device, size_t(n));
   ProbeIn<float> dns(p, ns3, 3), dng(p, ng3, 3), dwo(p, wo3, 3), du2(p, u2, 2), duc(p, uc, 1), dwi(p, wi_eval3, 3);
@@ -341,7 +357,15 @@
   if (p.err != hipSuccess) return probeError(ctx, p);
   Rec32 rec;
   memcpy(&rec, bsdf32, 32);
-  if (ng3)
+  DevBuf<Rec32> drec;
+  DevBuf<BsdfConst> dconst;
+  if (decoded) {
+    if ((p.err = drec.assign(&rec, 1)) != hipSuccess || (p.err = dconst.reserve(1)) != hipSuccess) return probeError(ctx, p);
+    hipLaunchKernelGGL(k_decode_records, dim3(1), dim3(64), 0, ctx->stream, drec.get(), 1u, dconst.get(), static_cast<Rec32 const*>(nullptr), 0u,
+                       static_cast<LightConst*>(nullptr));
+    hipLaunchKernelGGL(k_test_bsdf_decoded, dim3(p.blocks(64)), dim3(64), 0, ctx->stream, dconst.get(), n, dns.get(), dng.get(), dwo.get(),
+                       du2.get(), duc.get(), dwi.get(), dp.get(), ds.get(), de.get());
+  } else if (ng3)
     hipLaunchKernelGGL(k_test_bsdf_ng, dim3(p.blocks(64)), dim3(64), 0, ctx->stream, rec, n, dns.get(), dng.get(), dwo.get(), du2.get(),
                        duc.get(), dwi.get(), dp.get(), ds.get(), de.get());
   else
@@ -463,6 +487,13 @@
   if (!ctx || n < 0 || !bsdf32 || !ns3 || !ng3 || !wo3 || !u2 || !uc || !wi_eval3 || !prepared12 || !sample10 || !eval4)
     return DMT_ERR_INVALID;
   return probeBsdf(ctx, bsdf32, n, ns3, ng3, wo3, u2, uc, wi_eval3, prepared12, sample10, eval4);
+}
+
+int dmt_test_bsdf_decoded(dmt_ctx* ctx, const void* bsdf32, int n, const float* ns3, const float* ng3, const float* wo3, const float* u2,
+                          const float* uc, const float* wi_eval3, float* prepared12, float* sample10, float* eval4) {
+  if (!ctx || n < 0 || !bsdf32 || !ns3 || !ng3 || !wo3 || !u2 || !uc || !wi_eval3 || !prepared12 || !sample10 || !eval4)
+    return DMT_ERR_INVALID;
+  return probeBsdf(ctx, bsdf32, n, ns3, ng3, wo3, u2, uc, wi_eval3, prepared12, sample10, eval4, true);
 }
 
 int dmt_test_material(dmt_ctx* ctx, int n, const int32_t* tri, const float* bu, const float* bv, const float* ng3, void* rec32,
@@ -499,6 +530,25 @@
   memcpy(&rec, light32, 32);
   hipLaunchKernelGGL(k_test_light, dim3(p.blocks(64)), dim3(64), 0, ctx->stream, rec, n, dp.get(), dn.get(), du.get(), dh.get(),
                      dout.get());
+  return finishProbe(ctx, p);
+}
+
+int dmt_test_light_decoded(dmt_ctx* ctx, const void* light32, int n, const float* pos3, const float* nrm3, const float* u2,
+                           const int32_t* had_transmission, float* out14) {
+  if (!ctx || n < 0 || !light32 || !pos3 || !nrm3 || !u2 || !had_transmission || !out14) return DMT_ERR_INVALID;
+  if (n == 0) return DMT_OK;
+  Probe p(ctx->device, size_t(n));
+  ProbeIn<float> dp(p, pos3, 3), dn(p, nrm3, 3), du(p, u2, 2);
+  ProbeIn<int32_t> dh(p, had_transmission, 1);
+  ProbeOut<float> dout(p, out14, 14);
+  if (p.err != hipSuccess) return probeError(ctx, p);
+  DevBuf<Rec32> drec;
+  DevBuf<LightConst> dconst;
+  if ((p.err = drec.assign(light32, 1)) != hipSuccess || (p.err = dconst.reserve(1)) != hipSuccess) return probeError(ctx, p);
+  hipLaunchKernelGGL(k_decode_records, dim3(1), dim3(64), 0, ctx->stream, static_cast<Rec32 const*>(nullptr), 0u,
+                     static_cast<BsdfConst*>(nullptr), drec.get(), 1u, dconst.get());
+  hipLaunchKernelGGL(k_test_light_decoded, dim3(p.blocks(64)), dim3(64), 0, ctx->stream, dconst.get(), n, dp.get(), dn.get(), du.get(),
+                     dh.get(), dout.get());
   return finishProbe(ctx, p);
 }
 
diff --git a/cuda-optix-pathtracing_amd/csrc/pt_device.hpp b/cuda-optix-pathtracing_amd/csrc/pt_device.hpp
--- a/cuda-optix-pathtracing_amd/csrc/pt_device.hpp
+++ b/cuda-optix-pathtracing_amd/csrc/pt_device.hpp
@@ -707,12 +707,46 @@
 DMT_DEV f3 light_pos(Rec32 const& L) {
   return mk3(__uint_as_float(L.w[2]), __uint_as_float(L.w[3]), __uint_as_float(L.w[4]));
 }
-DMT_DEV LightSample sample_point_light(Rec32 const& L, f3 position, f2 u, bool hadT, f3 normal) {
+struct LightConst {
+  uint32_t type;
+  f3 intensity;
+  f3 pos;
+  float radius;
+  float radiusSqr;
+  float cosThetaE;
+  float omcSpread;
+  f3 dir;
+  float omcAngle;
+  uint32_t pad;
+};
+static_assert(sizeof(LightConst) == 64, "LightConst: 64 bytes");
+DMT_DEV LightConst light_decode(Rec32 const& L) {
+  LightConst c{};
+  c.type = light_type(L);
+  c.intensity = light_intensity(L);
+  if (c.type == LT_SPOT) {
+    c.radius = h2f(lo16(L.w[7]));
+    c.cosThetaE = h2f(hi16(L.w[6]));
+    c.pos = light_pos(L);
+    c.radiusSqr = c.radius * c.radius;
+    c.omcSpread = 1.f - c.cosThetaE;
+    c.dir = normalize(dir_from_octa(L.w[5]));
+  } else if (c.type == LT_POINT) {
+    c.radius = h2f(lo16(L.w[5]));
+    c.radiusSqr = sqr(c.radius);
+    c.pos = light_pos(L);
+  } else if (c.type == LT_DIR) {
+    c.dir = dir_from_octa(L.w[2]);
+    c.omcAngle = h2f(lo16(L.w[3]));
+  }
+  return c;
+}
+DMT_DEV LightSample sample_point_light(LightConst const& L, f3 position, f2 u, bool hadT, f3 normal) {
   LightSample s{};
   s.factor = 1.0f;
-  float const radius = h2f(lo16(L.w[5]));
-  float const radiusSqr = sqr(radius);
-  f3 lightN = position - light_pos(L);
+  float const radius = L.radius;
+  float const radiusSqr = L.radiusSqr;
+  f3 lightN = position - L.pos;
   float const distSqr = dot(lightN, lightN);
   float const dist = sqrtf(distSqr);
   lightN = lightN / dist;
@@ -740,14 +774,13 @@
   s.pLight = position + s.direction * s.distance;
   return s;
 }
-DMT_DEV LightSample sample_spot_light(Rec32 const& L, f3 position, f2 u, bool hadT, f3 normal) {
+DMT_DEV LightSample sample_spot_light(LightConst const& L, f3 position, f2 u, bool hadT, f3 normal) {
   LightSample s{};
   float const fltMax = 3.402823466e+38f;
   s.distance = fltMax;
-  float const radius = h2f(lo16(L.w[7]));
-  float const cosThetaE = h2f(hi16(L.w[6]));
-  f3 const lpos = light_pos(L);
-  float const radiusSqr = radius * radius;
+  float const radius = L.radius;
+  f3 const lpos = L.pos;
+  float const radiusSqr = L.radiusSqr;
   f3 lightN = position - lpos;
   float const distSqr = dot(lightN, lightN);
   float const dist = sqrtf(distSqr);
@@ -756,12 +789,12 @@
   bool outside = false;
   float cosTheta = 0.f;
   if (distSqr > radiusSqr) {
-    float const omcSpread = 1.f - cosThetaE;
+    float const omcSpread = L.omcSpread;
     float const omcHalf = sin_sqr_to_one_minus_cos(radiusSqr / distSqr);
     if (omcHalf < omcSpread) {
       s.direction = sample_uniform_cone(-lightN, omcHalf, u, cosTheta, s.pdf, s.delta);
     } else {
-      f3 const spotDir = normalize(dir_from_octa(L.w[5]));
+      f3 const spotDir = L.dir;
       s.direction = sample_uniform_cone(-spotDir, omcSpread, u, cosTheta, s.pdf, s.delta);
       if (!ray_sphere(position, s.direction, 0.f, fltMax, lpos, radius, s.pLight, s.distance)) {
         outside = true;
@@ -798,9 +831,9 @@
   }
   return s;
 }
-DMT_DEV LightSample sample_light(Rec32 const& L, f3 position, f2 u, bool hadT, f3 normal) {
+DMT_DEV LightSample sample_light(LightConst const& L, f3 position, f2 u, bool hadT, f3 normal) {
   LightSample s{};
-  uint32_t const type = light_type(L);
+  uint32_t const type = L.type;
   if (type == LT_SPOT) {
     s = sample_spot_light(L, position, u, hadT, normal);
   } else if (type == LT_POINT) {
@@ -813,8 +846,7 @@
     s.distance = 3.402823466e+38f;
   } else if (type == LT_DIR) {
     float unused = 0.f;
-    s.pLight = sample_uniform_cone(dir_from_octa(L.w[2]), h2f(lo16(L.w[3])), u, unused, s.pdf,
-                                   s.delta);
+    s.pLight = sample_uniform_cone(L.dir, L.omcAngle, u, unused, s.pdf, s.delta);
     s.direction = -s.pLight;
     s.factor = 1.f;
     s.delta = 1;
@@ -822,12 +854,21 @@
   }
   return s;
 }
-DMT_DEV f3 eval_light(Rec32 const& L, LightSample const& ls) {
-  f3 Le = light_intensity(L) * ls.factor;
-  uint32_t const t = light_type(L);
+DMT_DEV LightSample sample_light(Rec32 const& L, f3 position, f2 u, bool hadT, f3 normal) {
+  return sample_light(light_decode(L), position, u, hadT, normal);
+}
+DMT_DEV f3 eval_light(LightConst const& L, LightSample const& ls) {
+  f3 Le = L.intensity * ls.factor;
+  uint32_t const t = L.type;
   if (t == LT_POINT || t == LT_SPOT) Le = Le / (ls.distance * ls.distance);
   return Le;
 }
+DMT_DEV f3 eval_light(Rec32 const& L, LightSample const& ls) {
+  LightConst c{};
+  c.type = light_type(L);
+  c.intensity = light_intensity(L);
+  return eval_light(c, ls);
+}
 
 enum : uint32_t { BS_OREN = 0, BS_GGX_DIEL = 1, BS_GGX_COND = 2, BS_LAMBERT = 3,
                   BS_GGX_BLEND = 4 };
@@ -835,26 +876,40 @@
 __constant__ float c_ggxE[DMT_GGX_E_ROWS * DMT_GGX_E_COLS] = {DMT_GGX_E_TABLE_VALUES};
 __constant__ float c_ggxEavg[DMT_GGX_EAVG_COUNT] = {DMT_GGX_EAVG_TABLE_VALUES};
 
-DMT_DEV float table_read(float const* table, float x, int size) {
+struct TableCol {
+  int index, nIndex;
+  float t;
+};
+DMT_DEV TableCol table_col(float x, int size) {
   x = fminf(fmaxf(x, 0.f), 1.f) * float(size - 1);
-  int const index = int(fminf(float(int(x)), float(size - 1)));
-  int const nIndex = int(fminf(float(index + 1), float(size - 1)));
-  float const t = x - float(index);
-  float const d0 = table[index];
-  if (t == 0.f) return d0;
-  float const d1 = table[nIndex];
-  return (1.f - t) * d0 + t * d1;
-}
-DMT_DEV float table_read_2d(float const* table, float x, float y, int sx, int sy) {
+  TableCol c;
+  c.index = int(fminf(float(int(x)), float(size - 1)));
+  c.nIndex = int(fminf(float(c.index + 1), float(size - 1)));
+  c.t = x - float(c.index);
+  return c;
+}
+DMT_DEV float table_read_at(float const* table, TableCol c) {
+  float const d0 = table[c.index];
+  if (c.t == 0.f) return d0;
+  float const d1 = table[c.nIndex];
+  return (1.f - c.t) * d0 + c.t * d1;
+}
+DMT_DEV float table_read(float const* table, float x, int size) { return table_read_at(table, table_col(x, size)); }
+DMT_DEV float table_read_2d_at(float const* table, TableCol cx, float y, int sx, int sy) {
   y = fminf(fmaxf(y, 0.f), 1.f) * float(sy - 1);
   int const index = int(fminf(float(int(y)), float(sy - 1)));
   int const nIndex = int(fminf(float(index + 1), float(sy - 1)));
   float const t = y - float(index);
-  float const d0 = table_read(table + sx * index, x, sx);
+  float const d0 = table_read_at(table + sx * index, cx);
   if (t == 0.f) return d0;
-  float const d1 = table_read(table + sx * nIndex, x, sx);
+  float const d1 = table_read_at(table + sx * nIndex, cx);
   return (1.f - t) * d0 + t * d1;
 }
+DMT_DEV float table_read_2d(float const* table, float x, float y, int sx, int sy) {
+  return table_read_2d_at(table, table_col(x, sx), y, sx, sy);
+}
+
+constexpr float kThroughputEps = 1e-6f;
 
 struct Bsdf {
   uint32_t type;
@@ -925,34 +980,87 @@
          twoThirds * (sinTheta / cosTheta) * (1.f - sqr(sinTheta) * sinTheta);
 }
 
-DMT_DEV Bsdf bsdf_prepare(Rec32 const& r, f3 ns, f3 wo) {
+struct BsdfConst {
+  uint32_t type;
+  f3 weight;
+  union {
+    struct { float a, b; };
+    struct { float ax, ay; };
+  };
+  float eta;
+  uint32_t flags;
+  f3 c0;
+  float alpha2;
+  f3 c1;
+  float Eavg;
+  f3 Fss;
+  float colT;
+  int colIndex, colNext;
+  float sinPhi, cosPhi;
+  float phi0;
+  uint32_t pad[7];
+};
+static_assert(sizeof(BsdfConst) == 128, "BsdfConst: 128 bytes");
+constexpr uint32_t kBcIso = 1u, kBcReflection = 2u, kBcTransmission = 4u;
+
+DMT_DEV BsdfConst bsdf_decode(Rec32 const& r) {
+  BsdfConst c{};
+  c.type = hi16(r.w[1]);
+  c.weight = mk3(h2f(lo16(r.w[0])), h2f(hi16(r.w[0])), h2f(lo16(r.w[1])));
+  if (c.type == BS_OREN) {
+    c.a = h2f(hi16(r.w[5]));
+    c.b = h2f(lo16(r.w[6]));
+  } else if (c.type == BS_GGX_DIEL || c.type == BS_GGX_COND) {
+    c.phi0 = float(lo16(r.w[3])) / 65535 * 2.f * kPi;
+    uint32_t const axq = hi16(r.w[3]), ayq = lo16(r.w[4]);
+    c.ax = float(axq) / 65535;
+    c.ay = float(ayq) / 65535;
+    bool const conductor = c.type == BS_GGX_COND;
+    if (!conductor) {
+      c.eta = h2f(hi16(r.w[4]));
+      c.c0 = mk3(h2f(lo16(r.w[5])), h2f(hi16(r.w[5])), h2f(lo16(r.w[6])));
+      c.c1 = mk3(h2f(hi16(r.w[6])), h2f(lo16(r.w[7])), h2f(hi16(r.w[7])));
+      c.Fss = c.c1;
+    } else {
+      c.c0 = mk3(h2f(hi16(r.w[4])), h2f(lo16(r.w[5])), h2f(hi16(r.w[5])));
+      c.c1 = mk3(h2f(lo16(r.w[6])), h2f(hi16(r.w[6])), h2f(lo16(r.w[7])));
+      f3 const F0 = fresnel_conductor(1.f, c.c0, c.c1);
+      f3 const F82 = fresnel_conductor(1.f / 7.f, c.c0, c.c1);
+      f3 const B = (lerp3(F0, mk3(1, 1, 1), 0.46266436f) - F82) * 17.651384f;
+      c.Fss = lerp3(F0, mk3(1, 1, 1), 1.f / 21.f) - B * (1.f / 126.f);
+    }
+    c.alpha2 = c.ax * c.ay;
+    TableCol const col = table_col(c.alpha2, DMT_GGX_E_COLS);
+    c.colT = col.t, c.colIndex = col.index, c.colNext = col.nIndex;
+    c.Eavg = table_read(c_ggxEavg, c.alpha2, DMT_GGX_EAVG_COUNT);
+    sincos_bounded(c.phi0, c.sinPhi, c.cosPhi);
+    bool const hasReflection = conductor ? true : luminance(c.c0) > kThroughputEps;
+    bool const hasTransmission = conductor ? false : luminance(c.c1) > kThroughputEps;
+    c.flags = (axq == ayq ? kBcIso : 0u) | (hasReflection ? kBcReflection : 0u) | (hasTransmission ? kBcTransmission : 0u);
+  }
+  return c;
+}
+
+DMT_DEV Bsdf bsdf_prepare(BsdfConst const& c, f3 ns, f3 wo) {
   Bsdf b{};
-  b.type = hi16(r.w[1]);
-  b.weight = mk3(h2f(lo16(r.w[0])), h2f(hi16(r.w[0])), h2f(lo16(r.w[1])));
+  b.type = c.type;
+  b.weight = c.weight;
   if (b.type == BS_OREN) {
-    b.a = h2f(hi16(r.w[5]));
-    b.b = h2f(lo16(r.w[6]));
+    b.a = c.a;
+    b.b = c.b;
     float const nl = fmaxf(0.f, dot(ns, wo));
     float const Ev = b.a * kPi + b.b * oren_nayar_G(nl);
     f3 ms = b.weight * (1.f - Ev);
     ms = mk3(fmaxf(ms.x, 0.f), fmaxf(ms.y, 0.f), fmaxf(ms.z, 0.f));
     b.ms = q16(ms);
   } else if (b.type == BS_GGX_DIEL || b.type == BS_GGX_COND) {
-    b.phi0 = float(lo16(r.w[3])) / 65535 * 2.f * kPi;
-    uint32_t const axq = hi16(r.w[3]), ayq = lo16(r.w[4]);
-    b.iso = axq == ayq;
-    b.ax = float(axq) / 65535;
-    b.ay = float(ayq) / 65535;
-    f3 Fss;
-    if (b.type == BS_GGX_DIEL) {
-      b.eta = h2f(hi16(r.w[4]));
-      b.c0 = mk3(h2f(lo16(r.w[5])), h2f(hi16(r.w[5])), h2f(lo16(r.w[6])));
-      b.c1 = mk3(h2f(hi16(r.w[6])), h2f(lo16(r.w[7])), h2f(hi16(r.w[7])));
-      Fss = b.c1;
-    } else {
-      b.c0 = mk3(h2f(hi16(r.w[4])), h2f(lo16(r.w[5])), h2f(hi16(r.w[5])));
-      b.c1 = mk3(h2f(lo16(r.w[6])), h2f(hi16(r.w[6])), h2f(lo16(r.w[7])));
-    }
+    b.phi0 = c.phi0;
+    b.iso = (c.flags & kBcIso) != 0u;
+    b.ax = c.ax;
+    b.ay = c.ay;
+    b.eta = c.eta;
+    b.c0 = c.c0;
+    b.c1 = c.c1;
     {
       float const cos_HO = fabsf(dot(wo, ns));
       float unused = 0.f;
@@ -960,16 +1068,12 @@
       microfacet_fresnel(b, cos_HO, unused, R, T);
       b.weight = q16(R + T);
     }
-    if (b.type == BS_GGX_COND) {
-      f3 const F0 = fresnel_conductor(1.f, b.c0, b.c1);
-      f3 const F82 = fresnel_conductor(1.f / 7.f, b.c0, b.c1);
-      f3 const B = (lerp3(F0, mk3(1, 1, 1), 0.46266436f) - F82) * 17.651384f;
-      Fss = lerp3(F0, mk3(1, 1, 1), 1.f / 21.f) - B * (1.f / 126.f);
-    }
-    float const alpha2 = b.ax * b.ay;
+    f3 const Fss = c.Fss;
+    TableCol col;
+    col.index = c.colIndex, col.nIndex = c.colNext, col.t = c.colT;
     float const cos_NO = fmaxf(0.f, dot(ns, wo));
-    float const E = table_read_2d(c_ggxE, alpha2, cos_NO, DMT_GGX_E_COLS, DMT_GGX_E_ROWS);
-    float const Eavg = table_read(c_ggxEavg, alpha2, DMT_GGX_EAVG_COUNT);
+    float const E = table_read_2d_at(c_ggxE, col, cos_NO, DMT_GGX_E_COLS, DMT_GGX_E_ROWS);
+    float const Eavg = c.Eavg;
     float const missing = (1.f - E) / E;
     b.escale = 1.f + missing;
     f3 const Fms = Fss * Eavg / (mk3(1, 1, 1) - Fss * (1.f - Eavg));
@@ -977,6 +1081,7 @@
   }
   return b;
 }
+DMT_DEV Bsdf bsdf_prepare(Rec32 const& r, f3 ns, f3 wo) { return bsdf_prepare(bsdf_decode(r), ns, wo); }
 
 struct BsdfSample {
   f3 wi, f;
@@ -999,12 +1104,17 @@
   f3 const multi = b.ms * (1.f - El);
   return nl * (single + multi);
 }
-DMT_DEV f3 tangent_from_phi(f3 ns, float phi0) {
+struct BsdfLate {
+  BsdfConst const* rec;
+  uint32_t id;
+};
+DMT_DEV f3 tangent_from_phi(f3 ns, float phi0, BsdfLate late) {
   f3 const ref = fabsf(ns.x) < 0.999f ? mk3(1.0f, 0.0f, 0.0f) : mk3(0.0f, 1.0f, 0.0f);
   f3 const t = normalize(cross(ref, ns));
   f3 const bt = cross(ns, t);
   float s, c;
-  sincos_bounded(phi0, s, c);
+  if (late.rec) s = late.rec[late.id].sinPhi, c = late.rec[late.id].cosPhi;
+  else sincos_bounded(phi0, s, c);
   return c * t + s * bt;
 }
 DMT_DEV f3 sample_ggx_vndf(f3 wo, f2 u, float ax, float ay) {
@@ -1041,9 +1151,8 @@
 DMT_DEV float ggx_aniso_lambda(float ax, float ay, f3 V) {
   return ggx_lambda_from((sqr(ax * V.x) + sqr(ay * V.y)) / sqr(V.z));
 }
-constexpr float kThroughputEps = 1e-6f;
-
-DMT_DEV BsdfSample sample_ggx(Bsdf const& b, f3 wo, f3 ns, f3 ng, f2 u, float uc) {
+
+DMT_DEV BsdfSample sample_ggx(Bsdf const& b, f3 wo, f3 ns, f3 ng, f2 u, float uc, BsdfLate late) {
   BsdfSample s{};
   float const cos_NO = dot(ns, wo);
   s.eta = 1.f;
@@ -1055,7 +1164,7 @@
     if (b.iso)
       gram_schmidt(ns, X, Y);
     else
-      orthonormal_tangent(ns, tangent_from_phi(ns, b.phi0), X, Y);
+      orthonormal_tangent(ns, tangent_from_phi(ns, b.phi0, late), X, Y);
     lO = mk3(dot(X, wo), dot(Y, wo), cos_NO);
     lH = sample_ggx_vndf(lO, u, b.ax, b.ay);
     H = lH.x * X + lH.y * Y + lH.z * ns;
@@ -1103,10 +1212,16 @@
   }
   return s;
 }
-DMT_DEV f3 eval_ggx(Bsdf const& b, f3 wo, f3 wi, f3 ns, f3 ng, float& pdf) {
+DMT_DEV f3 eval_ggx(Bsdf const& b, f3 wo, f3 wi, f3 ns, f3 ng, float& pdf, BsdfLate late) {
   bool const conductor = b.type == BS_GGX_COND;
-  bool const hasReflection = conductor ? true : luminance(b.c0) > kThroughputEps;
-  bool const hasTransmission = conductor ? false : luminance(b.c1) > kThroughputEps;
+  bool hasReflection, hasTransmission;
+  if (late.rec) {
+    uint32_t const flags = late.rec[late.id].flags;
+    hasReflection = (flags & kBcReflection) != 0u, hasTransmission = (flags & kBcTransmission) != 0u;
+  } else {
+    hasReflection = conductor ? true : luminance(b.c0) > kThroughputEps;
+    hasTransmission = conductor ? false : luminance(b.c1) > kThroughputEps;
+  }
   bool const isotropic = b.ax == b.ay;
   float const cos_NO = dot(ns, wo);
   float const cos_NI = dot(ns, wi);
@@ -1139,7 +1254,7 @@
     lamO = ggx_lambda(alpha2, cos_NO);
   } else {
     f3 X, Y;
-    orthonormal_tangent(ns, tangent_from_phi(ns, b.phi0), X, Y);
+    orthonormal_tangent(ns, tangent_from_phi(ns, b.phi0, late), X, Y);
     f3 const lH = mk3(dot(X, H), dot(Y, H), dot(ns, H));
     f3 const lO = mk3(dot(X, wo), dot(Y, wo), cos_NO);
     f3 const lI = mk3(dot(X, wi), dot(Y, wi), cos_NI);
@@ -1154,7 +1269,7 @@
   return b.escale * (isT ? T : R) * common / (1.f + lamO + lamI);
 }
 
-DMT_DEV BsdfSample sample_bsdf(Bsdf const& b, f3 wo, f3 ns, f3 ng, f2 u, float uc) {
+DMT_DEV BsdfSample sample_bsdf(Bsdf const& b, f3 wo, f3 ns, f3 ng, f2 u, float uc, BsdfLate late = BsdfLate{nullptr, 0u}) {
   BsdfSample s{};
   if (dot(wo, ng) > 0.0f) {
     if (dot(ns, ng) < 0.0f) ns = -ns;
@@ -1167,12 +1282,12 @@
         s.pdf = 0;
       }
     } else {
-      s = sample_ggx(b, wo, ns, ng, u, uc);
+      s = sample_ggx(b, wo, ns, ng, u, uc, late);
     }
   }
   return s;
 }
-DMT_DEV f3 eval_bsdf(Bsdf const& b, f3 wo, f3 wi, f3 ns, f3 ng, float& pdf) {
+DMT_DEV f3 eval_bsdf(Bsdf const& b, f3 wo, f3 wi, f3 ns, f3 ng, float& pdf, BsdfLate late = BsdfLate{nullptr, 0u}) {
   pdf = 0;
   if (b.type == BS_OREN) {
     float const cos_NI = dot(ns, wi);
@@ -1187,7 +1302,7 @@
     pdf = cos_NI * kInvPi;
     return mk3(pdf, pdf, pdf);
   }
-  return eval_ggx(b, wo, wi, ns, ng, pdf);
+  return eval_ggx(b, wo, wi, ns, ng, pdf, late);
 }
 
 DMT_DEV uint32_t pick_index(float u, uint32_t count) {
diff --git a/include/dmt_hip.h b/include/dmt_hip.h
--- a/include/dmt_hip.h
+++ b/include/dmt_hip.h
@@ -95,6 +95,7 @@
 #define DMT_SAMPLER_TABLE_AUTO 1
 #define DMT_SAMPLER_TABLE_FORCE 2
 int dmt_set_sampler_table(dmt_ctx* ctx, int mode, uint64_t budget_bytes);
+int dmt_set_shade_constants(dmt_ctx* ctx, int on);
 typedef struct dmt_sampler_table_plan_record {
   uint32_t use;
   uint32_t period_width, period_height;
@@ -243,10 +244,15 @@
 int dmt_test_bsdf_ng(dmt_ctx* ctx, const void* bsdf32, int n, const float* ns3, const float* ng3, const float* wo3,
                      const float* u2, const float* uc, const float* wi_eval3, float* prepared12, float* sample10,
                      float* eval4);
+int dmt_test_bsdf_decoded(dmt_ctx* ctx, const void* bsdf32, int n, const float* ns3, const float* ng3, const float* wo3,
+                          const float* u2, const float* uc, const float* wi_eval3, float* prepared12, float* sample10,
+                          float* eval4);
 int dmt_test_material(dmt_ctx* ctx, int n, const int32_t* tri, const float* bu, const float* bv, const float* ng3, void* rec32,
                       float* ns3, void* rec2_32, float* mix);
 int dmt_test_light(dmt_ctx* ctx, const void* light32, int n, const float* pos3, const float* nrm3,
                    const float* u2, const int32_t* had_transmission, float* out14);
+int dmt_test_light_decoded(dmt_ctx* ctx, const void* light32, int n, const float* pos3, const float* nrm3,
+                           const float* u2, const int32_t* had_transmission, float* out14);
 int dmt_test_half(dmt_ctx* ctx, int n, const float* f_in, uint16_t* h_out, const uint16_t* h_in,
                   float* f_out);
 int dmt_test_trace_samples(dmt_ctx* ctx, int n, const int32_t* pxs, const int32_t* pys,
```
